# kocurvik/mdrp

Measured on AMD Instinct MI355X. Metric: image-pairs/sec (2000 corrs, 10k RANSAC iters), higher is better.
Workload: dtype f64

## Files before the change

### include/mdrp.h

```cpp
#ifndef MDRP_H
#define MDRP_H
#include <stddef.h>
#include <stdint.h>

#ifdef __cplusplus
extern "C" {
#endif

enum { MDRP_CALIB = 0, MDRP_SHARED_FOCAL = 1, MDRP_VARYING_FOCAL = 2,
       MDRP_RELPOSE_5PT = 3, MDRP_FUNDAMENTAL_7PT = 5,
       MDRP_SHARED_6PT = 4 };

enum {
    MDRP_OK = 0,
    MDRP_ERR_INVALID = 1,
    MDRP_ERR_HIP = 2,
    MDRP_ERR_NO_DEVICE = 3,
    MDRP_ERR_UNSUPPORTED = 4
};

enum {
    MDRP_MEM_HOST = 0,
    MDRP_MEM_DEVICE = 1
};

typedef struct {
    double q[4];
    double t[3];
    double scale, shift1, shift2;
    double f1, f2;
} mdrp_model;

typedef struct {
    uint64_t max_iterations;
    uint64_t min_iterations;
    double dyn_num_trials_mult;
    double success_prob;
    double max_reproj_error;
    double max_epipolar_error;
    uint64_t seed;
    int32_t monodepth_estimate_shift;
    float monodepth_weight_sampson;
    int32_t score_initial_model;
    int32_t progressive_sampling;
    uint64_t max_prosac_iterations;
    int32_t real_focal_check;
    int32_t reserved_;
} mdrp_ransac_opt;

typedef struct {
    uint64_t max_iterations;
    int32_t loss_type;
    double loss_scale;
    double gradient_tol;
    double step_tol;
    double initial_lambda;
    double min_lambda;
    double max_lambda;
} mdrp_bundle_opt;

typedef struct {
    int32_t model_id;
    int32_t pad_;
    double params[4];
} mdrp_camera;

typedef struct {
    mdrp_model model;
    uint64_t refinements, iterations, num_inliers;
    double inlier_ratio, model_score;
} mdrp_result;

typedef struct mdrp_handle mdrp_handle;

int mdrp_create_(int device, void *stream, mdrp_handle **out, int abi_version, int ransac_opt_bytes);
int mdrp_create_on_stream_(int device, void *stream, mdrp_handle **out, int abi_version, int ransac_opt_bytes);
#define mdrp_create(device, stream, out) mdrp_create_((device), (stream), (out), MDRP_ABI_VERSION, (int)sizeof(mdrp_ransac_opt))
#define mdrp_create_on_stream(device, stream, out) mdrp_create_on_stream_((device), (stream), (out), MDRP_ABI_VERSION, (int)sizeof(mdrp_ransac_opt))
void mdrp_destroy(mdrp_handle *h);
const char *mdrp_last_error(void);
const char *mdrp_version(void);
#define MDRP_ABI_VERSION 0x00000005
int mdrp_abi_version(void);
int mdrp_hip_build_version(void);
int mdrp_synchronize(mdrp_handle *h);

int mdrp_estimate_batch(mdrp_handle *h, int kind, int mem_space, const double *x1, const double *x2, const double *d1,
                        const double *d2, int batch, int n_max, const int32_t *n_per_pair, const mdrp_camera *cam1,
                        const mdrp_camera *cam2, const mdrp_ransac_opt *ropt, const mdrp_bundle_opt *bopt,
                        mdrp_result *out, uint8_t *inlier_mask);

int mdrp_estimate_batch_async(mdrp_handle *h, int kind, const double *x1_dev, const double *x2_dev, const double *d1_dev,
                              const double *d2_dev, int batch, int n_max, const int32_t *n_per_pair_host,
                              const mdrp_camera *cam1_host, const mdrp_camera *cam2_host, const mdrp_ransac_opt *ropt,
                              const mdrp_bundle_opt *bopt, uint8_t *inlier_mask_dev);
int mdrp_fetch_results(mdrp_handle *h, mdrp_result *out_host, int batch);
int mdrp_copy_results_device(mdrp_handle *h, void *dst_dev, int batch);

int mdrp_solver_batch(mdrp_handle *h, int solver, const double *x1h, const double *x2h, const double *d1,
                      const double *d2, int count, mdrp_model *out, int32_t *n_out);

int mdrp_classic_solver_batch(mdrp_handle *h, int kind, const double *x1h, const double *x2h, int count, mdrp_model *out,
                              int32_t *n_out);

int mdrp_score_models(mdrp_handle *h, int kind, int mem_space, const mdrp_model *models, int num_models,
                      const double *x1, const double *x2, int n, double sq_threshold, double *scores, int32_t *counts);

int mdrp_count_candidates(mdrp_handle *h, int kind, const mdrp_model *models, int num_models, const double *x1,
                          const double *x2, int n, double sq_threshold, int32_t *candidates);

int mdrp_bound_models(mdrp_handle *h, int kind, const mdrp_model *models, int num_models, const double *x1, const double *x2,
                      int n, double sq_threshold, double *score_lb, int32_t *count_ub);

int mdrp_refine_models(mdrp_handle *h, int kind, mdrp_model *models, int count, const double *x1, const double *x2,
                       const double *d1, const double *d2, int n, double scale_reproj, double weight_sampson,
                       const mdrp_bundle_opt *opt, int estimate_shift, double *final_cost );

int mdrp_last_sweep_stats(mdrp_handle *h, double *sweep_ms, int64_t *launches, int64_t *evaluations);

typedef struct {
    double count_ms;
    int64_t count_launches;
    double sweep_ms;
    int64_t sweep_launches;
    int64_t evals_algorithmic;
    int64_t evals_mfma;
    int64_t evals_fp64;
    int64_t evals_bound;
    double lo_ms;
    int64_t lo_launches;
    double final_ms;
    int64_t final_launches;
    double bound_ms;
    int64_t bound_launches;
    double solve_ms;
    int64_t solve_launches;
    int64_t lm_cost_evals;
    int64_t lm_accum_evals;
    int64_t final_cost_evals;
    int64_t final_accum_evals;
    int64_t fuse_gate_timeouts;
    int64_t fuse_wait_timeouts;
    int64_t first_chunk;
} mdrp_stats;
int mdrp_last_stats_sized(mdrp_handle *h, mdrp_stats *out, size_t out_size);
int mdrp_last_stats(mdrp_handle *h, mdrp_stats *out);

#ifdef __cplusplus
}
#endif
#endif
```

### mdrp_amd/_capi.py

```python
import ctypes as C
import os
import threading

import numpy as np

_HERE = os.path.dirname(os.path.abspath(__file__))
LIB_PATH = os.environ.get("MDRP_LIB") or os.path.join(_HERE, "libmdrp_hip.so")

CALIB, SHARED_FOCAL, VARYING_FOCAL = 0, 1, 2
RELPOSE_5PT, SHARED_6PT, FUNDAMENTAL_7PT = 3, 4, 5
MEM_HOST, MEM_DEVICE = 0, 1
SOLVER_P3P, SOLVER_SHIFT, SOLVER_SHARED, SOLVER_VARYING = 0, 1, 2, 3

EXPORTS = (
    "mdrp_create_", "mdrp_create_on_stream_", "mdrp_destroy", "mdrp_last_error", "mdrp_version", "mdrp_abi_version", "mdrp_hip_build_version", "mdrp_synchronize", "mdrp_estimate_batch",
    "mdrp_estimate_batch_async", "mdrp_fetch_results", "mdrp_copy_results_device", "mdrp_solver_batch", "mdrp_score_models", "mdrp_count_candidates", "mdrp_bound_models", "mdrp_refine_models",
    "mdrp_last_sweep_stats", "mdrp_last_stats", "mdrp_last_stats_sized", "mdrp_classic_solver_batch",
)


class Model(C.Structure):
    _fields_ = [("q", C.c_double * 4), ("t", C.c_double * 3), ("scale", C.c_double), ("shift1", C.c_double),
                ("shift2", C.c_double), ("f1", C.c_double), ("f2", C.c_double)]


class RansacOpt(C.Structure):
    _fields_ = [("max_iterations", C.c_uint64), ("min_iterations", C.c_uint64), ("dyn_num_trials_mult", C.c_double),
                ("success_prob", C.c_double), ("max_reproj_error", C.c_double), ("max_epipolar_error", C.c_double),
                ("seed", C.c_uint64), ("monodepth_estimate_shift", C.c_int32), ("monodepth_weight_sampson", C.c_float),
                ("score_initial_model", C.c_int32), ("progressive_sampling", C.c_int32), ("max_prosac_iterations", C.c_uint64),
                ("real_focal_check", C.c_int32), ("reserved_", C.c_int32)]


class BundleOpt(C.Structure):
    _fields_ = [("max_iterations", C.c_uint64), ("loss_type", C.c_int32), ("loss_scale", C.c_double),
                ("gradient_tol", C.c_double), ("step_tol", C.c_double), ("initial_lambda", C.c_double),
                ("min_lambda", C.c_double), ("max_lambda", C.c_double)]


class Camera(C.Structure):
    _fields_ = [("model_id", C.c_int32), ("pad_", C.c_int32), ("params", C.c_double * 4)]


class Stats(C.Structure):
    _fields_ = [("count_ms", C.c_double), ("count_launches", C.c_int64), ("sweep_ms", C.c_double), ("sweep_launches", C.c_int64),
                ("evals_algorithmic", C.c_int64), ("evals_mfma", C.c_int64), ("evals_fp64", C.c_int64), ("evals_bound", C.c_int64),
                ("lo_ms", C.c_double), ("lo_launches", C.c_int64), ("final_ms", C.c_double), ("final_launches", C.c_int64),
                ("bound_ms", C.c_double), ("bound_launches", C.c_int64), ("solve_ms", C.c_double), ("solve_launches", C.c_int64),
                ("lm_cost_evals", C.c_int64), ("lm_accum_evals", C.c_int64), ("final_cost_evals", C.c_int64), ("final_accum_evals", C.c_int64),
                ("fuse_gate_timeouts", C.c_int64), ("fuse_wait_timeouts", C.c_int64),
                ("first_chunk", C.c_int64)]


class Result(C.Structure):
    _fields_ = [("model", Model), ("refinements", C.c_uint64), ("iterations", C.c_uint64), ("num_inliers", C.c_uint64),
                ("inlier_ratio", C.c_double), ("model_score", C.c_double)]


MODEL_DTYPE = np.dtype([("q", "f8", 4), ("t", "f8", 3), ("scale", "f8"), ("shift1", "f8"), ("shift2", "f8"), ("f1", "f8"), ("f2", "f8")])
RESULT_DTYPE = np.dtype([("model", MODEL_DTYPE), ("refinements", "u8"), ("iterations", "u8"), ("num_inliers", "u8"),
                         ("inlier_ratio", "f8"), ("model_score", "f8")])
CAMERA_DTYPE = np.dtype([("model_id", "i4"), ("pad_", "i4"), ("params", "f8", 4)])
assert MODEL_DTYPE.itemsize == C.sizeof(Model) and RESULT_DTYPE.itemsize == C.sizeof(Result) and CAMERA_DTYPE.itemsize == C.sizeof(Camera)

_lib = None
_lib_lock = threading.Lock()


class MdrpError(RuntimeError):
    pass


def load_library():
    global _lib
    with _lib_lock:
        if _lib is not None:
            return _lib
        if not os.path.exists(LIB_PATH):
            raise MdrpError(f"{LIB_PATH} is not built (run __graft_entry__.build()); mdrp_amd has no CPU fallback")
        _ensure_hip_runtime()
        lib = C.CDLL(LIB_PATH)
        _check_hip_runtime_version(lib)
        vp, dp, ip = C.c_void_p, C.c_void_p, C.c_void_p
        lib.mdrp_last_error.restype = C.c_char_p
        lib.mdrp_version.restype = C.c_char_p
        abi = getattr(lib, "mdrp_abi_version", None)
        if abi is None or getattr(lib, "mdrp_create_", None) is None:
            raise MdrpError(f"{LIB_PATH} predates ABI {ABI_VERSION:#x} (no mdrp_abi_version / mdrp_create_): rebuild (mdrp_amd/build.py)")
        abi.restype = C.c_int
        if abi() != ABI_VERSION:
            raise MdrpError(f"{LIB_PATH} speaks ABI {abi():#x}, this binding {ABI_VERSION:#x}: rebuild (mdrp_amd/build.py)")
        lib.mdrp_create_.argtypes = [C.c_int, vp, C.POINTER(vp), C.c_int, C.c_int]
        lib.mdrp_create_on_stream_.argtypes = [C.c_int, vp, C.POINTER(vp), C.c_int, C.c_int]
        lib.mdrp_destroy.argtypes = [vp]
        lib.mdrp_destroy.restype = None
        lib.mdrp_synchronize.argtypes = [vp]
        lib.mdrp_estimate_batch.argtypes = [vp, C.c_int, C.c_int, dp, dp, dp, dp, C.c_int, C.c_int, ip, vp, vp,
                                            C.POINTER(RansacOpt), C.POINTER(BundleOpt), vp, vp]
        lib.mdrp_estimate_batch_async.argtypes = [vp, C.c_int, dp, dp, dp, dp, C.c_int, C.c_int, ip, vp, vp,
                                                  C.POINTER(RansacOpt), C.POINTER(BundleOpt), vp]
        lib.mdrp_fetch_results.argtypes = [vp, vp, C.c_int]
        lib.mdrp_copy_results_device.argtypes = [vp, vp, C.c_int]
        lib.mdrp_solver_batch.argtypes = [vp, C.c_int, dp, dp, dp, dp, C.c_int, vp, vp]
        lib.mdrp_score_models.argtypes = [vp, C.c_int, C.c_int, vp, C.c_int, dp, dp, C.c_int, C.c_double, vp, vp]
        lib.mdrp_count_candidates.argtypes = [vp, C.c_int, vp, C.c_int, dp, dp, C.c_int, C.c_double, vp]
        lib.mdrp_bound_models.argtypes = [vp, C.c_int, vp, C.c_int, dp, dp, C.c_int, C.c_double, vp, vp]
        lib.mdrp_refine_models.argtypes = [vp, C.c_int, vp, C.c_int, dp, dp, dp, dp, C.c_int, C.c_double, C.c_double,
                                           C.POINTER(BundleOpt), C.c_int, vp]
        lib.mdrp_last_sweep_stats.argtypes = [vp, C.POINTER(C.c_double), C.POINTER(C.c_int64), C.POINTER(C.c_int64)]
        lib.mdrp_last_stats.argtypes = [vp, C.POINTER(Stats)]
        lib.mdrp_last_stats_sized.argtypes = [vp, C.POINTER(Stats), C.c_size_t]
        lib.mdrp_classic_solver_batch.argtypes = [vp, C.c_int, dp, dp, C.c_int, vp, vp]
        _lib = lib
        return lib


ABI_VERSION = 0x00000005
ERR_UNSUPPORTED = 4


def _check(lib, rc):
    if rc == ERR_UNSUPPORTED:
        raise NotImplementedError(f"mdrp: {lib.mdrp_last_error().decode(errors='replace')} (DESIGN.md 9)")
    if rc != 0:
        raise MdrpError(f"mdrp error {rc}: {lib.mdrp_last_error().decode(errors='replace')}")


def _ptr(a):
    return None if a is None else C.c_void_p(a.ctypes.data)


def ransac_opt_from_dict(d=None):
    d = d or {}
    return RansacOpt(int(d.get("max_iterations", 100000)), int(d.get("min_iterations", 1000)),
                     float(d.get("dyn_num_trials_mult", 3.0)), float(d.get("success_prob", 0.9999)),
                     float(d.get("max_reproj_error", 12.0)), float(d.get("max_epipolar_error", 1.0)),
                     int(d.get("seed", 0)), int(bool(d.get("monodepth_estimate_shift", False))),
                     float(d.get("monodepth_weight_sampson", 1.0)), int(bool(d.get("score_initial_model", False))),
                     int(bool(d.get("progressive_sampling", False))), int(d.get("max_prosac_iterations", 100000)),
                     int(bool(d.get("real_focal_check", False))), 0)


LOSS_TYPES = {"TRIVIAL": 0, "TRUNCATED": 1, "HUBER": 2, "CAUCHY": 3, "TRUNCATED_CAUCHY": 4, "TRUNCATED_LE_ZACH": 5}


def bundle_opt_from_dict(d=None):
    d = d or {}
    lt = d.get("loss_type", "CAUCHY")
    if isinstance(lt, str):
        if lt.upper() not in LOSS_TYPES:
            raise ValueError(f"unknown loss_type {lt!r}")
        lt = LOSS_TYPES[lt.upper()]
    return BundleOpt(int(d.get("max_iterations", 100)), int(lt), float(d.get("loss_scale", 1.0)),
                     float(d.get("gradient_tol", 1e-10)), float(d.get("step_tol", 1e-8)), float(d.get("initial_lambda", 1e-3)),
                     float(d.get("min_lambda", 1e-10)), float(d.get("max_lambda", 1e10)))


def library_version():
    return load_library().mdrp_version().decode()


def library_source_hash():
    v = library_version()
    return v.split("MDRP_SRC_HASH=", 1)[1][:16] if "MDRP_SRC_HASH=" in v else None


_hip_runtime = None
hip_versions = None


def _check_hip_runtime_version(lib):
    import warnings
    try:
        lib.mdrp_hip_build_version.restype = C.c_int
        built = int(lib.mdrp_hip_build_version())
        v = C.c_int(0)
        rt = _hip_runtime.hipRuntimeGetVersion
        rt.argtypes = [C.POINTER(C.c_int)]
        if rt(C.byref(v)) != 0:
            return
    except (AttributeError, OSError):
        return
    have = int(v.value)
    if have // 10_000_000 != built // 10_000_000:
        raise MdrpError(f"libmdrp_hip.so was built against HIP {built // 10_000_000}.{built // 100_000 % 100} but the process's HIP runtime "
                        f"({getattr(_hip_runtime, '_name', '?')}) is {have // 10_000_000}.{have // 100_000 % 100}: set MDRP_HIP_RUNTIME to a "
                        "matching libamdhip64.so or rebuild (mdrp_amd/build.py)")
    global hip_versions
    hip_versions = {"built": built, "runtime": have}
    if have // 100_000 != built // 100_000 and os.environ.get("MDRP_DEBUG"):
        warnings.warn(f"mdrp: HIP runtime {have // 10_000_000}.{have // 100_000 % 100} in this process, library built against "
                      f"{built // 10_000_000}.{built // 100_000 % 100} (same major: continuing)", RuntimeWarning, stacklevel=3)


def _ensure_hip_runtime():
    global _hip_runtime
    if _hip_runtime is not None:
        return _hip_runtime
    import sys
    cands = []
    if os.environ.get("MDRP_HIP_RUNTIME"):
        cands.append(os.environ["MDRP_HIP_RUNTIME"])
    try:
        torch = sys.modules.get("torch")
        if torch is not None:
            tdir = os.path.dirname(torch.__file__)
        else:
            import importlib.util
            spec = importlib.util.find_spec("torch")
            tdir = list(spec.submodule_search_locations)[0] if spec is not None and spec.submodule_search_locations else None
        if tdir and os.path.exists(os.path.join(tdir, "lib", "libamdhip64.so")):
            cands.append(os.path.join(tdir, "lib", "libamdhip64.so"))
    except Exception:
        pass
    import glob
    rocm = os.environ.get("ROCM_PATH", "/opt/rocm")
    def _soname_version(path):
        tail = os.path.basename(path).split(".so.", 1)[-1]
        return tuple(int(x) for x in tail.split(".") if x.isdigit())
    cands += sorted(glob.glob(os.path.join(rocm, "lib", "libamdhip64.so.*")), key=_soname_version, reverse=True) + ["libamdhip64.so", os.path.join(rocm, "lib", "libamdhip64.so")]
    errs = []
    for c in cands:
        try:
            _hip_runtime = C.CDLL(c, mode=C.RTLD_GLOBAL)
            return _hip_runtime
        except OSError as e:
            errs.append(f"{c}: {e}")
    raise MdrpError("no HIP runtime (libamdhip64) could be loaded: " + "; ".join(errs))


class Handle:

    def __init__(self, device=0, stream=None):
        self._lib = load_library()
        h = C.c_void_p()
        if stream is None:
            _check(self._lib, self._lib.mdrp_create_(int(device), None, C.byref(h), ABI_VERSION, C.sizeof(RansacOpt)))
        else:
            _check(self._lib, self._lib.mdrp_create_on_stream_(int(device), C.c_void_p(int(stream)) if stream else None, C.byref(h), ABI_VERSION, C.sizeof(RansacOpt)))
        self._h = h
        self.device = int(device)
        self.stream = stream

    def close(self):
        if getattr(self, "_h", None):
            self._lib.mdrp_destroy(self._h)
            self._h = None

    def __del__(self):
        try:
            self.close()
        except Exception:
            pass

    def synchronize(self):
        _check(self._lib, self._lib.mdrp_synchronize(self._h))

    def estimate_batch(self, kind, x1, x2, d1, d2, ropt, bopt, n_per_pair=None, cam1=None, cam2=None, want_mask=True):
        x1 = np.ascontiguousarray(x1, dtype=np.float64)
        x2 = np.ascontiguousarray(x2, dtype=np.float64)
        if x1.ndim != 3 or x1.shape[2] != 2 or x2.shape != x1.shape:
            raise ValueError("expected x1,x2 (B,N,2)")
        if kind >= RELPOSE_5PT:
            d1 = d2 = None
        else:
            d1 = np.ascontiguousarray(d1, dtype=np.float64)
            d2 = np.ascontiguousarray(d2, dtype=np.float64)
            if d1.shape != x1.shape[:2] or d2.shape != d1.shape:
                raise ValueError("expected d1,d2 (B,N)")
        B, N = x1.shape[:2]
        npp = None if n_per_pair is None else np.ascontiguousarray(n_per_pair, dtype=np.int32)
        out = np.zeros(B, dtype=RESULT_DTYPE)
        mask = np.zeros((B, N), dtype=np.uint8) if want_mask else None
        c1 = None if cam1 is None else np.ascontiguousarray(cam1, dtype=CAMERA_DTYPE)
        c2 = None if cam2 is None else np.ascontiguousarray(cam2, dtype=CAMERA_DTYPE)
        _check(self._lib, self._lib.mdrp_estimate_batch(self._h, kind, MEM_HOST, _ptr(x1), _ptr(x2), _ptr(d1), _ptr(d2), B, N,
                                                        _ptr(npp), _ptr(c1), _ptr(c2), C.byref(ropt), C.byref(bopt),
                                                        _ptr(out), _ptr(mask)))
        return out, mask

    def estimate_batch_device(self, kind, x1_ptr, x2_ptr, d1_ptr, d2_ptr, batch, n_max, ropt, bopt, n_per_pair=None,
                              cam1=None, cam2=None, mask_ptr=None):
        npp = None if n_per_pair is None else np.ascontiguousarray(n_per_pair, dtype=np.int32)
        c1 = None if cam1 is None else np.ascontiguousarray(cam1, dtype=CAMERA_DTYPE)
        c2 = None if cam2 is None else np.ascontiguousarray(cam2, dtype=CAMERA_DTYPE)
        _check(self._lib, self._lib.mdrp_estimate_batch_async(self._h, kind, C.c_void_p(x1_ptr), C.c_void_p(x2_ptr),
                                                              C.c_void_p(d1_ptr) if d1_ptr else None, C.c_void_p(d2_ptr) if d2_ptr else None, int(batch), int(n_max),
                                                              _ptr(npp), _ptr(c1), _ptr(c2), C.byref(ropt), C.byref(bopt),
                                                              C.c_void_p(mask_ptr) if mask_ptr else None))

    def fetch_results(self, batch):
        out = np.zeros(batch, dtype=RESULT_DTYPE)
        _check(self._lib, self._lib.mdrp_fetch_results(self._h, _ptr(out), int(batch)))
        return out

    def copy_results_device(self, dst_ptr, batch):
        _check(self._lib, self._lib.mdrp_copy_results_device(self._h, C.c_void_p(dst_ptr), int(batch)))

    def last_sweep_stats(self):
        ms, launches, evals = C.c_double(0), C.c_int64(0), C.c_int64(0)
        _check(self._lib, self._lib.mdrp_last_sweep_stats(self._h, C.byref(ms), C.byref(launches), C.byref(evals)))
        return ms.value, launches.value, evals.value

    def last_stats(self):
        st = Stats()
        _check(self._lib, self._lib.mdrp_last_stats_sized(self._h, C.byref(st), C.sizeof(Stats)))
        d = {k: getattr(st, k) for k, _ in Stats._fields_}
        d["fuse_timeouts"] = d["fuse_gate_timeouts"] + d["fuse_wait_timeouts"]
        return d

    def solver_batch(self, solver, x1h, x2h, d1, d2):
        x1h = np.ascontiguousarray(x1h, dtype=np.float64).reshape(-1, 3, 3)
        x2h = np.ascontiguousarray(x2h, dtype=np.float64).reshape(-1, 3, 3)
        d1 = np.ascontiguousarray(d1, dtype=np.float64).reshape(-1, 3)
        d2 = np.ascontiguousarray(d2, dtype=np.float64).reshape(-1, 3)
        count = len(d1)
        out = np.zeros((count, 4), dtype=MODEL_DTYPE)
        n_out = np.zeros(count, dtype=np.int32)
        _check(self._lib, self._lib.mdrp_solver_batch(self._h, int(solver), _ptr(x1h), _ptr(x2h), _ptr(d1), _ptr(d2), count,
                                                      _ptr(out), _ptr(n_out)))
        return out, n_out

    def classic_solver_batch(self, kind, x1h, x2h):
        K, M = {RELPOSE_5PT: (5, 10), SHARED_6PT: (6, 15), FUNDAMENTAL_7PT: (7, 3)}[kind]
        x1h = np.ascontiguousarray(x1h, dtype=np.float64).reshape(-1, K, 3)
        x2h = np.ascontiguousarray(x2h, dtype=np.float64).reshape(-1, K, 3)
        count = len(x1h)
        out = np.zeros((count, M), dtype=MODEL_DTYPE)
        n_out = np.zeros(count, dtype=np.int32)
        _check(self._lib, self._lib.mdrp_classic_solver_batch(self._h, int(kind), _ptr(x1h), _ptr(x2h), count, _ptr(out), _ptr(n_out)))
        return out, n_out

    def score_models(self, kind, models, x1, x2, sq_threshold):
        models = np.ascontiguousarray(models, dtype=MODEL_DTYPE).reshape(-1)
        x1 = np.ascontiguousarray(x1, dtype=np.float64)
        x2 = np.ascontiguousarray(x2, dtype=np.float64)
        scores = np.zeros(len(models))
        counts = np.zeros(len(models), dtype=np.int32)
        _check(self._lib, self._lib.mdrp_score_models(self._h, int(kind), MEM_HOST, _ptr(models), len(models), _ptr(x1), _ptr(x2),
                                                      len(x1), float(sq_threshold), _ptr(scores), _ptr(counts)))
        return scores, counts

    def count_candidates(self, kind, models, x1, x2, sq_threshold):
        models = np.ascontiguousarray(models, dtype=MODEL_DTYPE).reshape(-1)
        x1 = np.ascontiguousarray(x1, dtype=np.float64)
        x2 = np.ascontiguousarray(x2, dtype=np.float64)
        cand = np.zeros(len(models), dtype=np.int32)
        _check(self._lib, self._lib.mdrp_count_candidates(self._h, int(kind), _ptr(models), len(models), _ptr(x1), _ptr(x2), len(x1),
                                                          float(sq_threshold), _ptr(cand)))
        return cand

    def bound_models(self, kind, models, x1, x2, sq_threshold):
        models = np.ascontiguousarray(models, dtype=MODEL_DTYPE).reshape(-1)
        x1 = np.ascontiguousarray(x1, dtype=np.float64)
        x2 = np.ascontiguousarray(x2, dtype=np.float64)
        lb = np.zeros(len(models))
        ub = np.zeros(len(models), dtype=np.int32)
        _check(self._lib, self._lib.mdrp_bound_models(self._h, int(kind), _ptr(models), len(models), _ptr(x1), _ptr(x2), len(x1),
                                                      float(sq_threshold), _ptr(lb), _ptr(ub)))
        return lb, ub

    def score_models_device(self, kind, models_ptr, num_models, x1_ptr, x2_ptr, n, sq_threshold, scores_ptr, counts_ptr):
        _check(self._lib, self._lib.mdrp_score_models(self._h, int(kind), MEM_DEVICE, C.c_void_p(models_ptr), int(num_models),
                                                      C.c_void_p(x1_ptr), C.c_void_p(x2_ptr), int(n), float(sq_threshold),
                                                      C.c_void_p(scores_ptr), C.c_void_p(counts_ptr)))

    def refine_models(self, kind, models, x1, x2, d1, d2, scale_reproj, weight_sampson, bopt, estimate_shift=False):
        models = np.ascontiguousarray(models, dtype=MODEL_DTYPE).reshape(-1).copy()
        x1 = np.ascontiguousarray(x1, dtype=np.float64)
        x2 = np.ascontiguousarray(x2, dtype=np.float64)
        d1 = None if d1 is None else np.ascontiguousarray(d1, dtype=np.float64)
        d2 = None if d2 is None else np.ascontiguousarray(d2, dtype=np.float64)
        cost = np.zeros(len(models))
        _check(self._lib, self._lib.mdrp_refine_models(self._h, int(kind), _ptr(models), len(models), _ptr(x1), _ptr(x2), _ptr(d1),
                                                       _ptr(d2), len(x1), float(scale_reproj), float(weight_sampson), C.byref(bopt),
                                                       int(bool(estimate_shift)), _ptr(cost)))
        return models, cost


_default_tls = threading.local()


def default_handle(device=0):
    handles = getattr(_default_tls, "handles", None)
    if handles is None:
        handles = _default_tls.handles = {}
    h = handles.get(device)
    if h is None:
        h = handles[device] = Handle(device)
    return h


def fundamental_to_model(F):
    m = np.zeros((), dtype=MODEL_DTYPE)
    flat = np.asarray(F, dtype=np.float64).reshape(9)
    m["q"] = flat[:4]; m["t"] = flat[4:7]; m["scale"] = flat[7]; m["shift1"] = flat[8]
    m["f1"] = m["f2"] = 1.0
    return m


def model_to_fundamental(m):
    return np.r_[m["q"], m["t"], m["scale"], m["shift1"]].reshape(3, 3).copy()


def model_to_array(m):
    return np.concatenate([m["q"], m["t"], [m["scale"], m["shift1"], m["shift2"], m["f1"], m["f2"]]]).astype(np.float64)


def array_to_models(a):
    a = np.asarray(a, dtype=np.float64).reshape(-1, 12)
    out = np.zeros(len(a), dtype=MODEL_DTYPE)
    out["q"] = a[:, :4]; out["t"] = a[:, 4:7]; out["scale"] = a[:, 7]; out["shift1"] = a[:, 8]; out["shift2"] = a[:, 9]
    out["f1"] = a[:, 10]; out["f2"] = a[:, 11]
    return out
```

### mdrp_amd/csrc/mdrp_capi.hip

```cpp
#include "../../include/mdrp.h"
#include "mdrp_kernels.h"
#include "mdrp_classic.h"
#ifdef MDRP_SPLIT_TU
#define MDRP_INST extern
#include "mdrp_instances.h"
namespace mdrp {
MDRP_INSTANCES_FINAL_64
MDRP_INSTANCES_FINAL_256
MDRP_INSTANCES_CLASSIC
}
#endif

#include <algorithm>
#include <cmath>
#include <cstdio>
#include <cstdlib>
#include <cstddef>
#include <cstring>
#include <functional>
#include <map>
#include <memory>
#include <mutex>
#include <string>
#include <vector>

using namespace mdrp;

static_assert(sizeof(mdrp_model) == sizeof(Model), "model layout");
static_assert(sizeof(mdrp_camera) == sizeof(CamDev), "camera layout");
static_assert(sizeof(mdrp_result) == sizeof(ResultDev), "result layout");

namespace {

thread_local std::string g_err;

#define HIPCHK(expr)                                                                                       \
    do {                                                                                                   \
        hipError_t e_ = (expr);                                                                            \
        if (e_ != hipSuccess) {                                                                            \
            char buf_[512];                                                                                \
            snprintf(buf_, sizeof buf_, "%s failed: %s (%s:%d)", #expr, hipGetErrorString(e_), __FILE__, __LINE__); \
            g_err = buf_;                                                                                  \
            return MDRP_ERR_HIP;                                                                           \
        }                                                                                                  \
    } while (0)

struct DevBuf {
    void *p = nullptr;
    size_t cap = 0;
    DevBuf() = default;
    DevBuf(const DevBuf &) = delete;
    DevBuf &operator=(const DevBuf &) = delete;
    ~DevBuf() { release(); }
    int ensure(size_t bytes) {
        if (bytes <= cap) return MDRP_OK;
        if (p) { (void)hipFree(p); p = nullptr; cap = 0; }
        size_t want = bytes + bytes / 8 + 256;
        hipError_t e = hipMalloc(&p, want);
        if (e != hipSuccess) { g_err = std::string("hipMalloc failed: ") + hipGetErrorString(e); p = nullptr; return MDRP_ERR_HIP; }
        cap = want;
        return MDRP_OK;
    }
    void release() { if (p) (void)hipFree(p); p = nullptr; cap = 0; }
    template <typename T> T *as() const { return reinterpret_cast<T *>(p); }
};

template <typename T, auto Destroy> struct Owned {
    T v = nullptr;
    Owned() = default;
    Owned(Owned &&o) noexcept : v(o.v) { o.v = nullptr; }
    Owned(const Owned &) = delete;
    Owned &operator=(const Owned &) = delete;
    ~Owned() { reset(); }
    void reset() { if (v) (void)Destroy(v); v = nullptr; }
    operator T() const { return v; }
    T operator->() const { return v; }
};
using Stream = Owned<hipStream_t, hipStreamDestroy>;
using Event = Owned<hipEvent_t, hipEventDestroy>;
template <typename T> using Pinned = Owned<T *, hipHostFree>;

struct Progress {
    int32_t n_active, pad_;
    unsigned long long max_needed;
    unsigned long long evals;
    unsigned long long evals_mfma;
    unsigned long long evals_sweep;
    unsigned long long evals_bound;
    int32_t wish_sum, wish_pairs;
};
struct Counters {
    int32_t unused_[2];
    Progress progress;
    int32_t lo_head[16];
    int32_t xcd_head[8 * LO_XCD_STRIDE];
};
static_assert(offsetof(Counters, progress) == 2 * sizeof(int32_t) && offsetof(Counters, lo_head) == 16 * sizeof(int32_t) &&
              offsetof(Counters, xcd_head) == 32 * sizeof(int32_t) && sizeof(Counters) == 640, "counter block layout");
static_assert(offsetof(Progress, evals_mfma) == offsetof(Progress, evals) + sizeof(unsigned long long), "k_count adds to stats[0] and stats[1]");
static_assert(offsetof(Progress, wish_pairs) == offsetof(Progress, wish_sum) + sizeof(int32_t), "RunParams::inl_stat is [2]");
constexpr size_t LM_STATS_BYTES = 6 * sizeof(unsigned long long);

struct DeviceGuard {
    int prev = -1;
    bool ok = true;
    explicit DeviceGuard(int device) {
        if (hipGetDevice(&prev) != hipSuccess) prev = -1;
        if (prev != device) ok = hipSetDevice(device) == hipSuccess;
    }
    ~DeviceGuard() {
        int cur = -1;
        if (prev >= 0 && hipGetDevice(&cur) == hipSuccess && cur != prev) (void)hipSetDevice(prev);
    }
};

}

struct mdrp_handle {
    std::mutex mu;
    int device = 0;
    hipStream_t stream = nullptr;
    Stream own_stream;
    Stream aux_stream;
    Stream aux_stream2;
    Stream copy_stream;
    Event ev_copied, ev_prepped, ev_solved6;
    DevBuf fuse;
    static constexpr int NC_MAX = 8;
    Event ev_lo, ev_tables, ev_sampled[2], ev_solved[NC_MAX], ev_scanned[NC_MAX];
    int num_cu = 256;
    DevBuf pts, dep, st;
    DevBuf params;
    Pinned<unsigned char> params_host;
    size_t params_host_cap = 0;
    DevBuf models, slot_score, slot_inl, triggers, work_pair, counters, results, mask, plan;
    DevBuf samples[2], tags[2], model_count[2];
    DevBuf tags_sorted[2];
    DevBuf tags_v, surv_count;
    DevBuf cand_stat;
    DevBuf und_count;
    DevBuf rfrag;
    DevBuf cplan;
    DevBuf surv2_count;
    DevBuf lo_mask;
    DevBuf red5;
    DevBuf lm_stats;
    Pinned<unsigned long long> lm_stats_host;
    int64_t fuse_gate_timeouts = 0, fuse_wait_timeouts = 0;
    int64_t first_chunk = 0;
    double seen_wish[3] = {-1.0, -1.0, -1.0};
    Pinned<int32_t> wish_host; Event ev_wish;
    int wish_kind = -1;
    bool fuse_disabled = false;
    int fuse_retry_in = 0;
    int fuse_backoff = 64;
    DevBuf in_x1, in_x2, in_d1, in_d2;
    DevBuf unit_a, unit_b, unit_c, unit_d, unit_e, unit_f;
    Pinned<Progress> progress_host;
    std::vector<std::pair<Event, Event>> ev_pool;
    std::vector<int> ev_what;
    size_t ev_used = 0;
    double sweep_ms = 0.0, count_ms = 0.0;
    double kind_ms[6] = {0, 0, 0, 0, 0, 0};
    int64_t kind_launches[6] = {0, 0, 0, 0, 0, 0};
    int64_t lm_cost_evals = 0, lm_accum_evals = 0, fin_cost_evals = 0, fin_accum_evals = 0;
    int64_t count_launches = 0;
    int64_t sweep_launches = 0, sweep_evals = 0, mfma_evals = 0, fp64_evals = 0, bound_evals = 0;
    int last_batch = 0;
};

namespace {

#define MDRP_LM_DISPATCH_T(KERNEL, T, kind, shift, grid, smem, stream, ...)                                          \
    do {                                                                                                             \
        if ((kind) == 0 && (shift)) hipLaunchKernelGGL((KERNEL<0, true, T>), grid, dim3(T), smem, stream, __VA_ARGS__);  \
        else if ((kind) == 0) hipLaunchKernelGGL((KERNEL<0, false, T>), grid, dim3(T), smem, stream, __VA_ARGS__);       \
        else if ((kind) == 1) hipLaunchKernelGGL((KERNEL<1, false, T>), grid, dim3(T), smem, stream, __VA_ARGS__);       \
        else hipLaunchKernelGGL((KERNEL<2, false, T>), grid, dim3(T), smem, stream, __VA_ARGS__);                        \
    } while (0)
#define MDRP_LM_DISPATCH(KERNEL, threads, kind, shift, grid, smem, stream, ...)                                      \
    do {                                                                                                             \
        if ((threads) == 64) MDRP_LM_DISPATCH_T(KERNEL, 64, kind, shift, grid, smem, stream, __VA_ARGS__);           \
        else MDRP_LM_DISPATCH_T(KERNEL, 256, kind, shift, grid, smem, stream, __VA_ARGS__);                          \
    } while (0)

#define MDRP_FINAL_DISPATCH_L(T, FL, kind, shift, grid, smem, stream, ...)                                                  \
    do {                                                                                                                   \
        if ((kind) == 0 && (shift)) hipLaunchKernelGGL((k_final<0, true, T, FL>), grid, dim3(T), smem, stream, __VA_ARGS__);  \
        else if ((kind) == 0) hipLaunchKernelGGL((k_final<0, false, T, FL>), grid, dim3(T), smem, stream, __VA_ARGS__);       \
        else if ((kind) == 1) hipLaunchKernelGGL((k_final<1, false, T, FL>), grid, dim3(T), smem, stream, __VA_ARGS__);       \
        else hipLaunchKernelGGL((k_final<2, false, T, FL>), grid, dim3(T), smem, stream, __VA_ARGS__);                        \
    } while (0)
#define MDRP_FINAL_DISPATCH_T(T, floss, kind, shift, grid, smem, stream, ...)                                               \
    do {                                                                                                                   \
        switch (floss) {                                                                                                   \
        case 1: MDRP_FINAL_DISPATCH_L(T, 1, kind, shift, grid, smem, stream, __VA_ARGS__); break;                          \
        case 2: MDRP_FINAL_DISPATCH_L(T, 2, kind, shift, grid, smem, stream, __VA_ARGS__); break;                          \
        case 3: MDRP_FINAL_DISPATCH_L(T, 3, kind, shift, grid, smem, stream, __VA_ARGS__); break;                          \
        case 4: MDRP_FINAL_DISPATCH_L(T, 4, kind, shift, grid, smem, stream, __VA_ARGS__); break;                          \
        case 5: MDRP_FINAL_DISPATCH_L(T, 5, kind, shift, grid, smem, stream, __VA_ARGS__); break;                          \
        default: MDRP_FINAL_DISPATCH_L(T, 0, kind, shift, grid, smem, stream, __VA_ARGS__); break;  \
        }                                                                                                                  \
    } while (0)
#define MDRP_FINAL_DISPATCH(threads, floss, kind, shift, grid, smem, stream, ...)                                           \
    do {                                                                                                                   \
        if ((threads) == 64) MDRP_FINAL_DISPATCH_T(64, floss, kind, shift, grid, smem, stream, __VA_ARGS__);               \
        else MDRP_FINAL_DISPATCH_T(256, floss, kind, shift, grid, smem, stream, __VA_ARGS__);                              \
    } while (0)

#define MDRP_SWEEP_DISPATCH(KERNEL, kind, grid, block, smem, stream, ...)                                                       \
    do {                                                                                                                        \
        if ((kind) == MDRP_CALIB || (kind) == MDRP_RELPOSE_5PT) hipLaunchKernelGGL((KERNEL<true, false>), grid, block, smem, stream, __VA_ARGS__); \
        else if ((kind) == MDRP_FUNDAMENTAL_7PT) hipLaunchKernelGGL((KERNEL<false, true>), grid, block, smem, stream, __VA_ARGS__); \
        else hipLaunchKernelGGL((KERNEL<false, false>), grid, block, smem, stream, __VA_ARGS__);                                 \
    } while (0)
#define MDRP_CLASSIC_LM_DISPATCH(KERNEL, threads, kind, grid, smem, stream, ...)                                                 \
    do {                                                                                                                        \
        if ((kind) == MDRP_RELPOSE_5PT && (threads) == 64) hipLaunchKernelGGL((KERNEL<CLASSIC_RELPOSE, 64>), grid, dim3(64), smem, stream, __VA_ARGS__); \
        else if ((kind) == MDRP_RELPOSE_5PT) hipLaunchKernelGGL((KERNEL<CLASSIC_RELPOSE, 256>), grid, dim3(256), smem, stream, __VA_ARGS__); \
        else if ((kind) == MDRP_SHARED_6PT && (threads) == 64) hipLaunchKernelGGL((KERNEL<CLASSIC_SHARED, 64>), grid, dim3(64), smem, stream, __VA_ARGS__); \
        else if ((kind) == MDRP_SHARED_6PT) hipLaunchKernelGGL((KERNEL<CLASSIC_SHARED, 256>), grid, dim3(256), smem, stream, __VA_ARGS__); \
        else if ((threads) == 64) hipLaunchKernelGGL((KERNEL<CLASSIC_FUND, 64>), grid, dim3(64), smem, stream, __VA_ARGS__);      \
        else hipLaunchKernelGGL((KERNEL<CLASSIC_FUND, 256>), grid, dim3(256), smem, stream, __VA_ARGS__);                        \
    } while (0)

int env_int(const char *name, int dflt) {
    const char *v = getenv(name);
    return v ? atoi(v) : dflt;
}

int lm_list_stride(int n_max) { return n_max <= LM_LIST_MAX_N ? ((n_max + 63) / 64) * 64 : 0; }
size_t lm_list_bytes(int n_max) { return (size_t)2 * lm_list_stride(n_max) * sizeof(uint16_t); }
int lm_mask_index_on(int n_max) { return lm_list_stride(n_max) > 0 && (size_t)3 * lm_list_stride(n_max) * sizeof(uint16_t) <= 32768 ? 1 : 0; }
size_t lm_final_list_bytes(int n_max) { return (size_t)(2 + lm_mask_index_on(n_max)) * lm_list_stride(n_max) * sizeof(uint16_t); }

int get_events(mdrp_handle *h, hipEvent_t *a, hipEvent_t *b, int what = 0) {
    if (h->ev_used == h->ev_pool.size()) {
        Event x, y;
        HIPCHK(hipEventCreate(&x.v));
        HIPCHK(hipEventCreate(&y.v));
        h->ev_pool.emplace_back(std::move(x), std::move(y));
        h->ev_what.push_back(0);
    }
    h->ev_what[h->ev_used] = what;
    *a = h->ev_pool[h->ev_used].first;
    *b = h->ev_pool[h->ev_used].second;
    h->ev_used++;
    return MDRP_OK;
}

int solver_for(int kind, int est_shift) {
    if (kind == MDRP_CALIB) return est_shift ? SOLVER_SHIFT : SOLVER_P3P;
    return kind == MDRP_SHARED_FOCAL ? SOLVER_SHARED : SOLVER_VARYING;
}

int model_slots(int kind) { return kind == MDRP_RELPOSE_5PT ? 12 : (kind == MDRP_SHARED_6PT ? 16 : 4); }
int sample_size(int kind) { return kind == MDRP_RELPOSE_5PT ? 5 : (kind == MDRP_SHARED_6PT ? 6 : (kind == MDRP_FUNDAMENTAL_7PT ? 7 : 3)); }

bool env_chunks(std::vector<uint64_t> &lead) {
    lead.clear();
    const char *e = getenv("MDRP_CHUNKS");
    if (!e) return false;
    const std::string spec = e;
    size_t pos = 0;
    while (pos < spec.size() && (int)lead.size() < mdrp_handle::NC_MAX - 1) {
        const size_t q = spec.find(',', pos);
        const long v = atol(spec.substr(pos, q == std::string::npos ? std::string::npos : q - pos).c_str());
        if (v > 0) lead.push_back((uint64_t)v);
        if (q == std::string::npos) break;
        pos = q + 1;
    }
    return true;
}

struct PassScratch {
    std::vector<std::pair<DevBuf *, size_t>> bufs;
    size_t fuse;
    size_t params, off_cam1, off_cam2, off_tn, off_tof, off_nper;
    size_t red5_blocks, red5_first_blocks;
    size_t total() const {
        size_t t = fuse;
        for (const auto &b : bufs) t += b.second;
        return t;
    }
};

PassScratch pass_scratch(mdrp_handle *h, int kind, int batch, int n_max, int n_tables, int chunk_cap, const std::vector<uint64_t> &lead) {
    const size_t b = (size_t)batch, n = (size_t)n_max, t = (size_t)n_tables, slots = b * chunk_cap * model_slots(kind);
    PassScratch z;
    z.fuse = 64 + 3 * sizeof(int32_t) * b;
    z.off_cam1 = sizeof(uint64_t) * t; z.off_cam2 = z.off_cam1 + sizeof(CamDev) * b; z.off_tn = z.off_cam2 + sizeof(CamDev) * b;
    z.off_tof = z.off_tn + sizeof(int32_t) * t; z.off_nper = z.off_tof + sizeof(int32_t) * b; z.params = z.off_nper + sizeof(int32_t) * b;
    z.red5_blocks = ((size_t)chunk_cap + 63) / 64;
    z.red5_first_blocks = (std::min<uint64_t>(lead.empty() ? 0 : lead[0], (uint64_t)chunk_cap / 2) + 63) / 64;
    const size_t samples = sizeof(uint32_t) * sample_size(kind) * t * chunk_cap, tags = sizeof(uint32_t) * slots, pair2 = sizeof(int32_t) * 2 * b;
    z.bufs = {
        {&h->pts, sizeof(double) * PT_STRIDE * b * n}, {&h->dep, kind >= MDRP_RELPOSE_5PT ? 0 : sizeof(double) * 2 * b * n}, {&h->st, sizeof(PairState) * b},
        {&h->samples[0], samples}, {&h->params, z.params},
        {&h->models, sizeof(Model) * slots}, {&h->slot_score, sizeof(double) * slots}, {&h->slot_inl, sizeof(int32_t) * slots},
        {&h->tags[0], tags}, {&h->model_count[0], pair2}, {&h->model_count[1], pair2}, {&h->tags[1], tags}, {&h->tags_sorted[0], tags},
        {&h->tags_sorted[1], tags}, {&h->samples[1], samples}, {&h->tags_v, tags},
        {&h->surv_count, sizeof(int32_t) * b}, {&h->cand_stat, sizeof(unsigned long long) * 2 * b}, {&h->und_count, pair2},
        {&h->cplan, sizeof(int32_t) * (b + 1)}, {&h->surv2_count, sizeof(int32_t) * b},
        {&h->rfrag, std::max<size_t>(1024, b * ((n + 15) / 16) * 1024)},
        {&h->triggers, sizeof(Trigger) * b * chunk_cap},
        {&h->work_pair, sizeof(int32_t) * (3 * b + 2)},
        {&h->counters, sizeof(Counters)},
        {&h->plan, sizeof(int32_t) * (2 * b + 2 + 4 + 16)},
        {&h->lo_mask, (kind == MDRP_RELPOSE_5PT || kind == MDRP_SHARED_6PT) ? (size_t)h->num_cu * 8 * std::max<size_t>(n, 1) : 0},
        {&h->red5, kind == MDRP_RELPOSE_5PT ? sizeof(double) * b * (z.red5_blocks + z.red5_first_blocks) * RED5_STRIDE * 64 : 0}};
    return z;
}

struct HostSrc { const double *x1, *x2, *d1, *d2; };
constexpr int HOST_SLICE_PAIRS = 256;

int run_pass(mdrp_handle *h, int kind, const double *x1, const double *x2, const double *d1, const double *d2, int batch,
             int n_max, const int32_t *n_host, const mdrp_camera *cam1, const mdrp_camera *cam2, const mdrp_ransac_opt *ro,
             const mdrp_bundle_opt *bo, int chunk_cap, uint8_t *mask_dev, ResultDev *results_dev, const HostSrc *host, int batch_call) {
    hipStream_t s = h->stream;
    const int est_shift = (kind == MDRP_CALIB && ro->monodepth_estimate_shift) ? 1 : 0;
    const bool classic = kind >= MDRP_RELPOSE_5PT;
    const int mps = model_slots(kind), ssz = sample_size(kind);

    std::vector<int32_t> table_of(batch), tab_n;
    {
        std::map<int32_t, int32_t> ids;
        for (int i = 0; i < batch; ++i) {
            auto it = ids.find(n_host[i]);
            if (it == ids.end()) { it = ids.emplace(n_host[i], (int32_t)tab_n.size()).first; tab_n.push_back(n_host[i]); }
            table_of[i] = it->second;
        }
    }
    const int n_tables = (int)tab_n.size();
    std::vector<uint64_t> tab_state(n_tables, ro->seed);

    const uint64_t certain = ro->max_iterations == 0 ? 1 : std::min<uint64_t>(ro->max_iterations, ro->min_iterations + 1);
    std::vector<uint64_t> lead;
    const bool chunks_set = env_chunks(lead);
    if (h->wish_kind >= 0 && hipEventQuery(h->ev_wish) == hipSuccess) {
        if (h->wish_host[1] > 0) h->seen_wish[h->wish_kind] = (double)h->wish_host[0] / (double)h->wish_host[1];
        h->wish_kind = -1;
    }
    if (!chunks_set) {
        if (kind == MDRP_FUNDAMENTAL_7PT) lead = {128, 1024};
        else if (kind == MDRP_SHARED_6PT) lead = {128};
        else if (kind == MDRP_RELPOSE_5PT) lead = {std::min<uint64_t>(512, std::max<uint64_t>(128, certain / 16 / 64 * 64))};
        else {
            lead = {std::min<uint64_t>(256, std::max<uint64_t>(128, certain / 16 / 64 * 64))};
            if (h->seen_wish[kind] >= 0.0 && certain >= 8192)
                lead[0] = (uint64_t)std::min(1024.0, std::max(128.0, std::ceil(h->seen_wish[kind] / 64.0) * 64.0));
        }
    }

    const PassScratch sz = pass_scratch(h, kind, batch, n_max, n_tables, chunk_cap, lead);
    int rc;
    for (const auto &b : sz.bufs) {
        if ((rc = b.first->ensure(b.second))) return rc;
        if (b.first == &h->params && h->params_host_cap < sz.params) {
            h->params_host.reset(); h->params_host_cap = 0;
            HIPCHK(hipHostMalloc((void **)&h->params_host.v, sz.params + sz.params / 2, hipHostMallocDefault));
            h->params_host_cap = sz.params + sz.params / 2;
        }
    }
    unsigned char *pd = h->params.as<unsigned char>();
    uint64_t *d_table_state = reinterpret_cast<uint64_t *>(pd);
    CamDev *d_cams1 = reinterpret_cast<CamDev *>(pd + sz.off_cam1), *d_cams2 = reinterpret_cast<CamDev *>(pd + sz.off_cam2);
    int32_t *d_table_n = reinterpret_cast<int32_t *>(pd + sz.off_tn), *d_table_of = reinterpret_cast<int32_t *>(pd + sz.off_tof),
            *d_nper = reinterpret_cast<int32_t *>(pd + sz.off_nper);
    Counters *cnt = h->counters.as<Counters>();
    const size_t groups_max = ((size_t)n_max + 15) / 16;
    const int trig_cap = chunk_cap;

    {
        unsigned char *ph = h->params_host;
        std::memcpy(ph, tab_state.data(), sizeof(uint64_t) * n_tables);
        const bool cams = kind == MDRP_CALIB || kind == MDRP_RELPOSE_5PT || kind == MDRP_SHARED_6PT;
        if (cams) { std::memcpy(ph + sz.off_cam1, cam1, sizeof(CamDev) * batch); std::memcpy(ph + sz.off_cam2, cam2 ? cam2 : cam1, sizeof(CamDev) * batch); }
        else std::memset(ph + sz.off_cam1, 0, 2 * sizeof(CamDev) * (size_t)batch);
        std::memcpy(ph + sz.off_tn, tab_n.data(), sizeof(int32_t) * n_tables);
        std::memcpy(ph + sz.off_tof, table_of.data(), sizeof(int32_t) * batch);
        std::memcpy(ph + sz.off_nper, n_host, sizeof(int32_t) * batch);
        HIPCHK(hipMemcpyAsync(pd, ph, sz.params, hipMemcpyHostToDevice, s));
    }
    HIPCHK(hipEventRecord(h->ev_tables, s));

    RunParams rp;
    std::memset(&rp, 0, sizeof rp);
    rp.kind = kind; rp.solver = solver_for(kind, est_shift); rp.est_shift = est_shift;
    rp.score_initial = ro->score_initial_model ? 1 : 0;
    rp.batch = batch; rp.n_max = n_max;
    rp.max_iterations = ro->max_iterations; rp.min_iterations = ro->min_iterations;
    rp.dyn_mult = ro->dyn_num_trials_mult; rp.log_prob_missing = std::log(1.0 - ro->success_prob);
    rp.weight_sampson = ro->monodepth_weight_sampson > 0.0f ? (double)ro->monodepth_weight_sampson : 0.0;
    rp.final_max_it = (int)std::min<uint64_t>(bo->max_iterations, 1u << 30); rp.final_loss = bo->loss_type;
    rp.grad_tol = bo->gradient_tol; rp.step_tol = bo->step_tol; rp.lambda0 = bo->initial_lambda;
    rp.lambda_min = bo->min_lambda; rp.lambda_max = bo->max_lambda;
    rp.chunk_len = chunk_cap; rp.chunk_off = 0; rp.slot_stride = chunk_cap * mps; rp.super_len = chunk_cap; rp.chunk_start = 0;
    rp.mps = mps; rp.sample_sz = ssz;

    auto launch_prep = [&](int p0, int pc, hipStream_t ps_) {
        const size_t o2 = (size_t)2 * p0 * n_max, o1 = (size_t)p0 * n_max;
        double *pts_p = h->pts.as<double>() + o1 * PT_STRIDE;
        uint4 *rfrag_p = h->rfrag.as<uint4>() + (size_t)p0 * groups_max * 64;
        if (classic)
            hipLaunchKernelGGL(kc_prep, dim3(pc), dim3(256), 0, ps_, rp, x1 + o2, x2 + o2, d_nper + p0, d_table_of + p0, d_cams1 + p0, d_cams2 + p0,
                               ro->max_epipolar_error, bo->loss_scale, pts_p, h->st.as<PairState>() + p0, rfrag_p);
        else
            hipLaunchKernelGGL(k_prep, dim3(pc), dim3(256), 0, ps_, rp, x1 + o2, x2 + o2, d1 + o1, d2 + o1, d_nper + p0, d_table_of + p0, d_cams1 + p0, d_cams2 + p0,
                               ro->max_epipolar_error, ro->max_reproj_error, bo->loss_scale, pts_p, h->dep.as<double>() + 2 * o1, h->st.as<PairState>() + p0, rfrag_p);
    };
    if (!host) {
        launch_prep(0, batch, s);
        HIPCHK(hipGetLastError());
    }
    rp.inl_stat = classic ? nullptr : &cnt->progress.wish_sum;

    const bool lo_overlap = env_int("MDRP_LO_OVERLAP", 1) != 0;
    const bool use_bound = env_int("MDRP_BOUND", 1) != 0;
    const bool score_split = env_int("MDRP_SCORE_SPLIT", 1) != 0;
    const int lo_threads = env_int("MDRP_LO_THREADS", (batch_call >= 128 && n_max < 4096) ? 64 : 256);
    const int final_threads = env_int("MDRP_FINAL_THREADS", batch_call >= 4096 ? 64 : 256);
    const int mask_index = lm_mask_index_on(n_max);
    const int clm_list_stride = lm_list_stride(n_max);
    const size_t clm_list_bytes = (size_t)2 * clm_list_stride * sizeof(uint16_t);
    const bool fuse_env = env_int("MDRP_FUSE_TAIL", ((kind == MDRP_CALIB && est_shift) || h->fuse_disabled) ? 0 : 1) != 0;
    bool final_done = false;
    auto launch_final = [&](const int32_t *ready, int32_t *fin_done, unsigned long long ticks, unsigned long long *timeouts) {
        if (classic)
            MDRP_CLASSIC_LM_DISPATCH(kc_final, final_threads, kind, dim3(batch), clm_list_bytes, s, rp, h->st.as<PairState>(), h->pts.as<double>(), mask_dev, results_dev,
                                     ready, fin_done, ticks, timeouts, clm_list_stride);
        else
            MDRP_FINAL_DISPATCH(final_threads, rp.final_loss, kind, est_shift, dim3(batch), (mask_index ? lm_final_list_bytes(n_max) : lm_list_bytes(n_max)), s, rp,
                                h->st.as<PairState>(), h->pts.as<double>(), h->dep.as<double>(), mask_dev, results_dev, lm_list_stride(n_max), mask_index,
                                h->lm_stats.as<unsigned long long>() + 2, ready, fin_done, ticks, timeouts);
    };
    const size_t tile_bytes = SCORE_TILE_BYTES;

    uint64_t it0 = 0;
    uint64_t max_needed = 0;
    while (true) {
        uint64_t lens[mdrp_handle::NC_MAX] = {0};
        int n_chunks = 1;
        if (it0 < certain) {
            const uint64_t span = std::min<uint64_t>(certain - it0, (uint64_t)chunk_cap);
            uint64_t used = 0;
            n_chunks = 0;
            if (it0 == 0)
                for (uint64_t l : lead) {
                    if (used + 2 * l > span) break;
                    lens[n_chunks++] = l; used += l;
                }
            lens[n_chunks++] = span - used;
        } else {
            lens[0] = std::min<uint64_t>(std::min<uint64_t>(std::max<uint64_t>(max_needed, 256), ro->max_iterations - it0), (uint64_t)chunk_cap);
        }
        uint64_t super_len = 0;
        for (int c = 0; c < n_chunks; ++c) super_len += lens[c];
        if (it0 == 0) h->first_chunk = (int64_t)lens[0];
        rp.chunk_start = it0; rp.super_len = (int)super_len;
        HIPCHK(hipMemsetAsync(h->counters.p, 0, sizeof(Counters), s));
        if (it0 == 0) HIPCHK(hipMemsetAsync(h->cand_stat.p, 0, sizeof(unsigned long long) * 2 * batch, s));
        const bool piped = n_chunks > 1 && lo_overlap;
        const bool fuse_tail = fuse_env && piped && it0 + super_len >= ro->max_iterations;
        int32_t *fz_ctl = nullptr, *fz_done = nullptr, *fz_fin = nullptr, *fz_ready = nullptr;
        if (fuse_tail) {
            if ((rc = h->fuse.ensure(sz.fuse))) return rc;
            fz_ctl = h->fuse.as<int32_t>(); fz_done = fz_ctl + 16; fz_fin = fz_done + batch; fz_ready = fz_fin + batch;
        }
        hipStream_t aux = piped ? h->aux_stream : s, aux2 = piped ? h->aux_stream2 : s;
        int offs[mdrp_handle::NC_MAX] = {0};
        for (int c = 1; c < n_chunks; ++c) offs[c] = offs[c - 1] + (int)lens[c - 1];
        const int samp_threads = env_int("MDRP_SAMPLE_THREADS", ssz == 3 ? SAMP_THREADS : (ssz == 5 ? 512 : 256));
        auto launch_samples = [&](hipStream_t st_, int len_, uint32_t *smp_) {
            if (ssz == 6) hipLaunchKernelGGL(kc_samples<6>, dim3(n_tables), dim3(samp_threads), 0, st_, n_tables, d_table_n, d_table_state, len_, smp_);
            else if (ssz == 5) hipLaunchKernelGGL(kc_samples<5>, dim3(n_tables), dim3(samp_threads), 0, st_, n_tables, d_table_n, d_table_state, len_, smp_);
            else if (ssz == 7) hipLaunchKernelGGL(kc_samples<7>, dim3(n_tables), dim3(samp_threads), 0, st_, n_tables, d_table_n, d_table_state, len_, smp_);
            else hipLaunchKernelGGL(k_samples, dim3(n_tables), dim3(samp_threads), 0, st_, n_tables, d_table_n, d_table_state, len_, smp_);
        };
        bool presampled[2] = {false, false};
        if (piped && it0 == 0) {
            HIPCHK(hipStreamWaitEvent(aux2, h->ev_tables, 0));
            for (int c = 0; c < 2 && c < n_chunks; ++c) {
                launch_samples(aux2, (int)lens[c], h->samples[c & 1].as<uint32_t>());
                HIPCHK(hipEventRecord(h->ev_sampled[c], aux2));
                presampled[c] = true;
            }
        }
        auto issue_solve = [&](int c, hipStream_t st_, int p0, int pc) -> int {
            RunParams r = rp;
            r.chunk_len = (int)lens[c]; r.chunk_off = offs[c]; r.batch = pc;
            const size_t so = (size_t)p0 * rp.slot_stride;
            uint32_t *tg = h->tags[c & 1].as<uint32_t>() + so;
            uint32_t *smp = h->samples[c & 1].as<uint32_t>();
            int32_t *mc = h->model_count[c & 1].as<int32_t>() + 2 * (size_t)p0;
            HIPCHK(hipMemsetAsync(mc, 0, sizeof(int32_t) * 2 * pc, st_));
            if (c < 2 && presampled[c]) HIPCHK(hipStreamWaitEvent(st_, h->ev_sampled[c], 0));
            else launch_samples(st_, r.chunk_len, smp);
            hipEvent_t v0, v1;
            int rc_;
            if ((rc_ = get_events(h, &v0, &v1, 5))) return rc_;
            HIPCHK(hipEventRecord(v0, st_));
            struct Stop { hipEvent_t e; hipStream_t s; ~Stop() { (void)hipEventRecord(e, s); } } stop_{v1, st_};
            PairState *st_p = h->st.as<PairState>() + p0;
            double *pts_p = h->pts.as<double>() + (size_t)p0 * n_max * PT_STRIDE;
            Model *models_p = h->models.as<Model>() + so;
            int32_t *inl_p = h->slot_inl.as<int32_t>() + so;
            if (classic) {
                const dim3 sgrid((r.chunk_len + 63) / 64, pc);
                if (kind == MDRP_SHARED_6PT)
                    hipLaunchKernelGGL(kc_solve<CLASSIC_SHARED>, sgrid, dim3(64), 0, st_, r, st_p, smp, pts_p, models_p, inl_p, tg, mc);
                else if (kind == MDRP_RELPOSE_5PT) {
                    const bool first_region = c == 0 && n_chunks > 1;
                    if (first_region && (size_t)sgrid.x > sz.red5_first_blocks) { g_err = "5-point first chunk longer than its Reduce5 region"; return MDRP_ERR_INVALID; }
                    double *red5 = h->red5.as<double>() + ((first_region ? (size_t)batch * sz.red5_blocks : 0) + (size_t)p0 * sgrid.x) * RED5_STRIDE * 64;
                    hipLaunchKernelGGL(kc_solve5_null, sgrid, dim3(64), SOLVE5N_LDS_BYTES, st_, r, st_p, smp, pts_p, red5);
                    hipLaunchKernelGGL(kc_solve5_reduce, sgrid, dim3(64), SOLVE5_LDS_BYTES, st_, r, st_p, red5);
                    hipLaunchKernelGGL(kc_solve5_roots, sgrid, dim3(64), SOLVE5B_LDS_BYTES, st_, r, st_p, smp, pts_p, red5, models_p, inl_p, tg, mc);
                }
                else
                    hipLaunchKernelGGL(kc_solve<CLASSIC_FUND>, sgrid, dim3(64), SOLVE7_LDS_BYTES, st_, r, st_p, smp, pts_p, models_p, inl_p, tg, mc);
                return MDRP_OK;
            }
            double *dep_p = h->dep.as<double>() + (size_t)p0 * n_max * 2;
#define MDRP_SOLVE_LAUNCH(S)                                                                                                   \
    hipLaunchKernelGGL(k_solve<S>, dim3((r.chunk_len + solve_threads(S) - 1) / solve_threads(S), pc), dim3(solve_threads(S)), 0, st_, r, st_p, smp, pts_p, dep_p, models_p, inl_p, tg, mc, 0, r.chunk_len)
            switch (r.solver) {
            case SOLVER_P3P: MDRP_SOLVE_LAUNCH(SOLVER_P3P); break;
            case SOLVER_SHIFT: MDRP_SOLVE_LAUNCH(SOLVER_SHIFT); break;
            case SOLVER_SHARED: MDRP_SOLVE_LAUNCH(SOLVER_SHARED); break;
            default: MDRP_SOLVE_LAUNCH(SOLVER_VARYING); break;
            }
#undef MDRP_SOLVE_LAUNCH
            return MDRP_OK;
        };
        auto sweep_chunk = [&](int c, int p0, int pc) -> int {
            RunParams r = rp;
            r.chunk_len = (int)lens[c]; r.chunk_off = offs[c]; r.batch = pc;
            const int len = r.chunk_len;
            const bool odd = c & 1;
            const size_t so = (size_t)p0 * rp.slot_stride;
            PairState *st_p = h->st.as<PairState>() + p0;
            const double *pts_p = h->pts.as<double>() + (size_t)p0 * n_max * PT_STRIDE;
            const Model *models_p = h->models.as<Model>() + so;
            uint32_t *tags_sc = h->tags_sorted[odd].as<uint32_t>() + so;
            int32_t *mcount_c = h->model_count[odd].as<int32_t>() + 2 * (size_t)p0;
            uint32_t *tags_c = h->tags[odd].as<uint32_t>() + so;
            uint32_t *tags_v = h->tags_v.as<uint32_t>() + so;
            int32_t *surv1 = h->surv_count.as<int32_t>() + p0, *surv2 = h->surv2_count.as<int32_t>() + p0;
            hipEvent_t e0, e1;
            int rc_;
            if ((rc_ = get_events(h, &e0, &e1, 0))) return rc_;
            unsigned long long *cstats = &cnt->progress.evals;
            {
                hipEvent_t c0, c1;
                if ((rc_ = get_events(h, &c0, &c1, 1))) return rc_;
                const bool two_phase = !(it0 == 0 && c == 0);
                unsigned long long *cand_stat = h->cand_stat.as<unsigned long long>() + 2 * (size_t)p0;
                uint32_t *tags_u = tags_sc;
                int32_t *und_part = reinterpret_cast<int32_t *>(h->tags_sorted[!odd].as<uint32_t>() + so), *und_cnt = h->und_count.as<int32_t>() + 2 * (size_t)p0;
                const uint4 *rfrag_p = h->rfrag.as<uint4>() + (size_t)p0 * groups_max * 64;
                hipLaunchKernelGGL(k_count_plan, dim3(1), dim3(PLAN_THREADS), 0, s, pc, st_p, mcount_c, 2, CNT_WG_MODELS, h->cplan.as<int32_t>(),
                                   surv1, (const int32_t *)nullptr, two_phase ? und_cnt : (int32_t *)nullptr);
                const dim3 cgrid((unsigned)pc * (unsigned)((len * mps + CNT_WG_MODELS - 1) / CNT_WG_MODELS));
                HIPCHK(hipEventRecord(c0, s));
                MDRP_SWEEP_DISPATCH(k_count, kind, cgrid, dim3(CNT_THREADS), 0, s, r, st_p, rfrag_p, models_p,
                                    tags_c, mcount_c, h->cplan.as<int32_t>(), tags_v, surv1, cstats, (int32_t *)nullptr, (const int32_t *)nullptr,
                                    1, tags_u, und_part, und_cnt, (const int32_t *)nullptr, cand_stat);
                if (two_phase) {
                    hipLaunchKernelGGL(k_count_plan, dim3(1), dim3(PLAN_THREADS), 0, s, pc, st_p, und_cnt, 2, CNT_WG_MODELS, h->cplan.as<int32_t>(),
                                       (int32_t *)nullptr, (const int32_t *)nullptr, (int32_t *)nullptr);
                    MDRP_SWEEP_DISPATCH(k_count, kind, cgrid, dim3(CNT_THREADS), 0, s, r, st_p, rfrag_p, models_p,
                                        tags_u, und_cnt, h->cplan.as<int32_t>(), tags_v, surv1, cstats, (int32_t *)nullptr, (const int32_t *)nullptr,
                                        2, (uint32_t *)nullptr, (int32_t *)nullptr, (int32_t *)nullptr, und_part, cand_stat);
                    h->count_launches++;
                }
                HIPCHK(hipEventRecord(c1, s));
                h->count_launches++;
            }
            const uint32_t *surv_tags = tags_v;
            const int32_t *surv_cnt = surv1;
            if (use_bound && batch_call > 16 && !(it0 == 0 && c == 0)) {
                hipLaunchKernelGGL(k_count_plan, dim3(1), dim3(PLAN_THREADS), 0, s, pc, st_p, surv1, 1, BND_THREADS, h->cplan.as<int32_t>(), surv2, (const int32_t *)nullptr);
                const dim3 bgrid((unsigned)pc * (unsigned)((len * mps + BND_THREADS - 1) / BND_THREADS));
                unsigned long long *bstats = &cnt->progress.evals_bound;
                hipEvent_t b0, b1;
                if ((rc_ = get_events(h, &b0, &b1, 4))) return rc_;
                HIPCHK(hipEventRecord(b0, s));
                MDRP_SWEEP_DISPATCH(k_bound, kind, bgrid, dim3(BND_THREADS), 0, s, r, st_p, pts_p, models_p, tags_v, surv1, h->cplan.as<int32_t>(), tags_c, surv2, bstats);
                HIPCHK(hipEventRecord(b1, s));
                surv_tags = tags_c; surv_cnt = surv2;
            }
            int32_t *plan = h->plan.as<int32_t>(), *totals = plan + 2 * (size_t)batch + 2;
            if (batch_call <= SCORE_WAVE_MAX_PAIRS) {
                hipLaunchKernelGGL(k_count_plan, dim3(1), dim3(PLAN_THREADS), 0, s, pc, st_p, surv_cnt, 1, SCW_THREADS / 64, plan, (int32_t *)nullptr, (const int32_t *)nullptr, (int32_t *)nullptr);
                hipLaunchKernelGGL(k_sort_tags, dim3(pc), dim3(256), 0, s, r, st_p, mcount_c, surv_cnt, surv_tags, tags_sc);
                HIPCHK(hipEventRecord(e0, s));
                const long long ub = (long long)pc * ((len * mps + SCW_THREADS / 64 - 1) / (SCW_THREADS / 64));
                const dim3 grid((unsigned)std::min<long long>(ub, (long long)h->num_cu * 32));
                MDRP_SWEEP_DISPATCH(k_score_w, kind, grid, dim3(SCW_THREADS), 0, s, r, st_p, pts_p, models_p, tags_sc, mcount_c,
                                    h->slot_score.as<double>() + so, h->slot_inl.as<int32_t>() + so, plan);
            } else if (score_split && !(it0 == 0 && c == 0)) {
                hipLaunchKernelGGL(k_sort_tags, dim3(pc), dim3(256), 0, s, r, st_p, mcount_c, surv_cnt, surv_tags, tags_sc);
                hipLaunchKernelGGL(k_plan, dim3(1), dim3(PLAN_THREADS), 0, s, pc, mcount_c, plan, totals, SPLIT_HYP);
                HIPCHK(hipEventRecord(e0, s));
                const long long ub = (long long)pc * ((len * mps + SPLIT_HYP - 1) / SPLIT_HYP + 1);
                const dim3 grid((unsigned)std::min<long long>(ub, (long long)h->num_cu * 32));
                MDRP_SWEEP_DISPATCH(k_score_split, kind, grid, dim3(SPLIT_THREADS), 0, s, r, st_p, pts_p, models_p, tags_sc, mcount_c,
                                    h->slot_score.as<double>() + so, h->slot_inl.as<int32_t>() + so, plan, totals);
            } else {
                hipLaunchKernelGGL(k_sort_tags, dim3(pc), dim3(256), 0, s, r, st_p, mcount_c, surv_cnt, surv_tags, tags_sc);
                hipLaunchKernelGGL(k_plan, dim3(1), dim3(PLAN_THREADS), 0, s, pc, mcount_c, plan, totals, SCORE_THREADS);
                HIPCHK(hipEventRecord(e0, s));
                const dim3 grid((unsigned)pc * (unsigned)((len * mps + SCORE_THREADS - 1) / SCORE_THREADS));
                MDRP_SWEEP_DISPATCH(k_score, kind, grid, dim3(SCORE_THREADS), tile_bytes, s, r, st_p, pts_p, models_p, tags_sc, mcount_c,
                                    h->slot_score.as<double>() + so, h->slot_inl.as<int32_t>() + so, plan, totals);
            }
            HIPCHK(hipEventRecord(e1, s));
            h->sweep_launches++;
            Trigger *trig_p = h->triggers.as<Trigger>() + (size_t)p0 * trig_cap;
            unsigned long long *scan_stats = &cnt->progress.evals_sweep;
#define MDRP_SCAN(M, I) hipLaunchKernelGGL((k_scan<M, I>), dim3(pc), dim3(64), 0, s, r, st_p, h->slot_score.as<double>() + so, h->slot_inl.as<int32_t>() + so, trig_p, trig_cap, mcount_c, scan_stats)
            if (mps == 16) MDRP_SCAN(16, 1);
            else if (mps == 12) MDRP_SCAN(12, 1);
            else if (len >= 1024) MDRP_SCAN(4, 4);
            else MDRP_SCAN(4, 1);
#undef MDRP_SCAN
            return MDRP_OK;
        };
        bool solved1 = false;
        int swept0 = 0;
        if (host && it0 == 0) {
            const bool sliced = piped && n_chunks >= 2 && batch >= 2 * HOST_SLICE_PAIRS;
            const int sl = sliced ? HOST_SLICE_PAIRS : batch;
            for (int p0 = 0; p0 < batch; p0 += sl) {
                const int pc = std::min(sl, batch - p0);
                const size_t o2 = (size_t)2 * p0 * n_max, o1 = (size_t)p0 * n_max, n2 = sizeof(double) * 2 * (size_t)pc * n_max, n1 = sizeof(double) * (size_t)pc * n_max;
                hipStream_t cs = sliced ? h->copy_stream : s;
                HIPCHK(hipMemcpyAsync(const_cast<double *>(x1) + o2, host->x1 + o2, n2, hipMemcpyHostToDevice, cs));
                HIPCHK(hipMemcpyAsync(const_cast<double *>(x2) + o2, host->x2 + o2, n2, hipMemcpyHostToDevice, cs));
                if (host->d1 && host->d2) {
                    HIPCHK(hipMemcpyAsync(const_cast<double *>(d1) + o1, host->d1 + o1, n1, hipMemcpyHostToDevice, cs));
                    HIPCHK(hipMemcpyAsync(const_cast<double *>(d2) + o1, host->d2 + o1, n1, hipMemcpyHostToDevice, cs));
                }
                if (!sliced) { launch_prep(p0, pc, s); break; }
                HIPCHK(hipEventRecord(h->ev_copied, cs)); HIPCHK(hipStreamWaitEvent(aux, h->ev_copied, 0));
                if (p0 == 0) HIPCHK(hipStreamWaitEvent(aux, h->ev_tables, 0));
                launch_prep(p0, pc, aux);
                HIPCHK(hipEventRecord(h->ev_prepped, aux));
                if ((rc = issue_solve(1, aux, p0, pc))) return rc;
                const bool last = p0 + sl >= batch, last_but_one = !last && p0 + 2 * sl >= batch;
                if (last_but_one || last) HIPCHK(hipStreamWaitEvent(s, h->ev_prepped, 0));
                auto solve_first = [&](int q0, int qc) -> int {
                    if (kind != MDRP_SHARED_6PT) return issue_solve(0, s, q0, qc);
                    int rc_ = issue_solve(0, aux, q0, qc);
                    if (rc_) return rc_;
                    HIPCHK(hipEventRecord(h->ev_solved6, aux));
                    HIPCHK(hipStreamWaitEvent(s, h->ev_solved6, 0));
                    return MDRP_OK;
                };
                if (last_but_one) { swept0 = p0 + pc; if ((rc = solve_first(0, swept0)) || (rc = sweep_chunk(0, 0, swept0))) return rc; }
                if (last) { if ((rc = solve_first(swept0, batch - swept0)) || (rc = sweep_chunk(0, swept0, batch - swept0))) return rc; swept0 = batch; }
            }
            if (sliced) { HIPCHK(hipEventRecord(h->ev_solved[1], aux)); solved1 = true; }
        }
        if (swept0 < batch && (rc = issue_solve(0, s, 0, batch))) return rc;
        if (piped) HIPCHK(hipEventRecord(h->ev_solved[0], s));
        for (int c = 0; c < n_chunks; ++c) {
            rp.chunk_len = (int)lens[c]; rp.chunk_off = offs[c];
            if (c == 0 && swept0 >= batch) {
                if (piped) HIPCHK(hipEventRecord(h->ev_scanned[0], s));
                continue;
            }
            if (piped && c + 1 < n_chunks && !(c == 0 && solved1)) {
                HIPCHK(hipStreamWaitEvent(aux, c == 0 ? h->ev_solved[0] : h->ev_scanned[c - 1], 0));
                if ((rc = issue_solve(c + 1, aux, 0, batch))) return rc;
                HIPCHK(hipEventRecord(h->ev_solved[c + 1], aux));
            }
            if (piped && c > 0) HIPCHK(hipStreamWaitEvent(s, h->ev_solved[c], 0));
            if (!piped && c > 0 && (rc = issue_solve(c, s, 0, batch))) return rc;
            if ((rc = sweep_chunk(c, 0, batch))) return rc;
            if (c + 1 < n_chunks) {
                if (piped) HIPCHK(hipEventRecord(h->ev_scanned[c], s));
                continue;
            }
            int32_t *lo_plan = h->work_pair.as<int32_t>();
            hipLaunchKernelGGL(k_lo_plan, dim3(1), dim3(PLAN_THREADS), 0, s, batch, h->st.as<PairState>(), (const int32_t *)nullptr, lo_plan);
            if (fuse_tail) {
                HIPCHK(hipMemsetAsync(fz_ctl, 0, 64 + 2 * sizeof(int32_t) * (size_t)batch, s));
                HIPCHK(hipMemsetAsync(fz_ready, 0xFF, sizeof(int32_t) * (size_t)batch, s));
            }
            if (piped) { HIPCHK(hipEventRecord(h->ev_scanned[c], s)); HIPCHK(hipStreamWaitEvent(aux2, h->ev_scanned[c], 0)); }
            const int lo_blocks = h->num_cu * (lo_threads == 64 ? 8 : 2);
            const FuseTail fz = fuse_tail ? FuseTail{fz_done, fz_ready, fz_ctl, h->st.as<PairState>()} : FuseTail{nullptr, nullptr, nullptr, nullptr};
            unsigned long long *lm_stats = h->lm_stats.as<unsigned long long>();
            int32_t *xheads = cnt->xcd_head;
            hipEvent_t l0, l1;
            if ((rc = get_events(h, &l0, &l1, 2))) return rc;
            HIPCHK(hipEventRecord(l0, aux2));
            if (classic)
                MDRP_CLASSIC_LM_DISPATCH(kc_lo, lo_threads, kind, dim3(lo_blocks), clm_list_bytes, aux2, rp, h->st.as<PairState>(), h->pts.as<double>(),
                                         h->models.as<Model>(), h->triggers.as<Trigger>(), trig_cap, lo_plan, cnt->lo_head, xheads,
                                         h->lo_mask.as<uint8_t>(), clm_list_stride, fz);
            else
                MDRP_LM_DISPATCH(k_lo, lo_threads, kind, est_shift, dim3(lo_blocks), lm_list_bytes(n_max), aux2, rp,
                                 h->st.as<PairState>(), h->pts.as<double>(), h->dep.as<double>(), h->models.as<Model>(), h->triggers.as<Trigger>(),
                                 trig_cap, lo_plan, cnt->lo_head, xheads, lm_list_stride(n_max), lm_stats, fz);
            HIPCHK(hipEventRecord(l1, aux2));
        }
        if (fuse_tail) {
            const int32_t *plan_l = h->work_pair.as<int32_t>();
            const int lo_blocks_l = h->num_cu * (lo_threads == 64 ? 8 : 2);
            const long long n_scale = std::max(1, (n_max + 1999) / 2000);
            const unsigned long long gate_ticks = 100ull * (unsigned long long)env_int("MDRP_FUSE_GATE_US", (int)std::min<long long>((50000 + 40ll * batch) * n_scale, 200000));
            const unsigned long long wait_ticks = 100ull * (unsigned long long)env_int("MDRP_FUSE_WAIT_US", (int)std::min<long long>((20000 + 4ll * batch) * n_scale, 100000));
            hipLaunchKernelGGL(k_gate, dim3(1), dim3(1), 0, s, (const int32_t *)cnt->lo_head, plan_l + 3 * (size_t)batch + 1,
                               (const int32_t *)fz_ctl, lo_blocks_l, gate_ticks, h->lm_stats.as<unsigned long long>() + 4);
            hipEvent_t g0, g1;
            if ((rc = get_events(h, &g0, &g1, 3))) return rc;
            HIPCHK(hipEventRecord(g0, s));
            launch_final(fz_ready, fz_fin, wait_ticks, h->lm_stats.as<unsigned long long>() + 5);
            HIPCHK(hipEventRecord(g1, s));
            final_done = true;
        }
        if (piped) { HIPCHK(hipEventRecord(h->ev_lo, aux2)); HIPCHK(hipStreamWaitEvent(s, h->ev_lo, 0)); }
        if (fuse_tail)
            launch_final(nullptr, fz_fin, 0, nullptr);
        if (!fuse_tail)
            hipLaunchKernelGGL(k_walk, dim3((batch + 63) / 64), dim3(64), 0, s, rp, h->st.as<PairState>(), h->models.as<Model>(),
                               h->triggers.as<Trigger>(), trig_cap, &cnt->progress.n_active, &cnt->progress.max_needed,
                               (const int32_t *)nullptr, 0, 0, 0);
        HIPCHK(hipGetLastError());
        HIPCHK(hipMemcpyAsync(h->progress_host, &cnt->progress, sizeof(Progress), hipMemcpyDeviceToHost, s));
        HIPCHK(hipStreamSynchronize(s));
        h->sweep_evals += (int64_t)h->progress_host->evals;
        h->mfma_evals += (int64_t)h->progress_host->evals_mfma;
        h->fp64_evals += (int64_t)h->progress_host->evals_sweep;
        h->bound_evals += (int64_t)h->progress_host->evals_bound;
        if (final_done && h->progress_host->wish_pairs > 0)
            h->seen_wish[kind] = (double)h->progress_host->wish_sum / (double)h->progress_host->wish_pairs;
        if (getenv("MDRP_DEBUG"))
            fprintf(stderr, "[mdrp] super-chunk start %llu len %llu (%d chunks): evals %llu (mfma %llu, fp32 bound %llu, fp64 sweep %llu = %.2f %%) active %d max_needed %llu\n",
                    (unsigned long long)it0, (unsigned long long)super_len, n_chunks, h->progress_host->evals, h->progress_host->evals_mfma,
                    h->progress_host->evals_bound, h->progress_host->evals_sweep, 100.0 * (double)h->progress_host->evals_sweep / (double)std::max<unsigned long long>(1, h->progress_host->evals),
                    h->progress_host->n_active, h->progress_host->max_needed);
        it0 += super_len;
        if (h->progress_host->n_active == 0 || it0 >= ro->max_iterations) break;
        max_needed = h->progress_host->max_needed;
    }

    if (final_done) return MDRP_OK;
    hipEvent_t f0, f1;
    if ((rc = get_events(h, &f0, &f1, 3))) return rc;
    HIPCHK(hipEventRecord(f0, s));
    launch_final(nullptr, nullptr, 0, nullptr);
    HIPCHK(hipEventRecord(f1, s));
    if (rp.inl_stat && h->wish_kind < 0) {
        HIPCHK(hipMemcpyAsync(h->wish_host, rp.inl_stat, 2 * sizeof(int32_t), hipMemcpyDeviceToHost, s));
        HIPCHK(hipEventRecord(h->ev_wish, s));
        h->wish_kind = kind;
    }
    HIPCHK(hipGetLastError());
// ... 249 lines not shown
        if ((rc = h->in_x1.ensure(sizeof(double) * 2 * np + 16)) || (rc = h->in_x2.ensure(sizeof(double) * 2 * np + 16)) ||
            (rc = h->in_d1.ensure(sizeof(double) * np + 16)) || (rc = h->in_d2.ensure(sizeof(double) * np + 16)))
            return rc;
        hsrc = HostSrc{x1, x2, (d1 && d2) ? d1 : nullptr, (d1 && d2) ? d2 : nullptr};
        if (d1 && d2) { d1 = h->in_d1.as<double>(); d2 = h->in_d2.as<double>(); }
        x1 = h->in_x1.as<double>(); x2 = h->in_x2.as<double>();
        use_host = true;
        mask_dev = nullptr;
    }
    rc = estimate_device(h, kind, x1, x2, d1, d2, batch, n_max, n_per_pair, cam1, cam2, ropt, bopt, mask_dev, use_host ? &hsrc : nullptr);
    if (rc) return rc;
    if (mem_space == MDRP_MEM_HOST && inlier_mask && np > 0)
        HIPCHK(hipMemcpyAsync(inlier_mask, h->mask.p, np, hipMemcpyDeviceToHost, h->stream));
    return fetch_results_locked(h, out, batch);
}

int mdrp_last_sweep_stats(mdrp_handle *h, double *sweep_ms, int64_t *launches, int64_t *evaluations) {
    if (!h) return MDRP_ERR_INVALID;
    std::lock_guard<std::mutex> lock_(h->mu);
    if (sweep_ms) *sweep_ms = h->sweep_ms;
    if (launches) *launches = h->sweep_launches;
    if (evaluations) *evaluations = h->sweep_evals;
    return MDRP_OK;
}

int mdrp_last_stats_sized(mdrp_handle *h, mdrp_stats *out, size_t out_size) {
    if (!h || !out || out_size < sizeof(double)) return MDRP_ERR_INVALID;
    std::lock_guard<std::mutex> lock_(h->mu);
    mdrp_stats full, *caller = out;
    out = &full;
    out->count_ms = h->count_ms; out->count_launches = h->count_launches;
    out->sweep_ms = h->sweep_ms; out->sweep_launches = h->sweep_launches;
    out->evals_algorithmic = h->sweep_evals; out->evals_mfma = h->mfma_evals; out->evals_fp64 = h->fp64_evals; out->evals_bound = h->bound_evals;
    out->lo_ms = h->kind_ms[2]; out->lo_launches = h->kind_launches[2]; out->final_ms = h->kind_ms[3]; out->final_launches = h->kind_launches[3];
    out->bound_ms = h->kind_ms[4]; out->bound_launches = h->kind_launches[4]; out->solve_ms = h->kind_ms[5]; out->solve_launches = h->kind_launches[5];
    out->lm_cost_evals = h->lm_cost_evals; out->lm_accum_evals = h->lm_accum_evals;
    out->final_cost_evals = h->fin_cost_evals; out->final_accum_evals = h->fin_accum_evals;
    out->fuse_gate_timeouts = h->fuse_gate_timeouts; out->fuse_wait_timeouts = h->fuse_wait_timeouts;
    out->first_chunk = h->first_chunk;
    std::memcpy(caller, &full, std::min(out_size, sizeof full));
    return MDRP_OK;
}

int mdrp_last_stats(mdrp_handle *h, mdrp_stats *out) { return mdrp_last_stats_sized(h, out, offsetof(mdrp_stats, fuse_gate_timeouts)); }

int mdrp_solver_batch(mdrp_handle *h, int solver, const double *x1h, const double *x2h, const double *d1, const double *d2,
                      int count, mdrp_model *out, int32_t *n_out) {
    if (!h || count < 0 || solver < 0 || solver > 3 || !out || !n_out) { g_err = "invalid argument"; return MDRP_ERR_INVALID; }
    if (count == 0) return MDRP_OK;
    MDRP_ENTER(h);
    int rc;
    if ((rc = h->unit_a.ensure(sizeof(double) * 9 * count)) || (rc = h->unit_b.ensure(sizeof(double) * 9 * count)) ||
        (rc = h->unit_c.ensure(sizeof(double) * 3 * count)) || (rc = h->unit_d.ensure(sizeof(double) * 3 * count)) ||
        (rc = h->unit_e.ensure(sizeof(Model) * 4 * count)) || (rc = h->unit_f.ensure(sizeof(int32_t) * count)))
        return rc;
    hipStream_t s = h->stream;
    HIPCHK(hipMemcpyAsync(h->unit_a.p, x1h, sizeof(double) * 9 * count, hipMemcpyHostToDevice, s));
    HIPCHK(hipMemcpyAsync(h->unit_b.p, x2h, sizeof(double) * 9 * count, hipMemcpyHostToDevice, s));
    HIPCHK(hipMemcpyAsync(h->unit_c.p, d1, sizeof(double) * 3 * count, hipMemcpyHostToDevice, s));
    HIPCHK(hipMemcpyAsync(h->unit_d.p, d2, sizeof(double) * 3 * count, hipMemcpyHostToDevice, s));
    HIPCHK(hipMemsetAsync(h->unit_e.p, 0, sizeof(Model) * 4 * count, s));
    hipLaunchKernelGGL(k_solver_unit, dim3((count + 63) / 64), dim3(64), 0, s, solver, count, h->unit_a.as<double>(),
                       h->unit_b.as<double>(), h->unit_c.as<double>(), h->unit_d.as<double>(), h->unit_e.as<Model>(), h->unit_f.as<int32_t>());
    HIPCHK(hipGetLastError());
    HIPCHK(hipMemcpyAsync(out, h->unit_e.p, sizeof(Model) * 4 * count, hipMemcpyDeviceToHost, s));
    HIPCHK(hipMemcpyAsync(n_out, h->unit_f.p, sizeof(int32_t) * count, hipMemcpyDeviceToHost, s));
    HIPCHK(hipStreamSynchronize(s));
    return MDRP_OK;
}

int mdrp_classic_solver_batch(mdrp_handle *h, int kind, const double *x1h, const double *x2h, int count, mdrp_model *out, int32_t *n_out) {
    if (!h || count < 0 || kind < MDRP_RELPOSE_5PT || kind > MDRP_FUNDAMENTAL_7PT || !out || !n_out) { g_err = "invalid argument"; return MDRP_ERR_INVALID; }
    if (count == 0) return MDRP_OK;
    MDRP_ENTER(h);
    const int K = kind == MDRP_RELPOSE_5PT ? 5 : (kind == MDRP_SHARED_6PT ? 6 : 7), M = kind == MDRP_RELPOSE_5PT ? MAX_MODELS_5PT : (kind == MDRP_SHARED_6PT ? MAX_MODELS_6PT : 3);
    int rc;
    if ((rc = h->unit_a.ensure(sizeof(double) * 3 * K * count)) || (rc = h->unit_b.ensure(sizeof(double) * 3 * K * count)) ||
        (rc = h->unit_e.ensure(sizeof(Model) * M * count)) || (rc = h->unit_f.ensure(sizeof(int32_t) * count)))
        return rc;
    hipStream_t s = h->stream;
    HIPCHK(hipMemcpyAsync(h->unit_a.p, x1h, sizeof(double) * 3 * K * count, hipMemcpyHostToDevice, s));
    HIPCHK(hipMemcpyAsync(h->unit_b.p, x2h, sizeof(double) * 3 * K * count, hipMemcpyHostToDevice, s));
    HIPCHK(hipMemsetAsync(h->unit_e.p, 0, sizeof(Model) * M * count, s));
    if (kind == MDRP_SHARED_6PT)
        hipLaunchKernelGGL(kc_solver_unit<CLASSIC_SHARED>, dim3((count + 63) / 64), dim3(64), 0, s, count, h->unit_a.as<double>(),
                           h->unit_b.as<double>(), h->unit_e.as<Model>(), h->unit_f.as<int32_t>());
    else if (kind == MDRP_RELPOSE_5PT)
        hipLaunchKernelGGL(kc_solver_unit<CLASSIC_RELPOSE>, dim3((count + 63) / 64), dim3(64), SOLVE5_LDS_BYTES, s, count, h->unit_a.as<double>(),
                           h->unit_b.as<double>(), h->unit_e.as<Model>(), h->unit_f.as<int32_t>());
    else
        hipLaunchKernelGGL(kc_solver_unit<CLASSIC_FUND>, dim3((count + 63) / 64), dim3(64), SOLVE7_LDS_BYTES, s, count, h->unit_a.as<double>(),
                           h->unit_b.as<double>(), h->unit_e.as<Model>(), h->unit_f.as<int32_t>());
    HIPCHK(hipGetLastError());
    HIPCHK(hipMemcpyAsync(out, h->unit_e.p, sizeof(Model) * M * count, hipMemcpyDeviceToHost, s));
    HIPCHK(hipMemcpyAsync(n_out, h->unit_f.p, sizeof(int32_t) * count, hipMemcpyDeviceToHost, s));
    HIPCHK(hipStreamSynchronize(s));
    return MDRP_OK;
}

int mdrp_score_models(mdrp_handle *h, int kind, int mem_space, const mdrp_model *models, int num_models, const double *x1,
                      const double *x2, int n, double sq_threshold, double *scores, int32_t *counts) {
    if (!h || num_models < 0 || n < 0 || kind < 0 || kind > 5 || !scores || !counts) { g_err = "invalid argument"; return MDRP_ERR_INVALID; }
    if (num_models == 0) return MDRP_OK;
    MDRP_ENTER(h);
    hipStream_t s = h->stream;
    const int chunk = (num_models + 3) / 4;
    const size_t slots = (size_t)chunk * 4;
    int rc;
    if ((rc = h->pts.ensure(sizeof(double) * PT_STRIDE * std::max(n, 1))) || (rc = h->st.ensure(sizeof(PairState))) ||
        (rc = h->models.ensure(sizeof(Model) * slots)) || (rc = h->slot_score.ensure(sizeof(double) * slots)) ||
        (rc = h->slot_inl.ensure(sizeof(int32_t) * slots)) || (rc = h->tags[0].ensure(sizeof(uint32_t) * slots)) ||
        (rc = h->model_count[0].ensure(2 * sizeof(int32_t))))
        return rc;
    const double *x1d = x1, *x2d = x2;
    const Model *md = reinterpret_cast<const Model *>(models);
    if (mem_space == MDRP_MEM_HOST) {
        if ((rc = h->in_x1.ensure(sizeof(double) * 2 * std::max(n, 1))) || (rc = h->in_x2.ensure(sizeof(double) * 2 * std::max(n, 1)))) return rc;
        HIPCHK(hipMemcpyAsync(h->in_x1.p, x1, sizeof(double) * 2 * n, hipMemcpyHostToDevice, s));
        HIPCHK(hipMemcpyAsync(h->in_x2.p, x2, sizeof(double) * 2 * n, hipMemcpyHostToDevice, s));
        HIPCHK(hipMemcpyAsync(h->models.p, models, sizeof(Model) * num_models, hipMemcpyHostToDevice, s));
        x1d = h->in_x1.as<double>(); x2d = h->in_x2.as<double>();
        md = h->models.as<Model>();
    } else {
        HIPCHK(hipMemcpyAsync(h->models.p, models, sizeof(Model) * num_models, hipMemcpyDeviceToDevice, s));
        md = h->models.as<Model>();
    }
    if ((rc = upload_iota(s, h->tags[0].p, num_models))) return rc;
    const int32_t counts2[2] = {num_models, 0};
    HIPCHK(hipMemcpyAsync(h->model_count[0].p, counts2, 2 * sizeof(int32_t), hipMemcpyHostToDevice, s));
    if ((rc = stage_unit_pair(h, x1d, x2d, n, sq_threshold))) return rc;
    RunParams rp;
    std::memset(&rp, 0, sizeof rp);
    rp.kind = kind; rp.batch = 1; rp.n_max = std::max(n, 1); rp.chunk_len = chunk; rp.chunk_off = 0; rp.slot_stride = chunk * 4; rp.super_len = chunk;
    rp.mps = 4; rp.sample_sz = 3;
    const size_t tile_bytes = SCORE_TILE_BYTES;
    if ((rc = h->plan.ensure(sizeof(int32_t) * 8))) return rc;
    int32_t *plan = h->plan.as<int32_t>(), *totals = plan + 4;
    hipLaunchKernelGGL(k_plan, dim3(1), dim3(PLAN_THREADS), 0, s, 1, h->model_count[0].as<int32_t>(), plan, totals, SCORE_THREADS);
    const dim3 grid((unsigned)std::min(h->num_cu * 4, (num_models + SCORE_THREADS - 1) / SCORE_THREADS));
    h->ev_used = 0; h->sweep_launches = 1; h->sweep_evals = (int64_t)num_models * n;
    hipEvent_t e0, e1;
    if ((rc = get_events(h, &e0, &e1))) return rc;
    HIPCHK(hipEventRecord(e0, s));
    MDRP_SWEEP_DISPATCH(k_score, kind, grid, dim3(SCORE_THREADS), tile_bytes, s, rp, h->st.as<PairState>(), h->pts.as<double>(), md,
                        h->tags[0].as<uint32_t>(), h->model_count[0].as<int32_t>(), h->slot_score.as<double>(), h->slot_inl.as<int32_t>(), plan, totals);
    HIPCHK(hipEventRecord(e1, s));
    HIPCHK(hipGetLastError());
    const hipMemcpyKind back = mem_space == MDRP_MEM_HOST ? hipMemcpyDeviceToHost : hipMemcpyDeviceToDevice;
    HIPCHK(hipMemcpyAsync(scores, h->slot_score.p, sizeof(double) * num_models, back, s));
    HIPCHK(hipMemcpyAsync(counts, h->slot_inl.p, sizeof(int32_t) * num_models, back, s));
    return finish_timing(h);
}

int mdrp_count_candidates(mdrp_handle *h, int kind, const mdrp_model *models, int num_models, const double *x1, const double *x2,
                          int n, double sq_threshold, int32_t *candidates) {
    if (!h || num_models < 0 || n < 0 || kind < 0 || kind > 5 || !candidates || !models) { g_err = "invalid argument"; return MDRP_ERR_INVALID; }
    if (num_models == 0) return MDRP_OK;
    MDRP_ENTER(h);
    hipStream_t s = h->stream;
    const int nn = std::max(n, 1);
    const size_t slots = (size_t)num_models;
    int rc;
    if ((rc = h->pts.ensure(sizeof(double) * PT_STRIDE * nn)) || (rc = h->st.ensure(sizeof(PairState))) ||
        (rc = h->models.ensure(sizeof(Model) * slots)) || (rc = h->slot_inl.ensure(sizeof(int32_t) * slots)) ||
        (rc = h->tags[0].ensure(sizeof(uint32_t) * slots)) || (rc = h->tags_v.ensure(sizeof(uint32_t) * slots)) ||
        (rc = h->model_count[0].ensure(2 * sizeof(int32_t))) || (rc = h->surv_count.ensure(sizeof(int32_t))) ||
        (rc = h->cplan.ensure(2 * sizeof(int32_t))) || (rc = h->rfrag.ensure((size_t)((nn + 15) / 16) * 1024)) ||
        (rc = h->unit_f.ensure(sizeof(int32_t) * slots)) || (rc = h->in_x1.ensure(sizeof(double) * 2 * nn)) ||
        (rc = h->in_x2.ensure(sizeof(double) * 2 * nn)))
        return rc;
    HIPCHK(hipMemcpyAsync(h->in_x1.p, x1, sizeof(double) * 2 * n, hipMemcpyHostToDevice, s));
    HIPCHK(hipMemcpyAsync(h->in_x2.p, x2, sizeof(double) * 2 * n, hipMemcpyHostToDevice, s));
    HIPCHK(hipMemcpyAsync(h->models.p, models, sizeof(Model) * num_models, hipMemcpyHostToDevice, s));
    if ((rc = upload_iota(s, h->tags[0].p, num_models))) return rc;
    const int32_t counts2[2] = {num_models, 0};
    HIPCHK(hipMemcpyAsync(h->model_count[0].p, counts2, 2 * sizeof(int32_t), hipMemcpyHostToDevice, s));
    HIPCHK(hipMemsetAsync(h->surv_count.p, 0, sizeof(int32_t), s));
    if ((rc = stage_unit_pair(h, h->in_x1.as<double>(), h->in_x2.as<double>(), n, sq_threshold))) return rc;
    hipLaunchKernelGGL(k_frag_unit, dim3((n + 16 + 255) / 256), dim3(256), 0, s, n, h->pts.as<double>(), h->rfrag.as<uint4>());
    RunParams rp;
    std::memset(&rp, 0, sizeof rp);
    rp.kind = kind; rp.batch = 1; rp.n_max = nn; rp.slot_stride = num_models; rp.mps = 4; rp.sample_sz = 3;
    hipLaunchKernelGGL(k_count_plan, dim3(1), dim3(PLAN_THREADS), 0, s, 1, h->st.as<PairState>(), h->model_count[0].as<int32_t>(), 2, CNT_WG_MODELS, h->cplan.as<int32_t>(),
                       (int32_t *)nullptr);
    const dim3 grid((unsigned)((num_models + CNT_WG_MODELS - 1) / CNT_WG_MODELS));
    MDRP_SWEEP_DISPATCH(k_count, kind, grid, dim3(CNT_THREADS), 0, s, rp, h->st.as<PairState>(), h->rfrag.as<uint4>(), h->models.as<Model>(),
                        h->tags[0].as<uint32_t>(), h->model_count[0].as<int32_t>(), h->cplan.as<int32_t>(),
                        h->tags_v.as<uint32_t>(), h->surv_count.as<int32_t>(), (unsigned long long *)nullptr, h->unit_f.as<int32_t>());
    HIPCHK(hipGetLastError());
    HIPCHK(hipMemcpyAsync(candidates, h->unit_f.p, sizeof(int32_t) * num_models, hipMemcpyDeviceToHost, s));
    HIPCHK(hipStreamSynchronize(s));
    return MDRP_OK;
}

int mdrp_bound_models(mdrp_handle *h, int kind, const mdrp_model *models, int num_models, const double *x1, const double *x2,
                      int n, double sq_threshold, double *score_lb, int32_t *count_ub) {
    if (!h || num_models < 0 || n < 0 || kind < 0 || kind > 5 || !score_lb || !count_ub || !models) { g_err = "invalid argument"; return MDRP_ERR_INVALID; }
    if (num_models == 0) return MDRP_OK;
    MDRP_ENTER(h);
    hipStream_t s = h->stream;
    const int nn = std::max(n, 1);
    const size_t slots = (size_t)num_models;
    int rc;
    if ((rc = h->pts.ensure(sizeof(double) * PT_STRIDE * nn)) || (rc = h->st.ensure(sizeof(PairState))) ||
        (rc = h->models.ensure(sizeof(Model) * slots)) || (rc = h->slot_inl.ensure(sizeof(int32_t) * slots)) ||
        (rc = h->tags[0].ensure(sizeof(uint32_t) * slots)) || (rc = h->tags_v.ensure(sizeof(uint32_t) * slots)) ||
        (rc = h->surv_count.ensure(sizeof(int32_t))) || (rc = h->surv2_count.ensure(sizeof(int32_t))) ||
        (rc = h->cplan.ensure(2 * sizeof(int32_t))) || (rc = h->unit_a.ensure(sizeof(double) * slots)) ||
        (rc = h->unit_f.ensure(sizeof(int32_t) * slots)) || (rc = h->in_x1.ensure(sizeof(double) * 2 * nn)) ||
        (rc = h->in_x2.ensure(sizeof(double) * 2 * nn)))
        return rc;
    HIPCHK(hipMemcpyAsync(h->in_x1.p, x1, sizeof(double) * 2 * n, hipMemcpyHostToDevice, s));
    HIPCHK(hipMemcpyAsync(h->in_x2.p, x2, sizeof(double) * 2 * n, hipMemcpyHostToDevice, s));
    HIPCHK(hipMemcpyAsync(h->models.p, models, sizeof(Model) * num_models, hipMemcpyHostToDevice, s));
    if ((rc = upload_iota(s, h->tags_v.p, num_models))) return rc;
    HIPCHK(hipMemcpyAsync(h->surv_count.p, &num_models, sizeof(int32_t), hipMemcpyHostToDevice, s));
    HIPCHK(hipMemsetAsync(h->unit_a.p, 0, sizeof(double) * slots, s));
    HIPCHK(hipMemsetAsync(h->unit_f.p, 0, sizeof(int32_t) * slots, s));
    if ((rc = stage_unit_pair(h, h->in_x1.as<double>(), h->in_x2.as<double>(), n, sq_threshold))) return rc;
    RunParams rp;
    std::memset(&rp, 0, sizeof rp);
    rp.kind = kind; rp.batch = 1; rp.n_max = nn; rp.slot_stride = num_models; rp.mps = 4; rp.sample_sz = 3;
    hipLaunchKernelGGL(k_count_plan, dim3(1), dim3(PLAN_THREADS), 0, s, 1, h->st.as<PairState>(), h->surv_count.as<int32_t>(), 1, BND_THREADS,
                       h->cplan.as<int32_t>(), h->surv2_count.as<int32_t>());
    const dim3 grid((unsigned)((num_models + BND_THREADS - 1) / BND_THREADS));
    MDRP_SWEEP_DISPATCH(k_bound, kind, grid, dim3(BND_THREADS), 0, s, rp, h->st.as<PairState>(), h->pts.as<double>(), h->models.as<Model>(),
                        h->tags_v.as<uint32_t>(), h->surv_count.as<int32_t>(), h->cplan.as<int32_t>(),
                        h->tags[0].as<uint32_t>(), h->surv2_count.as<int32_t>(), (unsigned long long *)nullptr, h->unit_a.as<double>(), h->unit_f.as<int32_t>());
    HIPCHK(hipGetLastError());
    HIPCHK(hipMemcpyAsync(score_lb, h->unit_a.p, sizeof(double) * num_models, hipMemcpyDeviceToHost, s));
    HIPCHK(hipMemcpyAsync(count_ub, h->unit_f.p, sizeof(int32_t) * num_models, hipMemcpyDeviceToHost, s));
    HIPCHK(hipStreamSynchronize(s));
    return MDRP_OK;
}

int mdrp_refine_models(mdrp_handle *h, int kind, mdrp_model *models, int count, const double *x1, const double *x2,
                       const double *d1, const double *d2, int n, double scale_reproj, double weight_sampson,
                       const mdrp_bundle_opt *opt, int estimate_shift, double *final_cost) {
    if (!h || count < 0 || n < 0 || kind < 0 || kind > 5 || !opt || !models) { g_err = "invalid argument"; return MDRP_ERR_INVALID; }
    if (count == 0) return MDRP_OK;
    MDRP_ENTER(h);
    hipStream_t s = h->stream;
    int rc;
    const int nn = std::max(n, 1);
    if (kind >= MDRP_RELPOSE_5PT) {
        if ((rc = h->pts.ensure(sizeof(double) * PT_STRIDE * nn)) || (rc = h->in_x1.ensure(sizeof(double) * 2 * nn)) ||
            (rc = h->in_x2.ensure(sizeof(double) * 2 * nn)) || (rc = h->unit_e.ensure(sizeof(Model) * count)) ||
            (rc = h->unit_a.ensure(sizeof(double) * count)))
            return rc;
        HIPCHK(hipMemcpyAsync(h->in_x1.p, x1, sizeof(double) * 2 * n, hipMemcpyHostToDevice, s));
        HIPCHK(hipMemcpyAsync(h->in_x2.p, x2, sizeof(double) * 2 * n, hipMemcpyHostToDevice, s));
        HIPCHK(hipMemcpyAsync(h->unit_e.p, models, sizeof(Model) * count, hipMemcpyHostToDevice, s));
        hipLaunchKernelGGL(k_pack_unit, dim3((n + 255) / 256 + 1), dim3(256), 0, s, n, h->in_x1.as<double>(), h->in_x2.as<double>(),
                           (const double *)nullptr, (const double *)nullptr, h->pts.as<double>(), (double *)nullptr);
        MDRP_CLASSIC_LM_DISPATCH(kc_refine_unit, (count >= 2048 ? 64 : 256), kind, dim3(count), 0, s, count, h->unit_e.as<Model>(),
                                 h->pts.as<double>(), n, lm_opt(opt), h->unit_a.as<double>());
        HIPCHK(hipGetLastError());
        HIPCHK(hipMemcpyAsync(models, h->unit_e.p, sizeof(Model) * count, hipMemcpyDeviceToHost, s));
        if (final_cost) HIPCHK(hipMemcpyAsync(final_cost, h->unit_a.p, sizeof(double) * count, hipMemcpyDeviceToHost, s));
        HIPCHK(hipStreamSynchronize(s));
        return MDRP_OK;
    }
    if ((rc = h->pts.ensure(sizeof(double) * PT_STRIDE * nn)) || (rc = h->dep.ensure(sizeof(double) * 2 * nn)) ||
        (rc = h->in_x1.ensure(sizeof(double) * 2 * nn)) || (rc = h->in_x2.ensure(sizeof(double) * 2 * nn)) ||
        (rc = h->in_d1.ensure(sizeof(double) * nn)) || (rc = h->in_d2.ensure(sizeof(double) * nn)) ||
        (rc = h->unit_e.ensure(sizeof(Model) * count)) || (rc = h->unit_a.ensure(sizeof(double) * count)))
        return rc;
    HIPCHK(hipMemcpyAsync(h->in_x1.p, x1, sizeof(double) * 2 * n, hipMemcpyHostToDevice, s));
    HIPCHK(hipMemcpyAsync(h->in_x2.p, x2, sizeof(double) * 2 * n, hipMemcpyHostToDevice, s));
    HIPCHK(hipMemcpyAsync(h->in_d1.p, d1, sizeof(double) * n, hipMemcpyHostToDevice, s));
    HIPCHK(hipMemcpyAsync(h->in_d2.p, d2, sizeof(double) * n, hipMemcpyHostToDevice, s));
    HIPCHK(hipMemcpyAsync(h->unit_e.p, models, sizeof(Model) * count, hipMemcpyHostToDevice, s));
    hipLaunchKernelGGL(k_pack_unit, dim3((n + 255) / 256 + 1), dim3(256), 0, s, n, h->in_x1.as<double>(), h->in_x2.as<double>(),
                       h->in_d1.as<double>(), h->in_d2.as<double>(), h->pts.as<double>(), h->dep.as<double>());
    MDRP_LM_DISPATCH(k_refine_unit, (count >= 2048 ? 64 : 256), kind, (kind == MDRP_CALIB && estimate_shift), dim3(count), lm_list_bytes(n), s,
                     count, h->unit_e.as<Model>(), h->pts.as<double>(), h->dep.as<double>(), n, scale_reproj, weight_sampson, lm_opt(opt),
                     h->unit_a.as<double>(), lm_list_stride(n));
    HIPCHK(hipGetLastError());
    HIPCHK(hipMemcpyAsync(models, h->unit_e.p, sizeof(Model) * count, hipMemcpyDeviceToHost, s));
    if (final_cost) HIPCHK(hipMemcpyAsync(final_cost, h->unit_a.p, sizeof(double) * count, hipMemcpyDeviceToHost, s));
    HIPCHK(hipStreamSynchronize(s));
    return MDRP_OK;
}

}
```

### mdrp_amd/csrc/mdrp_kernels.h

```cpp
#pragma once
#include <hip/hip_runtime.h>
#include <float.h>
#include "mdrp_logtab.h"
#include "mdrp_math.h"

#ifdef MDRP_SECONDARY_TU
#define MDRP_GLOBAL static __global__
#else
#define MDRP_GLOBAL __global__
#endif

namespace mdrp {

constexpr int PT_STRIDE = 6;
#define MDRP_TILE_PTS 512
#define MDRP_SCORE_MINWAVES 4
constexpr int TILE_PTS = MDRP_TILE_PTS;
constexpr size_t SCORE_TILE_BYTES = (size_t)TILE_PTS * (PT_STRIDE * sizeof(double) + 4 * sizeof(float));
#define MDRP_P1F_UNROLL 8
#define MDRP_P1_UNROLL 4
constexpr int PRUNE_EVERY = 4;
#define MDRP_DENSE_KEY 40
#define MDRP_SOLVE_MINWAVES 2
#define MDRP_SCORE_THREADS 256
// ... 548 lines not shown
    const double C = fma(c, e0, fma(d, e1, e2));
    return C * C < thr_hi * dmax;
}

template <bool POSE, bool BOUND>
__device__ __forceinline__ void score_tile(const double *__restrict__ recs, int npts, const double E[9], const Model *__restrict__ mp,
                                           double thr, double thr_dmax, double &score, int &cnt, Prune &pr) {
    const double thr_hi = thr * (1.0 + 1e-12);
    for (int p0 = 0; p0 < npts; p0 += 32) {
        const int g = min(32, npts - p0);
        const double *base = recs + (size_t)p0 * PT_STRIDE;
        uint32_t mask = 0;
        if (g == 32) {
#pragma unroll 1
            for (int j0 = 0; j0 < 32; j0 += MDRP_P1_UNROLL) {
#pragma unroll
                for (int jj = 0; jj < MDRP_P1_UNROLL; ++jj) {
                    const int j = j0 + jj;
                    const double2 *P = reinterpret_cast<const double2 *>(base + j * PT_STRIDE);
                    const double2 p01 = P[0], p23 = P[1];
                    if (BOUND) {
                        mask |= sampson_maybe(E, p01.x, p01.y, p23.x, p23.y, thr_hi, thr_dmax) ? (1u << j) : 0u;
                    } else {
                        const SampsonTerms s = sampson_terms(E, p01.x, p01.y, p23.x, p23.y);
                        mask |= (s.C2 < thr_hi * s.den) ? (1u << j) : 0u;
                    }
                }
            }
        } else {
            for (int j = 0; j < g; ++j) {
                const double2 *P = reinterpret_cast<const double2 *>(base + j * PT_STRIDE);
                const double2 p01 = P[0], p23 = P[1];
                if (BOUND) {
                    mask |= sampson_maybe(E, p01.x, p01.y, p23.x, p23.y, thr_hi, thr_dmax) ? (1u << j) : 0u;
                } else {
                    const SampsonTerms s = sampson_terms(E, p01.x, p01.y, p23.x, p23.y);
                    mask |= (s.C2 < thr_hi * s.den) ? (1u << j) : 0u;
                }
            }
        }
        if (pr.dead) mask = 0;
        if (mask) {
            double R[9], t[3];
            if (POSE) {
                double q[4];
                q[0] = mp->q[0]; q[1] = mp->q[1]; q[2] = mp->q[2]; q[3] = mp->q[3];
                t[0] = mp->t[0]; t[1] = mp->t[1]; t[2] = mp->t[2];
                quat_to_R(q, R);
            }
            while (mask) {
                const int j = __ffs(mask) - 1;
                mask &= mask - 1;
                score_point<POSE>(base + j * PT_STRIDE, E, R, t, thr, score, cnt);
            }
        }
        pr.processed += g;
        if (pr.rec_score < DBL_MAX && ((p0 >> 5) & (PRUNE_EVERY - 1)) == PRUNE_EVERY - 1) {
            pr.dead = pr.dead || (((long long)cnt + (long long)(pr.n - pr.processed) <= pr.rec_cnt) &&
                                  (score + thr * (double)(pr.processed - cnt) >= pr.rec_score));
            if (__all(pr.dead)) { pr.wave_dead = true; return; }
        }
    }
}

typedef float f32x2 __attribute__((ext_vector_type(2)));
template <bool POSE>
__device__ __forceinline__ void score_tile_f32(const double *__restrict__ recs, const float4 *__restrict__ recs32, int npts,
                                               const double E[9], const float Ef[9], float tb, const Model *__restrict__ mp,
                                               double thr, double &score, int &cnt, Prune &pr) {
    constexpr int WIN = 64;
    static_assert(TILE_PTS % WIN == 0, "window must divide the tile");
    f32x2 Ev[9];
#pragma unroll
    for (int i = 0; i < 9; ++i) Ev[i] = (f32x2)(Ef[i]);
    for (int p0 = 0; p0 < npts; p0 += WIN) {
        const int g = min(WIN, npts - p0);
        const double *base = recs + (size_t)p0 * PT_STRIDE;
        uint32_t half[2] = {0, 0};
#pragma unroll
        for (int h = 0; h < 2; ++h) {
            const int q0 = 32 * h;
            if (q0 < g) {
                const float4 *b32 = recs32 + p0 + q0;
                uint32_t mask = 0;
#pragma unroll 1
                for (int j0 = 0; j0 < 32; j0 += MDRP_P1F_UNROLL) {
#pragma unroll
                    for (int jj = 0; jj < MDRP_P1F_UNROLL; jj += 2) {
                        const int j = j0 + jj;
                        const float4 ab = b32[j], cd = b32[j + 1];
                        const f32x2 a = {ab.x, ab.y}, b = {ab.z, ab.w}, c = {cd.x, cd.y}, d = {cd.z, cd.w};
                        const f32x2 e0 = __builtin_elementwise_fma(Ev[0], a, __builtin_elementwise_fma(Ev[1], b, Ev[2]));
                        const f32x2 e1 = __builtin_elementwise_fma(Ev[3], a, __builtin_elementwise_fma(Ev[4], b, Ev[5]));
                        const f32x2 e2 = __builtin_elementwise_fma(Ev[6], a, __builtin_elementwise_fma(Ev[7], b, Ev[8]));
                        const f32x2 C = __builtin_elementwise_fma(c, e0, __builtin_elementwise_fma(d, e1, e2));
                        const float cx = C.x, cy = C.y;
                        unsigned long long kx, ky, co;
                        asm("v_cmp_ngt_f32_e64 %0, |%1|, %2" : "=s"(kx) : "v"(cx), "v"(tb));
                        asm("v_cmp_ngt_f32_e64 %0, |%1|, %2" : "=s"(ky) : "v"(cy), "v"(tb));
                        asm("v_addc_co_u32_e64 %0, %1, %0, %0, %2" : "+v"(mask), "=s"(co) : "s"(kx));
                        asm("v_addc_co_u32_e64 %0, %1, %0, %0, %2" : "+v"(mask), "=s"(co) : "s"(ky));
                    }
                }
                mask = __brev(mask);
                const int valid = g - q0;
                if (valid < 32) mask &= (1u << valid) - 1u;
                half[h] = mask;
            }
        }
        uint64_t m = (uint64_t)half[0] | ((uint64_t)half[1] << 32);
        if (pr.dead) m = 0;
        if (m) {
            double R[9], t[3];
            if (POSE) {
                double q[4];
                q[0] = mp->q[0]; q[1] = mp->q[1]; q[2] = mp->q[2]; q[3] = mp->q[3];
                t[0] = mp->t[0]; t[1] = mp->t[1]; t[2] = mp->t[2];
                quat_to_R(q, R);
            }
            while (m) {
                const int j = __ffsll((unsigned long long)m) - 1;
                m &= m - 1;
                score_point<POSE>(base + j * PT_STRIDE, E, R, t, thr, score, cnt);
            }
        }
        pr.processed += g;
        if (pr.rec_score < DBL_MAX) {
            pr.dead = pr.dead || (((long long)cnt + (long long)(pr.n - pr.processed) <= pr.rec_cnt) &&
                                  (score + thr * (double)(pr.processed - cnt) >= pr.rec_score));
            if (__all(pr.dead)) { pr.wave_dead = true; return; }
        }
    }
}

__device__ __forceinline__ int plan_find(const int32_t *__restrict__ prefix, int batch, int w) {
    int lo = 0, hi = batch;
    while (hi - lo > 1) {
        const int mid = (lo + hi) >> 1;
        if (prefix[mid] <= w) lo = mid; else hi = mid;
    }
    return lo;
}

#define MDRP_CNT_TILES 8
constexpr int CNT_TILES = MDRP_CNT_TILES;
constexpr int CNT_ROUNDS = (16 * CNT_TILES) / 64;
static_assert(CNT_TILES == 4 || CNT_TILES == 8, "a wavefront owns 64 or 128 hypotheses");
constexpr int CNT_WAVE_MODELS = 16 * CNT_TILES;
constexpr int CNT_THREADS = 256;
constexpr int CNT_WG_MODELS = CNT_WAVE_MODELS * (CNT_THREADS / 64);
typedef __bf16 bf16x8_t __attribute__((ext_vector_type(8)));
typedef float f32x4_t __attribute__((ext_vector_type(4)));

constexpr int PLAN_THREADS = 1024;
__device__ __forceinline__ int plan_block_scan(int v, int &total, int *s_w) {
    const int lane = threadIdx.x & 63, wave = threadIdx.x >> 6;
    int inc = v;
#pragma unroll
    for (int o = 1; o < 64; o <<= 1) { const int u = __shfl_up(inc, o, 64); if (lane >= o) inc += u; }
    __syncthreads();
    if (lane == 63) s_w[wave] = inc;
    __syncthreads();
    if (wave == 0) {
        const int x = lane < PLAN_THREADS / 64 ? s_w[lane] : 0;
        int xi = x;
#pragma unroll
        for (int o = 1; o < PLAN_THREADS / 64; o <<= 1) { const int u = __shfl_up(xi, o, 64); if (lane >= o) xi += u; }
        if (lane < PLAN_THREADS / 64) s_w[lane] = xi - x;
        if (lane == PLAN_THREADS / 64 - 1) s_w[PLAN_THREADS / 64] = xi;
    }
    __syncthreads();
    total = s_w[PLAN_THREADS / 64];
    return inc - v + s_w[wave];
}
MDRP_GLOBAL __launch_bounds__(PLAN_THREADS) void k_count_plan(int batch, const PairState *__restrict__ st, const int32_t *__restrict__ counts, int stride,
                                                             int per_wg, int32_t *__restrict__ plan, int32_t *__restrict__ zero_a,
                                                             const int32_t *__restrict__ begin = nullptr, int32_t *__restrict__ zero_b2 = nullptr ) {
    __shared__ int s_w[PLAN_THREADS / 64 + 1];
    int run = 0;
    for (int p0 = 0; p0 < batch; p0 += PLAN_THREADS) {
        const int p = p0 + threadIdx.x;
        const int b = (p < batch && st[p].active) ? (counts[stride * p] - (begin ? begin[stride * p] : 0) + per_wg - 1) / per_wg : 0;
        int tot;
        const int ex = plan_block_scan(b, tot, s_w);
        if (p < batch) { plan[p] = run + ex; if (zero_a) zero_a[p] = 0; if (zero_b2) zero_b2[2 * p] = 0; }
        run += tot;
    }
    if (threadIdx.x == 0) plan[batch] = run;
}

__device__ __forceinline__ int count_split_tiles(const PairState &ps, int n_tiles, const unsigned long long *__restrict__ cand_stat, int pair) {
    if (!(ps.best_min_score < DBL_MAX) || n_tiles < 4 || !cand_stat) return n_tiles;
    const unsigned long long cs = cand_stat[2 * pair], es = cand_stat[2 * pair + 1];
    if (es == 0) return n_tiles;
    const double rec_score = ps.best_min_score * (1.0 + 1e-12);
    long long bar = (long long)floor((double)ps.n - rec_score / ps.sq_thr);
    if (bar > (long long)ps.best_min_cnt) bar = (long long)ps.best_min_cnt;
    if (bar <= 0) return n_tiles;
    const double g = fmin(0.5, 1.1 * (double)cs / (double)es + 0.005);
    const long long ra = (long long)((double)((long long)ps.n - bar) / (1.0 - g)) + 32;
    const int ta = (int)((ra + 255) >> 8);
    return ta + 2 > n_tiles ? n_tiles : ta;
}

template <bool POSE, bool RAWF = false>
__global__ __launch_bounds__(CNT_THREADS, 4) void k_count(RunParams rp, const PairState *__restrict__ st, const uint4 *__restrict__ rfrag,
                                                          const Model *__restrict__ models, const uint32_t *__restrict__ tags,
                                                          const int32_t *__restrict__ model_count, const int32_t *__restrict__ plan,
                                                          uint32_t *__restrict__ tags_surv,
                                                          int32_t *__restrict__ surv_count, unsigned long long *__restrict__ stats,
                                                          int32_t *__restrict__ cand_out ,
                                                          const int32_t *__restrict__ tag_begin = nullptr ,
                                                          int phase = 0, uint32_t *__restrict__ tags_und = nullptr, int32_t *__restrict__ und_part = nullptr,
                                                          int32_t *__restrict__ und_count = nullptr, const int32_t *__restrict__ part_in = nullptr,
                                                          unsigned long long *__restrict__ cand_stat = nullptr ) {
    constexpr int A_TILE_GROUPS = 16;
    __shared__ uint4 s_lds[2 * A_TILE_GROUPS * 64];
    uint4 (*s_frag)[CNT_WAVE_MODELS][4] = reinterpret_cast<uint4 (*)[CNT_WAVE_MODELS][4]>(s_lds);
    static_assert(sizeof(uint4) * (CNT_THREADS / 64) * CNT_WAVE_MODELS * 4 <= sizeof(uint4) * 2 * A_TILE_GROUPS * 64, "fragment staging fits the tile buffers");
    const int total = plan[rp.batch];
    const int w = blockIdx.x;
    if (w >= total) return;
    const int pair = plan_find(plan, rp.batch, w);
    const int blk = w - plan[pair];
    const PairState &ps = st[pair];
    const int tbeg = tag_begin ? tag_begin[2 * pair] : 0;
    const int n = ps.n, cnt = model_count[2 * pair] - tbeg;
    const int tid = threadIdx.x, lane = tid & 63, wave = tid >> 6;
    const int m0 = blk * CNT_WG_MODELS + wave * CNT_WAVE_MODELS;
    const size_t slot_base = (size_t)pair * rp.slot_stride;
    const uint32_t *tags_p = tags + slot_base + tbeg;
    const double thr = ps.sq_thr;
    uint32_t slot_r[CNT_ROUNDS] = {};
    int part_r[CNT_ROUNDS] = {};
    double mq[CNT_ROUNDS][4], mt[CNT_ROUNDS][3], mf[CNT_ROUNDS][2], ms[CNT_ROUNDS][2];
#pragma unroll
    for (int r = 0; r < CNT_ROUNDS; ++r) {
        const int i = m0 + 64 * r + lane;
        if (i < cnt) { slot_r[r] = tags_p[i] & 0xFFFFFFu; if (phase == 2) part_r[r] = part_in[slot_base + tbeg + i]; }
    }
#pragma unroll
    for (int r = 0; r < CNT_ROUNDS; ++r) {
        const Model *mp = models + slot_base + slot_r[r];
        const double2 *P = reinterpret_cast<const double2 *>(mp);
        const double2 q01 = P[0], q23 = P[1], t01 = P[2], t2s = P[3], f12 = P[5];
        mq[r][0] = q01.x; mq[r][1] = q01.y; mq[r][2] = q23.x; mq[r][3] = q23.y;
        mt[r][0] = t01.x; mt[r][1] = t01.y; mt[r][2] = t2s.x;
        mf[r][0] = f12.x; mf[r][1] = f12.y;
        ms[r][0] = t2s.y; ms[r][1] = RAWF ? P[4].x : 0.0;
    }
#pragma unroll
    for (int r = 0; r < CNT_ROUNDS; ++r) {
        const int i = m0 + 64 * r + lane;
        uint16_t eh[8], el[8], e8[3];
        float tb = 1.0f;
#pragma unroll
        for (int j = 0; j < 8; ++j) { eh[j] = 0; el[j] = 0; }
        e8[0] = e8[1] = e8[2] = 0;
        if (i < cnt) {
            double R[9], Em[9], E[9];
            if (RAWF) {
#pragma unroll
                for (int q = 0; q < 4; ++q) E[q] = mq[r][q];
                E[4] = mt[r][0]; E[5] = mt[r][1]; E[6] = mt[r][2]; E[7] = ms[r][0]; E[8] = ms[r][1];
            } else {
                quat_to_R(mq[r], R);
                essential_from_Rt(R, mt[r], Em);
                if (POSE) {
#pragma unroll
                    for (int q = 0; q < 9; ++q) E[q] = Em[q];
                } else fundamental_from_E(Em, mf[r][0], mf[r][1], E);
            }
            count_setup_scaled(E, ps.box, thr, eh, el, e8, tb);
        }
        uint4 *dst = s_frag[wave][64 * r + lane];
        dst[0] = pack_bf16x8(eh);
        dst[1] = pack_bf16x8(el);
        dst[2] = make_uint4((uint32_t)e8[0] | ((uint32_t)e8[1] << 16), (uint32_t)e8[2], 0u, 0u);
        dst[3] = make_uint4(__float_as_uint(tb), 0u, 0u, 0u);
    }
    __syncthreads();
    const bool idle = m0 >= cnt;
    const int col = lane & 15, ksl = lane >> 4;
    const int part = ksl < 2 ? 0 : ksl - 1;
    bf16x8_t bfrag[CNT_TILES];
    float tbv[CNT_TILES];
    float cand[CNT_TILES];
#pragma unroll
    for (int t = 0; t < CNT_TILES; ++t) {
        const uint4 *src = s_frag[wave][16 * t + col];
        bfrag[t] = __builtin_bit_cast(bf16x8_t, src[part]);
        const float tb2 = __uint_as_float(src[3].x);
        tbv[t] = tb2;
        cand[t] = 0.f;
    }
    __syncthreads();
    f32x4_t acc[CNT_TILES];
    auto mfma2 = [&](const uint4 &araw, int t0) {
        const bf16x8_t a = __builtin_bit_cast(bf16x8_t, araw);
        asm volatile("v_mfma_f32_16x16x32_bf16 %0, %2, %3, 0\n\t"
                     "v_mfma_f32_16x16x32_bf16 %1, %2, %4, 0"
                     : "=&v"(acc[t0]), "=&v"(acc[t0 + 1]) : "v"(a), "v"(bfrag[t0]), "v"(bfrag[t0 + 1]));
    };
    auto test2 = [&](int t0) {
        float d0, d1, d2, d3, d4, d5, d6, d7;
        asm volatile("v_fma_f32 %2, -%10, %10, %18 clamp\n\t"
                     "v_fma_f32 %3, -%11, %11, %18 clamp\n\t"
                     "v_fma_f32 %4, -%12, %12, %18 clamp\n\t"
                     "v_fma_f32 %5, -%13, %13, %18 clamp\n\t"
                     "v_fma_f32 %6, -%14, %14, %19 clamp\n\t"
                     "v_fma_f32 %7, -%15, %15, %19 clamp\n\t"
                     "v_fma_f32 %8, -%16, %16, %19 clamp\n\t"
                     "v_fma_f32 %9, -%17, %17, %19 clamp\n\t"
                     "v_add_f32 %2, %2, %3\n\t"
                     "v_add_f32 %4, %4, %5\n\t"
                     "v_add_f32 %6, %6, %7\n\t"
                     "v_add_f32 %8, %8, %9\n\t"
                     "v_add_f32 %0, %0, %2\n\t"
                     "v_add_f32 %1, %1, %6\n\t"
                     "v_add_f32 %0, %0, %4\n\t"
                     "v_add_f32 %1, %1, %8"
                     : "+v"(cand[t0]), "+v"(cand[t0 + 1]), "=&v"(d0), "=&v"(d1), "=&v"(d2), "=&v"(d3), "=&v"(d4), "=&v"(d5), "=&v"(d6), "=&v"(d7)
                     : "v"(acc[t0][0]), "v"(acc[t0][1]), "v"(acc[t0][2]), "v"(acc[t0][3]), "v"(acc[t0 + 1][0]), "v"(acc[t0 + 1][1]),
                       "v"(acc[t0 + 1][2]), "v"(acc[t0 + 1][3]), "v"(tbv[t0]), "v"(tbv[t0 + 1]));
    };
    const int G = (n + 15) >> 4;
    const uint4 *A = rfrag + (size_t)pair * ((rp.n_max + 15) >> 4) * 64;
    const int n_tiles = (G + A_TILE_GROUPS - 1) / A_TILE_GROUPS;
    const int t_split = phase == 0 ? n_tiles : count_split_tiles(ps, n_tiles, cand_stat, pair);
    const int t_lo = phase == 2 ? t_split : 0, t_hi = phase == 1 ? t_split : n_tiles;
    uint4 stage[4];
    auto fetch = [&](int tile) {
        const int g0 = tile * A_TILE_GROUPS;
#pragma unroll
        for (int k = 0; k < 4; ++k) {
            const int idx = k * CNT_THREADS + tid;
            stage[k] = (g0 + (idx >> 6)) < G ? A[(size_t)g0 * 64 + idx] : make_uint4(0u, 0u, 0u, 0u);
        }
    };
    auto commit = [&](int buf) {
#pragma unroll
        for (int k = 0; k < 4; ++k) s_lds[buf * A_TILE_GROUPS * 64 + k * CNT_THREADS + tid] = stage[k];
    };
    if (t_lo >= t_hi) return;
    fetch(t_lo);
    commit(t_lo & 1);
    __syncthreads();
    for (int tile = t_lo; tile < t_hi; ++tile) {
        const int buf = tile & 1;
        if (tile + 1 < t_hi) fetch(tile + 1);
        if (!idle) {
            const uint4 *T = s_lds + buf * A_TILE_GROUPS * 64 + lane;
            uint4 f0 = T[0], f1 = T[64];
#pragma unroll
            for (int t = 0; t < CNT_TILES; t += 2) mfma2(f0, t);
#pragma unroll
            for (int g = 0; g < A_TILE_GROUPS; g += 2) {
                f0 = T[(size_t)min(g + 2, A_TILE_GROUPS - 1) * 64];
#pragma unroll
                for (int t = 0; t < CNT_TILES; t += 2) { test2(t); mfma2(f1, t); }
                f1 = T[(size_t)min(g + 3, A_TILE_GROUPS - 1) * 64];
                if (g + 2 < A_TILE_GROUPS) {
#pragma unroll
                    for (int t = 0; t < CNT_TILES; t += 2) { test2(t); mfma2(f0, t); }
                } else {
#pragma unroll
                    for (int t = 0; t < CNT_TILES; t += 2) test2(t);
                }
            }
        }
        if (tile + 1 < t_hi) commit(buf ^ 1);
        __syncthreads();
    }
    if (idle) return;
    uint32_t *s_out = reinterpret_cast<uint32_t *>(&s_frag[wave][0][0]);
    const int swept = (t_hi - t_lo) * A_TILE_GROUPS * 16, real = min(max(n - t_lo * A_TILE_GROUPS * 16, 0), swept);
    const int pad = swept - real;
    const bool split_a = phase == 1 && t_hi < n_tiles;
    const int rest = split_a ? n - t_hi * A_TILE_GROUPS * 16 : 0;
#pragma unroll
    for (int t = 0; t < CNT_TILES; ++t) {
        float o = cand[t];
        o += __shfl_xor(o, 16, 64);
        o += __shfl_xor(o, 32, 64);
        if (ksl == 0) s_out[16 * t + col] = (uint32_t)((int)o - pad);
    }
    __builtin_amdgcn_fence(__ATOMIC_RELEASE, "wavefront");
    __builtin_amdgcn_wave_barrier();
    const long long rec_cnt = (long long)ps.best_min_cnt;
    const double rec_score = ps.best_min_score < DBL_MAX ? ps.best_min_score * (1.0 + 1e-12) : DBL_MAX;
#pragma unroll
    for (int r = 0; r < CNT_ROUNDS; ++r) {
        const int i = m0 + 64 * r + lane;
        const bool live = i < cnt;
        const int cnd_here = live ? (int)s_out[64 * r + lane] + part_r[r] : 0;
        const int cnd = cnd_here + rest;
        if (cand_stat && phase == 1 && !split_a && rec_cnt == 0 && !(ps.best_min_score < DBL_MAX)) {
            const int tot = wave_sum_i(cnd_here), lv = __popcll(__ballot(live));
            if (lane == 0 && lv) { atomicAdd(&cand_stat[2 * pair], (unsigned long long)tot); atomicAdd(&cand_stat[2 * pair + 1], (unsigned long long)lv * (unsigned long long)n); }
        }
        if (cand_out && live) cand_out[i] = cnd;
        const bool surv = live && ((long long)cnd > rec_cnt || thr * (double)(n - cnd) < rec_score);
        const unsigned long long ball = __ballot(surv);
        if (ball) {
            int base = 0;
            const int first = __ffsll((long long)ball) - 1;
            if (lane == first) base = atomicAdd(split_a ? &und_count[2 * pair] : &surv_count[pair], __popcll(ball));
            base = __shfl(base, first, 64);
            if (surv) {
                const size_t at = slot_base + base + __popcll(ball & ((1ull << lane) - 1ull));
                if (split_a) { tags_und[at] = slot_r[r]; und_part[at] = cnd_here; }
                else {
                    const uint32_t key = (uint32_t)min(PROBE_PTS, (int)(((long long)cnd * PROBE_PTS + n - 1) / n));
                    tags_surv[at] = slot_r[r] | (key << 24);
                }
            }
        }
    }
    if (stats && lane == 0 && wave == 0 && blk == 0) {
        if (phase != 2) atomicAdd(&stats[0], (unsigned long long)cnt * (unsigned long long)n);
        atomicAdd(&stats[1], (unsigned long long)(((cnt + 15) / 16) * 16) * (unsigned long long)swept);
    }
}

constexpr int BND_THREADS = 256;
#define MDRP_BND_TILE 256
constexpr int BND_TILE = MDRP_BND_TILE;

template <bool POSE, bool RAWF>
__device__ __forceinline__ void model_matrix(const Model &m, double E[9]) {
    if (RAWF) {
#pragma unroll
        for (int q = 0; q < 9; ++q) E[q] = reinterpret_cast<const double *>(&m)[q];
    } else {
        double R[9], Em[9];
        quat_to_R(m.q, R);
        essential_from_Rt(R, m.t, Em);
        if (POSE) {
#pragma unroll
            for (int q = 0; q < 9; ++q) E[q] = Em[q];
        } else fundamental_from_E(Em, m.f1, m.f2, E);
    }
}

template <bool POSE, bool RAWF = false>
__global__ __launch_bounds__(BND_THREADS, 4) void k_bound(RunParams rp, const PairState *__restrict__ st, const double *__restrict__ pts,
                                                          const Model *__restrict__ models, const uint32_t *__restrict__ tags_in,
                                                          const int32_t *__restrict__ cnt_in, const int32_t *__restrict__ plan,
                                                          uint32_t *__restrict__ tags_out,
                                                          int32_t *__restrict__ cnt_out, unsigned long long *__restrict__ stats,
                                                          double *__restrict__ dbg_lb = nullptr ,
                                                          int32_t *__restrict__ dbg_cnt_ub = nullptr) {
    __shared__ float4 s_rec[BND_TILE];
    struct Open { uint32_t tag; int32_t sane; float Ef[9], eC, eD, thr_dn, c0, c1; double lb; };
    __shared__ Open s_open[BND_THREADS];
    __shared__ int s_wave_open[BND_THREADS / 64];
    const int total = plan[rp.batch];
    const int w = blockIdx.x;
    if (w >= total) return;
    const int pair = plan_find(plan, rp.batch, w);
    const int blk = w - plan[pair];
    const PairState &ps = st[pair];
    const int n = ps.n, cnt = cnt_in[pair];
    const int tid = threadIdx.x, lane = tid & 63, wave = tid >> 6;
    const int i = blk * BND_THREADS + tid;
    bool open = i < cnt;
    const size_t slot_base = (size_t)pair * rp.slot_stride;
    const double thr = ps.sq_thr;
    uint32_t tag = 0;
    float Ef[9], eC = 0.f, eD = 1.f, thr_dn = 0.f;
    bool sane = false;
#pragma unroll
    for (int q = 0; q < 9; ++q) Ef[q] = 0.f;
    if (open) {
        tag = tags_in[slot_base + i];
        const Model m = models[slot_base + (tag & 0xFFFFFFu)];
        double E[9];
        model_matrix<POSE, RAWF>(m, E);
        sane = bound_setup32(E, ps.box, thr, Ef, eC, eD, thr_dn);
    }
    double total_lb = 0.0;
    f32x2 cnt2 = {0.f, 0.f};
    const float thr_cnt = (float)(thr * (1.0 + 1e-5)) * (1.0f + 1e-6f);
    const float BIG = 1.2089258e24f;
    const f32x2 nbig = {-BIG, -BIG}, kcnt = {thr_cnt * BIG, thr_cnt * BIG};
    const long long rec_cnt = (long long)ps.best_min_cnt;
    const double rec_score = ps.best_min_score < DBL_MAX ? ps.best_min_score * (1.0 + 1e-12) : DBL_MAX;
    float4 *s_pair = s_rec;
    const double *gp = pts + (size_t)pair * rp.n_max * PT_STRIDE;
    for (int t0 = 0; t0 < n; t0 += BND_TILE) {
        const int npts = min(BND_TILE, n - t0);
        __syncthreads();
        for (int j = tid; j < npts; j += BND_THREADS) {
            const double2 *src = reinterpret_cast<const double2 *>(gp + (size_t)(t0 + j) * PT_STRIDE);
            const double2 p0 = src[0], p1 = src[1];
            store_rec32(s_pair, j, p0.x, p0.y, p1.x, p1.y);
        }
        __syncthreads();
        if (__ballot(open)) {
            f32x2 Ev[9];
#pragma unroll
            for (int q = 0; q < 9; ++q) Ev[q] = (f32x2){Ef[q], Ef[q]};
            const f32x2 eDv = {eD, eD};
            const int npairs = npts >> 1;
            for (int j0 = 0; j0 < npairs; j0 += 32) {
                const int je = min(32, npairs - j0);
                f32x2 part = {0.f, 0.f};
#pragma unroll 2
                for (int j = 0; j < je; ++j) {
                    const float4 ab = s_pair[2 * (j0 + j)], cd = s_pair[2 * (j0 + j) + 1];
                    const f32x2 a = {ab.x, ab.y}, b = {ab.z, ab.w}, c = {cd.x, cd.y}, d = {cd.z, cd.w};
                    const f32x2 e0 = __builtin_elementwise_fma(Ev[0], a, __builtin_elementwise_fma(Ev[1], b, Ev[2]));
                    const f32x2 e1 = __builtin_elementwise_fma(Ev[3], a, __builtin_elementwise_fma(Ev[4], b, Ev[5]));
                    const f32x2 e2 = __builtin_elementwise_fma(Ev[6], a, __builtin_elementwise_fma(Ev[7], b, Ev[8]));
                    const f32x2 g0 = __builtin_elementwise_fma(Ev[0], c, __builtin_elementwise_fma(Ev[3], d, Ev[6]));
                    const f32x2 g1 = __builtin_elementwise_fma(Ev[1], c, __builtin_elementwise_fma(Ev[4], d, Ev[7]));
                    const f32x2 C = __builtin_elementwise_fma(c, e0, __builtin_elementwise_fma(d, e1, e2));
                    const f32x2 den = __builtin_elementwise_fma(e0, e0, __builtin_elementwise_fma(e1, e1, __builtin_elementwise_fma(g0, g0, __builtin_elementwise_fma(g1, g1, eDv))));
                    const f32x2 t = {fmaxf(fabsf(C.x) - eC, 0.0f), fmaxf(fabsf(C.y) - eC, 0.0f)};
                    const f32x2 rc = {__builtin_amdgcn_rcpf(den.x), __builtin_amdgcn_rcpf(den.y)};
                    const f32x2 q = (t * t) * rc;
                    const f32x2 term = {__builtin_fminf(q.x, thr_dn), __builtin_fminf(q.y, thr_dn)};
                    part += term;
                    f32x2 o;
                    asm("v_pk_fma_f32 %0, %1, %2, %3 clamp" : "=v"(o) : "v"(q), "v"(nbig), "v"(kcnt));
                    cnt2 += o;
                }
                total_lb += (double)part.x + (double)part.y;
            }
            if (npts & 1) {
                const float *fl = reinterpret_cast<const float *>(s_pair) + (npts >> 1) * 8;
                const float q = bound_r2_32(Ef, eC, eD, fl[0], fl[2], fl[4], fl[6]);
                total_lb += (double)__builtin_fminf(q, thr_dn);
                cnt2.x += (q < thr_cnt) ? 1.0f : 0.0f;
            }
        }
        const int seen = t0 + npts;
        if (open && sane) {
            const long long cnt_ub = (long long)(cnt2.x + cnt2.y) + 1 + (long long)(n - seen);
            if (cnt_ub <= rec_cnt && total_lb * (1.0 - BOUND_SLACK) >= rec_score) open = false;
        }
        if (seen >= n) break;
        const unsigned long long ob = __ballot(open);
        if (lane == 0) s_wave_open[wave] = __popcll(ob);
        __syncthreads();
        int tot = 0, before = 0, waves_used = 0;
#pragma unroll
        for (int v = 0; v < BND_THREADS / 64; ++v) { const int c = s_wave_open[v]; if (v < wave) before += c; tot += c; waves_used += c > 0; }
        if (tot == 0) break;
        if ((tot + 63) / 64 < waves_used) {
            if (open) {
                Open &o = s_open[before + __popcll(ob & ((1ull << lane) - 1ull))];
                o.tag = tag; o.sane = sane; o.eC = eC; o.eD = eD; o.thr_dn = thr_dn; o.c0 = cnt2.x; o.c1 = cnt2.y; o.lb = total_lb;
#pragma unroll
                for (int q = 0; q < 9; ++q) o.Ef[q] = Ef[q];
            }
            __syncthreads();
            open = tid < tot;
            if (open) {
                const Open &o = s_open[tid];
                tag = o.tag; sane = o.sane != 0; eC = o.eC; eD = o.eD; thr_dn = o.thr_dn; cnt2.x = o.c0; cnt2.y = o.c1; total_lb = o.lb;
#pragma unroll
                for (int q = 0; q < 9; ++q) Ef[q] = o.Ef[q];
            }
        }
    }
    const bool surv = open;
    if (dbg_lb && surv) {
        dbg_lb[tag & 0xFFFFFFu] = sane ? total_lb * (1.0 - BOUND_SLACK) : 0.0;
        dbg_cnt_ub[tag & 0xFFFFFFu] = sane ? (int32_t)min((long long)n, (long long)(cnt2.x + cnt2.y) + 1) : n;
    }
    const unsigned long long ball = __ballot(surv);
    if (ball) {
        int base = 0;
        const int first = __ffsll((long long)ball) - 1;
        if (lane == first) base = atomicAdd(&cnt_out[pair], __popcll(ball));
        base = __shfl(base, first, 64);
        if (surv) tags_out[slot_base + base + __popcll(ball & ((1ull << lane) - 1ull))] = tag;
    }
    if (stats && tid == 0 && blk == 0) atomicAdd(stats, (unsigned long long)cnt * (unsigned long long)n);
}

MDRP_GLOBAL __launch_bounds__(256) void k_sort_tags(RunParams rp, const PairState *__restrict__ st, int32_t *__restrict__ model_count,
                                                   const int32_t *__restrict__ surv_count,
                                                   const uint32_t *__restrict__ tags, uint32_t *__restrict__ tags_sorted) {
    const int pair = blockIdx.x, tid = threadIdx.x;
    const PairState &ps = st[pair];
    if (!ps.active) return;
    __shared__ int s_hist[PROBE_PTS + 1], s_pos[PROBE_PTS + 1];
    __shared__ int s_dense;
    if (tid <= PROBE_PTS) s_hist[tid] = 0;
    if (tid == 0) s_dense = 0;
    __syncthreads();
    const int cnt = surv_count[pair];
    const size_t slot_base = (size_t)pair * rp.slot_stride;
    const uint32_t *src = tags + slot_base;
    uint32_t *dst = tags_sorted + slot_base;
    const int dense_min = ps.n >= 8 ? MDRP_DENSE_KEY : PROBE_PTS + 1;
    for (int i = tid; i < cnt; i += 256) atomicAdd(&s_hist[min(src[i] >> 24, (uint32_t)PROBE_PTS)], 1);
    __syncthreads();
    if (tid < 64) {
        const int v = tid < dense_min ? s_hist[tid] : 0;
        int incl = v;
#pragma unroll
        for (int o = 1; o < 64; o <<= 1) {
            const int u = __shfl_up(incl, o, 64);
            if (tid >= o) incl += u;
        }
        s_pos[tid] = incl - v;
        if (tid == 63) s_pos[64] = incl;
    }
    __syncthreads();
    const int cap = rp.slot_stride;
    for (int i = tid; i < cnt; i += 256) {
        const uint32_t t = src[i];
        const int key = (int)min(t >> 24, (uint32_t)PROBE_PTS);
        if (key >= dense_min) dst[cap - 1 - atomicAdd(&s_dense, 1)] = t & 0xFFFFFFu;
        else dst[atomicAdd(&s_pos[key], 1)] = t & 0xFFFFFFu;
    }
    __syncthreads();
    if (tid == 0) { model_count[2 * pair] = cnt - s_dense; model_count[2 * pair + 1] = s_dense; }
}

MDRP_GLOBAL __launch_bounds__(PLAN_THREADS) void k_plan(int batch, const int32_t *__restrict__ model_count, int32_t *__restrict__ plan,
                                                       int32_t *__restrict__ totals , int per_wg) {
    __shared__ int s_w[PLAN_THREADS / 64 + 1];
    int run_d = 0, run_s = 0;
    int32_t *pd = plan, *psp = plan + batch + 1;
    for (int p0 = 0; p0 < batch; p0 += PLAN_THREADS) {
        const int p = p0 + threadIdx.x;
        int bd = 0, bs = 0;
        if (p < batch) {
            bs = (model_count[2 * p] + per_wg - 1) / per_wg;
            bd = (model_count[2 * p + 1] + per_wg - 1) / per_wg;
        }
        int tot_d, tot_s;
        const int ed = plan_block_scan(bd, tot_d, s_w), es = plan_block_scan(bs, tot_s, s_w);
        if (p < batch) { pd[p] = run_d + run_s + ed + es; psp[p] = bs; }
        run_d += tot_d;
        run_s += tot_s;
    }
    if (threadIdx.x == 0) { pd[batch] = run_d + run_s; psp[batch] = 0; totals[0] = run_d; totals[1] = run_d + run_s; totals[2] = 0; }
}

template <bool POSE, bool RAWF = false>
__global__ __launch_bounds__(SCORE_THREADS, MDRP_SCORE_MINWAVES) void k_score(RunParams rp, const PairState *__restrict__ st, const double *__restrict__ pts,
                                                         const Model *__restrict__ models, const uint32_t *__restrict__ tags,
                                                         const int32_t *__restrict__ model_count, double *__restrict__ slot_score,
                                                         int32_t *__restrict__ slot_inl, const int32_t *__restrict__ plan,
                                                         int32_t *__restrict__ totals) {
    extern __shared__ double tile[];
    float4 *tile32 = reinterpret_cast<float4 *>(tile + TILE_PTS * PT_STRIDE);
    const int total = totals[1];
    const int tid = threadIdx.x;
    for (int w = blockIdx.x; w < total; w += gridDim.x) {
    const int pair = plan_find(plan, rp.batch, w);
    const int blk_sparse = plan[rp.batch + 1 + pair];
    const int bi = w - plan[pair];
    const bool dense = bi >= blk_sparse;
    const int blk = dense ? bi - blk_sparse : bi;
    const int cnt_sparse = model_count[2 * pair], cnt_dense = model_count[2 * pair + 1];
    const PairState &ps = st[pair];
    const int n = ps.n;
    const double thr = ps.sq_thr;
    const size_t slot_base = (size_t)pair * rp.slot_stride;
    const int cap = rp.slot_stride;
    bool live;
    uint32_t slot = 0;
    {
        const int i = blk * SCORE_THREADS + tid;
        live = i < (dense ? cnt_dense : cnt_sparse);
        if (live) slot = tags[slot_base + (dense ? cap - 1 - i : i)];
    }
    double E[9], thr_dmax;
    float tb, Ef[9];
    const Model *mp = models + slot_base + slot;
#pragma unroll
    for (int i = 0; i < 9; ++i) E[i] = 0;
    if (live) {
        const Model m = *mp;
        double R[9], Em[9];
        if (RAWF) {
#pragma unroll
            for (int i = 0; i < 9; ++i) E[i] = reinterpret_cast<const double *>(&m)[i];
        } else {
            quat_to_R(m.q, R);
            essential_from_Rt(R, m.t, Em);
            if (POSE) {
#pragma unroll
                for (int i = 0; i < 9; ++i) E[i] = Em[i];
            } else {
                fundamental_from_E(Em, m.f1, m.f2, E);
            }
        }
    }
    bound_setup(E, ps, thr, Ef, tb, thr_dmax);
    double score = 0;
    int cnt = 0;
    Prune pr;
    pr.rec_cnt = (long long)ps.best_min_cnt;
    pr.rec_score = ps.best_min_score < DBL_MAX ? ps.best_min_score * (1.0 + 1e-12) : DBL_MAX;
    pr.n = n; pr.processed = 0; pr.dead = !live; pr.wave_dead = false;
    const double *gp = pts + (size_t)pair * rp.n_max * PT_STRIDE;
    for (int t0 = 0; t0 < n; t0 += TILE_PTS) {
        const int npts = min(TILE_PTS, n - t0);
        __syncthreads();
        {
            const double2 *src = reinterpret_cast<const double2 *>(gp + (size_t)t0 * PT_STRIDE);
            double2 *dst = reinterpret_cast<double2 *>(tile);
            for (int i = tid; i < npts; i += SCORE_THREADS) {
                const double2 p0 = src[3 * i], p1 = src[3 * i + 1], p2 = src[3 * i + 2];
                dst[3 * i] = p0; dst[3 * i + 1] = p1; dst[3 * i + 2] = p2;
                if (!dense) store_rec32(tile32, i, p0.x, p0.y, p1.x, p1.y);
            }
        }
        __syncthreads();
        if (!pr.wave_dead) {
            if (dense) score_tile_dense<POSE>(tile, npts, E, mp, thr, score, cnt, pr);
            else score_tile_f32<POSE>(tile, tile32, npts, E, Ef, tb, mp, thr, score, cnt, pr);
        }
    }
    if (live) {
        const bool pruned = pr.dead;
        slot_score[slot_base + slot] = pruned ? DBL_MAX : score + thr * (double)(n - cnt);
        slot_inl[slot_base + slot] = pruned ? -2 : cnt;
    }
    }
}

constexpr int SCORE_WAVE_MAX_PAIRS = 128;
constexpr int SCW_THREADS = 256;
template <bool POSE, bool RAWF = false>
__global__ __launch_bounds__(SCW_THREADS) void k_score_w(RunParams rp, const PairState *__restrict__ st, const double *__restrict__ pts,
                                                         const Model *__restrict__ models, const uint32_t *__restrict__ tags ,
                                                         const int32_t *__restrict__ model_count, double *__restrict__ slot_score,
                                                         int32_t *__restrict__ slot_inl, const int32_t *__restrict__ plan ) {
    __shared__ double s_r2[SCW_THREADS / 64][64];
    const int total = plan[rp.batch];
    const int lane = threadIdx.x & 63, wave = threadIdx.x >> 6;
    const unsigned long long lt = (1ull << lane) - 1ull;
    for (int w = blockIdx.x; w < total; w += gridDim.x) {
        const int pair = plan_find(plan, rp.batch, w);
        const int i = (w - plan[pair]) * (SCW_THREADS / 64) + wave;
        const int cnt_sparse = model_count[2 * pair], cnt_dense = model_count[2 * pair + 1];
        if (i >= cnt_sparse + cnt_dense) continue;
        const PairState &ps = st[pair];
        const int n = ps.n;
        const double thr = ps.sq_thr;
        const size_t slot_base = (size_t)pair * rp.slot_stride;
        const uint32_t slot = tags[slot_base + (i < cnt_sparse ? i : rp.slot_stride - 1 - (i - cnt_sparse))];
        const Model m = models[slot_base + slot];
        double E[9], R[9], t[3] = {m.t[0], m.t[1], m.t[2]};
#pragma unroll
        for (int q = 0; q < 9; ++q) R[q] = 0;
        if (RAWF) {
#pragma unroll
            for (int q = 0; q < 9; ++q) E[q] = reinterpret_cast<const double *>(&m)[q];
        } else {
            double Em[9];
            quat_to_R(m.q, R);
            essential_from_Rt(R, m.t, Em);
            if (POSE) {
#pragma unroll
                for (int q = 0; q < 9; ++q) E[q] = Em[q];
            } else fundamental_from_E(Em, m.f1, m.f2, E);
        }
        const long long rec_cnt = (long long)ps.best_min_cnt;
        const double rec_score = ps.best_min_score < DBL_MAX ? ps.best_min_score * (1.0 + 1e-12) : DBL_MAX;
        const double *gp = pts + (size_t)pair * rp.n_max * PT_STRIDE;
        double score = 0;
        int cnt = 0;
        bool pruned = false;
        for (int t0 = 0; t0 < n; t0 += 64) {
            const int r = t0 + lane;
            double s1 = 0;
            int c1 = 0;
            if (r < n) score_point<POSE>(gp + (size_t)r * PT_STRIDE, E, R, t, thr, s1, c1);
            const unsigned long long ball = __ballot(c1 != 0);
            if (ball) {
                if (c1) s_r2[wave][__popcll(ball & lt)] = s1;
                __builtin_amdgcn_fence(__ATOMIC_RELEASE, "wavefront");
                __builtin_amdgcn_wave_barrier();
                __builtin_amdgcn_fence(__ATOMIC_ACQUIRE, "wavefront");
                const int k = __popcll(ball);
                for (int j = 0; j < k; ++j) score += s_r2[wave][j];
                cnt += k;
                __builtin_amdgcn_wave_barrier();
            }
            const int processed = min(t0 + 64, n);
            if (rec_score < DBL_MAX && ((processed & 127) == 0 || processed == n) &&
                (long long)cnt + (long long)(n - processed) <= rec_cnt && score + thr * (double)(processed - cnt) >= rec_score) { pruned = true; break; }
        }
        if (lane == 0) {
            slot_score[slot_base + slot] = pruned ? DBL_MAX : score + thr * (double)(n - cnt);
            slot_inl[slot_base + slot] = pruned ? -2 : cnt;
        }
    }
}

constexpr int SPLIT_THREADS = 256;
constexpr int SPLIT_WAVES = SPLIT_THREADS / 64;
constexpr int SPLIT_HYP = 64;
constexpr int SPLIT_Q = 8;
constexpr int SPLIT_STEP = SPLIT_WAVES * SPLIT_Q;
static_assert(128 % SPLIT_STEP == 0, "the bail-out positions (every 128 records) must be step boundaries");
template <bool POSE, bool RAWF = false>
__global__ __launch_bounds__(SPLIT_THREADS, MDRP_SCORE_MINWAVES) void k_score_split(RunParams rp, const PairState *__restrict__ st, const double *__restrict__ pts,
                                                               const Model *__restrict__ models, const uint32_t *__restrict__ tags ,
                                                               const int32_t *__restrict__ model_count, double *__restrict__ slot_score,
                                                               int32_t *__restrict__ slot_inl, const int32_t *__restrict__ plan ,
                                                               const int32_t *__restrict__ totals) {
    __shared__ double s_rec[2][SPLIT_WAVES][SPLIT_Q * PT_STRIDE];
    __shared__ float4 s_rec32[2][SPLIT_WAVES][SPLIT_Q];
    __shared__ double s_r2[2][SPLIT_STEP][SPLIT_HYP];
    __shared__ int32_t s_cnt[2][SPLIT_WAVES][SPLIT_HYP];
    __shared__ unsigned long long s_dead[2];
    const int total = totals[1];
    const int lane = threadIdx.x & 63;
    const int wave = __builtin_amdgcn_readfirstlane(threadIdx.x >> 6);
    for (int w = blockIdx.x; w < total; w += gridDim.x) {
        const int pair = plan_find(plan, rp.batch, w);
        const int blk_sparse = plan[rp.batch + 1 + pair];
        const int bi = w - plan[pair];
        const bool dense = bi >= blk_sparse;
        const int blk = dense ? bi - blk_sparse : bi;
        const int cnt_sparse = model_count[2 * pair], cnt_dense = model_count[2 * pair + 1];
        const PairState &ps = st[pair];
        const int n = ps.n;
        const double thr = ps.sq_thr;
        const size_t slot_base = (size_t)pair * rp.slot_stride;
        const int i = blk * SPLIT_HYP + lane;
        const bool live = i < (dense ? cnt_dense : cnt_sparse);
        uint32_t slot = 0;
        if (live) slot = tags[slot_base + (dense ? rp.slot_stride - 1 - i : i)];
        double E[9], R[9], t[3] = {0, 0, 0};
#pragma unroll
        for (int q = 0; q < 9; ++q) { E[q] = 0; R[q] = 0; }
        if (live) {
            const Model m = models[slot_base + slot];
            if (RAWF) {
#pragma unroll
                for (int q = 0; q < 9; ++q) E[q] = reinterpret_cast<const double *>(&m)[q];
            } else {
                double Em[9];
                quat_to_R(m.q, R);
                essential_from_Rt(R, m.t, Em);
                t[0] = m.t[0]; t[1] = m.t[1]; t[2] = m.t[2];
                if (POSE) {
#pragma unroll
                    for (int q = 0; q < 9; ++q) E[q] = Em[q];
                } else fundamental_from_E(Em, m.f1, m.f2, E);
            }
        }
        double thr_dmax;
        float Ef[9], tb;
        bound_setup(E, ps, thr, Ef, tb, thr_dmax);
        const long long rec_cnt = (long long)ps.best_min_cnt;
        const double rec_score = ps.best_min_score < DBL_MAX ? ps.best_min_score * (1.0 + 1e-12) : DBL_MAX;
        const double *gp = pts + (size_t)pair * rp.n_max * PT_STRIDE;
        const int steps = (n + SPLIT_STEP - 1) / SPLIT_STEP;
        double2 nx = {0, 0};
        auto fetch = [&](int j) {
            const int r = j * SPLIT_STEP + wave * SPLIT_Q + lane / 3;
            if (lane < 3 * SPLIT_Q && r < n) nx = reinterpret_cast<const double2 *>(gp + (size_t)r * PT_STRIDE)[lane % 3];
        };
        auto stage = [&](int j) {
            const int k = lane / 3, part = lane % 3;
            if (lane < 3 * SPLIT_Q && j * SPLIT_STEP + wave * SPLIT_Q + k < n) {
                reinterpret_cast<double2 *>(s_rec[j & 1][wave])[lane] = nx;
                float *q = reinterpret_cast<float *>(s_rec32[j & 1][wave]) + (k >> 1) * 8 + (k & 1);
                if (part == 0) { q[0] = (float)nx.x; q[2] = (float)nx.y; }
                else if (part == 1) { q[4] = (float)nx.x; q[6] = (float)nx.y; }
            }
        };
        fetch(0);
        stage(0);
        __syncthreads();
        double score = 0;
        int cnt = 0;
        bool dead = !live;
        bool skip = !live;
        for (int j = 0; j <= steps; ++j) {
            if (j > 0) {
                const unsigned long long dm = s_dead[(j - 1) & 1];
                if (dm == ~0ull) break;
                skip = (dm >> lane) & 1;
            }
            if (wave == 0) {
                if (j > 0) {
                    const int b = (j - 1) & 1;
                    if (!dead) {
#pragma unroll 1
                        for (int q = 0; q < SPLIT_WAVES; ++q) {
#pragma unroll
                            for (int r = 0; r < SPLIT_Q; ++r) score += s_r2[b][q * SPLIT_Q + r][lane];
                            cnt += s_cnt[b][q][lane];
                        }
                    }
                    const int processed = min(j * SPLIT_STEP, n);
                    if (rec_score < DBL_MAX && ((processed & 127) == 0 || processed == n))
                        dead = dead || (((long long)cnt + (long long)(n - processed) <= rec_cnt) &&
                                        (score + thr * (double)(processed - cnt) >= rec_score));
                }
                if (j < steps) {
                    const unsigned long long dm = __ballot(dead);
                    if (lane == 0) s_dead[j & 1] = dm;
                }
                skip = dead;
            }
            if (j == steps) break;
            if (j + 1 < steps) fetch(j + 1);
            const int b = j & 1;
            const int valid = min(SPLIT_Q, n - (j * SPLIT_STEP + wave * SPLIT_Q));
            const double *rec = s_rec[b][wave];
            double *out = &s_r2[b][wave * SPLIT_Q][lane];
            int found = 0;
            if (dense) {
#pragma unroll 2
                for (int jj = 0; jj < SPLIT_Q; ++jj) {
                    double v = 0.0, r2;
                    if (jj < valid && !skip && record_inlier<POSE>(rec + jj * PT_STRIDE, E, R, t, thr, r2)) { v = r2; ++found; }
                    out[jj * SPLIT_HYP] = v;
                }
            } else {
#pragma unroll
                for (int jj = 0; jj < SPLIT_Q; ++jj) out[jj * SPLIT_HYP] = 0.0;
                const float4 *b32 = s_rec32[b][wave];
                f32x2 Ev[9];
#pragma unroll
                for (int q = 0; q < 9; ++q) Ev[q] = (f32x2)(Ef[q]);
                uint32_t mask = 0;
#pragma unroll
                for (int jj = 0; jj < SPLIT_Q; jj += 2) {
                    const float4 ab = b32[jj], cd = b32[jj + 1];
                    const f32x2 a = {ab.x, ab.y}, bb = {ab.z, ab.w}, c = {cd.x, cd.y}, d = {cd.z, cd.w};
                    const f32x2 e0 = __builtin_elementwise_fma(Ev[0], a, __builtin_elementwise_fma(Ev[1], bb, Ev[2]));
                    const f32x2 e1 = __builtin_elementwise_fma(Ev[3], a, __builtin_elementwise_fma(Ev[4], bb, Ev[5]));
                    const f32x2 e2 = __builtin_elementwise_fma(Ev[6], a, __builtin_elementwise_fma(Ev[7], bb, Ev[8]));
                    const f32x2 C = __builtin_elementwise_fma(c, e0, __builtin_elementwise_fma(d, e1, e2));
                    mask |= (!(fabsf(C.x) > tb) ? 1u : 0u) << jj;
                    mask |= (!(fabsf(C.y) > tb) ? 1u : 0u) << (jj + 1);
                }
                mask &= valid >= SPLIT_Q ? 0xFFu : (valid > 0 ? (1u << valid) - 1u : 0u);
                if (skip) mask = 0;
                while (mask) {
                    const int jj = __ffs(mask) - 1;
                    mask &= mask - 1;
                    double r2;
                    if (record_inlier<POSE>(rec + jj * PT_STRIDE, E, R, t, thr, r2)) { out[jj * SPLIT_HYP] = r2; ++found; }
                }
            }
            s_cnt[b][wave][lane] = found;
            if (j + 1 < steps) stage(j + 1);
            __syncthreads();
        }
        if (wave == 0 && live) {
            slot_score[slot_base + slot] = dead ? DBL_MAX : score + thr * (double)(n - cnt);
            slot_inl[slot_base + slot] = dead ? -2 : cnt;
        }
    }
}

template <int MPS = 4, int IPL = 1>
__global__ __launch_bounds__(64) void k_scan(RunParams rp, PairState *__restrict__ st, const double *__restrict__ slot_score,
                                             const int32_t *__restrict__ slot_inl, Trigger *__restrict__ triggers,
                                             int trig_cap, const int32_t *__restrict__ model_count,
                                             unsigned long long *__restrict__ evals) {
    const int pair = blockIdx.x, lane = threadIdx.x;
    PairState &ps = st[pair];
    if (!ps.active) { if (lane == 0) ps.n_triggers = 0; return; }
    if (lane == 0 && evals) atomicAdd(evals, (unsigned long long)(model_count[2 * pair] + model_count[2 * pair + 1]) * (unsigned long long)ps.n);
    long long run_cnt = (long long)ps.best_min_cnt;
    double run_score = ps.best_min_score;
    const double nan_score = (double)ps.n * ps.sq_thr;
    int ntrig = rp.chunk_off > 0 ? ps.n_triggers : 0;
    static_assert(MPS % 4 == 0, "slots of an iteration are read as 16-byte groups");
    constexpr int NG = MPS / 4;
    const size_t slot_base = (size_t)pair * rp.slot_stride + (size_t)rp.chunk_off * MPS;
    struct Slots { int4 c[IPL][NG]; double2 s01[IPL][NG], s23[IPL][NG]; };
    auto fetch = [&](int it0) {
        Slots r;
#pragma unroll
        for (int j = 0; j < IPL; ++j) {
            const int it = it0 + IPL * lane + j;
#pragma unroll
            for (int g = 0; g < NG; ++g) {
                if (it < rp.chunk_len) {
                    r.c[j][g] = *reinterpret_cast<const int4 *>(slot_inl + slot_base + (size_t)it * MPS + 4 * g);
                    const double2 *sp = reinterpret_cast<const double2 *>(slot_score + slot_base + (size_t)it * MPS + 4 * g);
                    r.s01[j][g] = sp[0]; r.s23[j][g] = sp[1];
                } else { r.c[j][g] = make_int4(-1, -1, -1, -1); r.s01[j][g] = r.s23[j][g] = make_double2(DBL_MAX, DBL_MAX); }
            }
        }
        return r;
    };
    Slots nxt = fetch(0);
    for (int it0 = 0; it0 < rp.chunk_len; it0 += 64 * IPL) {
        const Slots cur = nxt;
        if (it0 + 64 * IPL < rp.chunk_len) nxt = fetch(it0 + 64 * IPL);
        int c[IPL][MPS];
        double s[IPL][MPS];
        long long lc = -1;
        double ls = DBL_MAX;
#pragma unroll
        for (int j = 0; j < IPL; ++j) {
#pragma unroll
            for (int g = 0; g < NG; ++g) {
                c[j][4 * g] = cur.c[j][g].x; c[j][4 * g + 1] = cur.c[j][g].y; c[j][4 * g + 2] = cur.c[j][g].z; c[j][4 * g + 3] = cur.c[j][g].w;
                s[j][4 * g] = c[j][4 * g] >= 0 ? cur.s01[j][g].x : DBL_MAX; s[j][4 * g + 1] = c[j][4 * g + 1] >= 0 ? cur.s01[j][g].y : DBL_MAX;
                s[j][4 * g + 2] = c[j][4 * g + 2] >= 0 ? cur.s23[j][g].x : DBL_MAX; s[j][4 * g + 3] = c[j][4 * g + 3] >= 0 ? cur.s23[j][g].y : DBL_MAX;
            }
            if (c[j][0] == -3) { c[j][0] = 0; s[j][0] = nan_score; }
#pragma unroll
            for (int k = 0; k < MPS; ++k) if (c[j][k] >= 0) { lc = max(lc, (long long)c[j][k]); ls = fmin(ls, s[j][k]); }
        }
        if (__all(lc <= run_cnt && !(ls < run_score))) continue;
        long long pc = lc;
        double psn = ls;
#pragma unroll
        for (int o = 1; o < 64; o <<= 1) {
            const long long vc = __shfl_up(pc, o, 64);
            const double vs = __shfl_up(psn, o, 64);
            if (lane >= o) { pc = max(pc, vc); psn = fmin(psn, vs); }
        }
        const long long tot_c = __shfl(pc, 63, 64);
        const double tot_s = __shfl(psn, 63, 64);
        long long ec = __shfl_up(pc, 1, 64);
        double es = __shfl_up(psn, 1, 64);
        if (lane == 0) { ec = -1; es = DBL_MAX; }
        long long bc = max(run_cnt, ec);
        double bs = fmin(run_score, es);
        int k_ref[IPL], k_min[IPL], cnt_min[IPL], cnt_ref[IPL], mine = 0;
        double score_min[IPL];
#pragma unroll
        for (int j = 0; j < IPL; ++j) {
            k_ref[j] = -1; k_min[j] = -1; cnt_min[j] = 0; cnt_ref[j] = 0; score_min[j] = 0;
#pragma unroll
            for (int k = 0; k < MPS; ++k) {
                if (c[j][k] >= 0) {
                    const bool more = (long long)c[j][k] > bc, better = s[j][k] < bs;
                    if (more || better) {
                        if (more) bc = c[j][k];
                        if (better) { bs = s[j][k]; k_min[j] = k; score_min[j] = s[j][k]; cnt_min[j] = c[j][k]; }
                        k_ref[j] = k; cnt_ref[j] = c[j][k];
                    }
                }
            }
            mine += k_ref[j] >= 0;
        }
        int before = mine;
#pragma unroll
        for (int o = 1; o < 64; o <<= 1) { const int v = __shfl_up(before, o, 64); if (lane >= o) before += v; }
        const int step_total = __shfl(before, 63, 64);
        int pos = ntrig + before - mine;
#pragma unroll
// ... 809 lines not shown
```

Baseline: 130,100.

## Record per-segment non-candidate counts in count pass to tighten bound and score pruning

The candidate-counting kernel now snapshots per-hypothesis prefix counts at up to eight boundaries across the point set, using cross-lane permlane reductions into LDS, and stores how many remaining points are provably non-candidates. The bound and split-score kernels read this row and credit those points as guaranteed outliers. That tightens the inlier-count upper bound and the score lower bound, so hypotheses can be marked dead earlier and more scoring work is skipped. The cost is extra LDS, reductions and a 16-byte global write per model in the count kernel, plus an extra load in the consumers. Debug APIs for row inspection and an open-hypothesis histogram are also added.

```diff
diff --git a/include/mdrp.h b/include/mdrp.h
--- a/include/mdrp.h
+++ b/include/mdrp.h
@@ -109,6 +109,12 @@
 int mdrp_count_candidates(mdrp_handle *h, int kind, const mdrp_model *models, int num_models, const double *x1,
                           const double *x2, int n, double sq_threshold, int32_t *candidates);
 
+int mdrp_count_candidate_rows(mdrp_handle *h, int kind, const mdrp_model *models, int num_models, const double *x1,
+                              const double *x2, int n, double sq_threshold, int32_t *candidates, uint16_t *rows,
+                              int32_t *row_step);
+
+int mdrp_debug_bound_open(mdrp_handle *h, uint64_t *open_after_tile, int tiles);
+
 int mdrp_bound_models(mdrp_handle *h, int kind, const mdrp_model *models, int num_models, const double *x1, const double *x2,
                       int n, double sq_threshold, double *score_lb, int32_t *count_ub);
 
diff --git a/mdrp_amd/_capi.py b/mdrp_amd/_capi.py
--- a/mdrp_amd/_capi.py
+++ b/mdrp_amd/_capi.py
@@ -15,7 +15,7 @@
 EXPORTS = (
     "mdrp_create_", "mdrp_create_on_stream_", "mdrp_destroy", "mdrp_last_error", "mdrp_version", "mdrp_abi_version", "mdrp_hip_build_version", "mdrp_synchronize", "mdrp_estimate_batch",
     "mdrp_estimate_batch_async", "mdrp_fetch_results", "mdrp_copy_results_device", "mdrp_solver_batch", "mdrp_score_models", "mdrp_count_candidates", "mdrp_bound_models", "mdrp_refine_models",
-    "mdrp_last_sweep_stats", "mdrp_last_stats", "mdrp_last_stats_sized", "mdrp_classic_solver_batch",
+    "mdrp_last_sweep_stats", "mdrp_last_stats", "mdrp_last_stats_sized", "mdrp_classic_solver_batch", "mdrp_count_candidate_rows", "mdrp_debug_bound_open",
 )
 
 
@@ -105,6 +105,8 @@
         lib.mdrp_score_models.argtypes = [vp, C.c_int, C.c_int, vp, C.c_int, dp, dp, C.c_int, C.c_double, vp, vp]
         lib.mdrp_count_candidates.argtypes = [vp, C.c_int, vp, C.c_int, dp, dp, C.c_int, C.c_double, vp]
         lib.mdrp_bound_models.argtypes = [vp, C.c_int, vp, C.c_int, dp, dp, C.c_int, C.c_double, vp, vp]
+        lib.mdrp_count_candidate_rows.argtypes = [vp, C.c_int, vp, C.c_int, dp, dp, C.c_int, C.c_double, vp, vp, vp]
+        lib.mdrp_debug_bound_open.argtypes = [vp, vp, C.c_int]
         lib.mdrp_refine_models.argtypes = [vp, C.c_int, vp, C.c_int, dp, dp, dp, dp, C.c_int, C.c_double, C.c_double,
                                            C.POINTER(BundleOpt), C.c_int, vp]
         lib.mdrp_last_sweep_stats.argtypes = [vp, C.POINTER(C.c_double), C.POINTER(C.c_int64), C.POINTER(C.c_int64)]
@@ -350,6 +352,22 @@
                                                           float(sq_threshold), _ptr(cand)))
         return cand
 
+    def count_candidate_rows(self, kind, models, x1, x2, sq_threshold):
+        models = np.ascontiguousarray(models, dtype=MODEL_DTYPE).reshape(-1)
+        x1 = np.ascontiguousarray(x1, dtype=np.float64)
+        x2 = np.ascontiguousarray(x2, dtype=np.float64)
+        cand = np.zeros(len(models), dtype=np.int32)
+        rows = np.zeros((len(models), 8), dtype=np.uint16)
+        step = C.c_int32(0)
+        _check(self._lib, self._lib.mdrp_count_candidate_rows(self._h, int(kind), _ptr(models), len(models), _ptr(x1), _ptr(x2), len(x1),
+                                                              float(sq_threshold), _ptr(cand), _ptr(rows), C.addressof(step)))
+        return cand, rows, int(step.value)
+
+    def bound_open_counts(self, tiles=64):
+        out = np.zeros(int(tiles), dtype=np.uint64)
+        _check(self._lib, self._lib.mdrp_debug_bound_open(self._h, _ptr(out), int(tiles)))
+        return out
+
     def bound_models(self, kind, models, x1, x2, sq_threshold):
         models = np.ascontiguousarray(models, dtype=MODEL_DTYPE).reshape(-1)
         x1 = np.ascontiguousarray(x1, dtype=np.float64)
diff --git a/mdrp_amd/csrc/mdrp_capi.hip b/mdrp_amd/csrc/mdrp_capi.hip
--- a/mdrp_amd/csrc/mdrp_capi.hip
+++ b/mdrp_amd/csrc/mdrp_capi.hip
@@ -142,6 +142,8 @@
     DevBuf rfrag;
     DevBuf cplan;
     DevBuf surv2_count;
+    DevBuf cand_rows;
+    DevBuf bound_open;
     DevBuf lo_mask;
     DevBuf red5;
     DevBuf lm_stats;
@@ -301,7 +303,7 @@
         {&h->tags[0], tags}, {&h->model_count[0], pair2}, {&h->model_count[1], pair2}, {&h->tags[1], tags}, {&h->tags_sorted[0], tags},
         {&h->tags_sorted[1], tags}, {&h->samples[1], samples}, {&h->tags_v, tags},
         {&h->surv_count, sizeof(int32_t) * b}, {&h->cand_stat, sizeof(unsigned long long) * 2 * b}, {&h->und_count, pair2},
-        {&h->cplan, sizeof(int32_t) * (b + 1)}, {&h->surv2_count, sizeof(int32_t) * b},
+        {&h->cplan, sizeof(int32_t) * (b + 1)}, {&h->surv2_count, sizeof(int32_t) * b}, {&h->cand_rows, sizeof(uint4) * slots},
         {&h->rfrag, std::max<size_t>(1024, b * ((n + 15) / 16) * 1024)},
         {&h->triggers, sizeof(Trigger) * b * chunk_cap},
         {&h->work_pair, sizeof(int32_t) * (3 * b + 2)},
@@ -313,6 +315,7 @@
 }
 
 struct HostSrc { const double *x1, *x2, *d1, *d2; };
+constexpr int BOUND_HIST_TILES = 64;
 constexpr int HOST_SLICE_PAIRS = 256;
 
 int run_pass(mdrp_handle *h, int kind, const double *x1, const double *x2, const double *d1, const double *d2, int batch,
@@ -419,6 +422,13 @@
     const bool lo_overlap = env_int("MDRP_LO_OVERLAP", 1) != 0;
     const bool use_bound = env_int("MDRP_BOUND", 1) != 0;
     const bool score_split = env_int("MDRP_SCORE_SPLIT", 1) != 0;
+    const bool tile_bounds = env_int("MDRP_TILE_BOUNDS", 1) != 0 && batch_call > 16 && n_max <= ROW_N_MAX;
+    const int row_shift = cand_row_shift(n_max);
+    unsigned long long *bound_open = nullptr;
+    if (env_int("MDRP_BOUND_HIST", 0) != 0) {
+        if (!h->bound_open.p) { if ((rc = h->bound_open.ensure(sizeof(unsigned long long) * BOUND_HIST_TILES))) return rc; HIPCHK(hipMemsetAsync(h->bound_open.p, 0, sizeof(unsigned long long) * BOUND_HIST_TILES, s)); }
+        if ((n_max + BND_TILE - 1) / BND_TILE <= BOUND_HIST_TILES) bound_open = h->bound_open.as<unsigned long long>();
+    }
     const int lo_threads = env_int("MDRP_LO_THREADS", (batch_call >= 128 && n_max < 4096) ? 64 : 256);
     const int final_threads = env_int("MDRP_FINAL_THREADS", batch_call >= 4096 ? 64 : 256);
     const int mask_index = lm_mask_index_on(n_max);
@@ -551,6 +561,7 @@
             hipEvent_t e0, e1;
             int rc_;
             if ((rc_ = get_events(h, &e0, &e1, 0))) return rc_;
+            uint4 *rows_c = (tile_bounds && !(it0 == 0 && c == 0)) ? h->cand_rows.as<uint4>() + so : nullptr;
             unsigned long long *cstats = &cnt->progress.evals;
             {
                 hipEvent_t c0, c1;
@@ -566,13 +577,13 @@
                 HIPCHK(hipEventRecord(c0, s));
                 MDRP_SWEEP_DISPATCH(k_count, kind, cgrid, dim3(CNT_THREADS), 0, s, r, st_p, rfrag_p, models_p,
                                     tags_c, mcount_c, h->cplan.as<int32_t>(), tags_v, surv1, cstats, (int32_t *)nullptr, (const int32_t *)nullptr,
-                                    1, tags_u, und_part, und_cnt, (const int32_t *)nullptr, cand_stat);
+                                    1, tags_u, und_part, und_cnt, (const int32_t *)nullptr, cand_stat, rows_c, row_shift);
                 if (two_phase) {
                     hipLaunchKernelGGL(k_count_plan, dim3(1), dim3(PLAN_THREADS), 0, s, pc, st_p, und_cnt, 2, CNT_WG_MODELS, h->cplan.as<int32_t>(),
                                        (int32_t *)nullptr, (const int32_t *)nullptr, (int32_t *)nullptr);
                     MDRP_SWEEP_DISPATCH(k_count, kind, cgrid, dim3(CNT_THREADS), 0, s, r, st_p, rfrag_p, models_p,
                                         tags_u, und_cnt, h->cplan.as<int32_t>(), tags_v, surv1, cstats, (int32_t *)nullptr, (const int32_t *)nullptr,
-                                        2, (uint32_t *)nullptr, (int32_t *)nullptr, (int32_t *)nullptr, und_part, cand_stat);
+                                        2, (uint32_t *)nullptr, (int32_t *)nullptr, (int32_t *)nullptr, und_part, cand_stat, rows_c, row_shift);
                     h->count_launches++;
                 }
                 HIPCHK(hipEventRecord(c1, s));
@@ -587,7 +598,8 @@
                 hipEvent_t b0, b1;
                 if ((rc_ = get_events(h, &b0, &b1, 4))) return rc_;
                 HIPCHK(hipEventRecord(b0, s));
-                MDRP_SWEEP_DISPATCH(k_bound, kind, bgrid, dim3(BND_THREADS), 0, s, r, st_p, pts_p, models_p, tags_v, surv1, h->cplan.as<int32_t>(), tags_c, surv2, bstats);
+                MDRP_SWEEP_DISPATCH(k_bound, kind, bgrid, dim3(BND_THREADS), 0, s, r, st_p, pts_p, models_p, tags_v, surv1, h->cplan.as<int32_t>(), tags_c, surv2, bstats,
+                                    (double *)nullptr, (int32_t *)nullptr, rows_c, row_shift, bound_open);
                 HIPCHK(hipEventRecord(b1, s));
                 surv_tags = tags_c; surv_cnt = surv2;
             }
@@ -607,7 +619,8 @@
                 const long long ub = (long long)pc * ((len * mps + SPLIT_HYP - 1) / SPLIT_HYP + 1);
                 const dim3 grid((unsigned)std::min<long long>(ub, (long long)h->num_cu * 32));
                 MDRP_SWEEP_DISPATCH(k_score_split, kind, grid, dim3(SPLIT_THREADS), 0, s, r, st_p, pts_p, models_p, tags_sc, mcount_c,
-                                    h->slot_score.as<double>() + so, h->slot_inl.as<int32_t>() + so, plan, totals);
+                                    h->slot_score.as<double>() + so, h->slot_inl.as<int32_t>() + so, plan, totals,
+                                    rows_c, row_shift);
             } else {
                 hipLaunchKernelGGL(k_sort_tags, dim3(pc), dim3(256), 0, s, r, st_p, mcount_c, surv_cnt, surv_tags, tags_sc);
                 hipLaunchKernelGGL(k_plan, dim3(1), dim3(PLAN_THREADS), 0, s, pc, mcount_c, plan, totals, SCORE_THREADS);
@@ -1163,8 +1176,8 @@
     return finish_timing(h);
 }
 
-int mdrp_count_candidates(mdrp_handle *h, int kind, const mdrp_model *models, int num_models, const double *x1, const double *x2,
-                          int n, double sq_threshold, int32_t *candidates) {
+static int count_candidates_impl(mdrp_handle *h, int kind, const mdrp_model *models, int num_models, const double *x1, const double *x2,
+                                 int n, double sq_threshold, int32_t *candidates, uint16_t *rows_out, int32_t *row_step_out) {
     if (!h || num_models < 0 || n < 0 || kind < 0 || kind > 5 || !candidates || !models) { g_err = "invalid argument"; return MDRP_ERR_INVALID; }
     if (num_models == 0) return MDRP_OK;
     MDRP_ENTER(h);
@@ -1178,7 +1191,7 @@
         (rc = h->model_count[0].ensure(2 * sizeof(int32_t))) || (rc = h->surv_count.ensure(sizeof(int32_t))) ||
         (rc = h->cplan.ensure(2 * sizeof(int32_t))) || (rc = h->rfrag.ensure((size_t)((nn + 15) / 16) * 1024)) ||
         (rc = h->unit_f.ensure(sizeof(int32_t) * slots)) || (rc = h->in_x1.ensure(sizeof(double) * 2 * nn)) ||
-        (rc = h->in_x2.ensure(sizeof(double) * 2 * nn)))
+        (rc = h->in_x2.ensure(sizeof(double) * 2 * nn)) || (rows_out && (rc = h->cand_rows.ensure(sizeof(uint4) * slots))))
         return rc;
     HIPCHK(hipMemcpyAsync(h->in_x1.p, x1, sizeof(double) * 2 * n, hipMemcpyHostToDevice, s));
     HIPCHK(hipMemcpyAsync(h->in_x2.p, x2, sizeof(double) * 2 * n, hipMemcpyHostToDevice, s));
@@ -1195,12 +1208,41 @@
     hipLaunchKernelGGL(k_count_plan, dim3(1), dim3(PLAN_THREADS), 0, s, 1, h->st.as<PairState>(), h->model_count[0].as<int32_t>(), 2, CNT_WG_MODELS, h->cplan.as<int32_t>(),
                        (int32_t *)nullptr);
     const dim3 grid((unsigned)((num_models + CNT_WG_MODELS - 1) / CNT_WG_MODELS));
+    uint4 *rows = (rows_out && nn <= ROW_N_MAX) ? h->cand_rows.as<uint4>() : nullptr;
+    const int row_shift = cand_row_shift(nn);
+    if (rows_out) { HIPCHK(hipMemsetAsync(h->cand_rows.p, 0, sizeof(uint4) * slots, s)); *row_step_out = 1 << row_shift; }
     MDRP_SWEEP_DISPATCH(k_count, kind, grid, dim3(CNT_THREADS), 0, s, rp, h->st.as<PairState>(), h->rfrag.as<uint4>(), h->models.as<Model>(),
                         h->tags[0].as<uint32_t>(), h->model_count[0].as<int32_t>(), h->cplan.as<int32_t>(),
-                        h->tags_v.as<uint32_t>(), h->surv_count.as<int32_t>(), (unsigned long long *)nullptr, h->unit_f.as<int32_t>());
+                        h->tags_v.as<uint32_t>(), h->surv_count.as<int32_t>(), (unsigned long long *)nullptr, h->unit_f.as<int32_t>(),
+                        (const int32_t *)nullptr, 0, (uint32_t *)nullptr, (int32_t *)nullptr, (int32_t *)nullptr, (const int32_t *)nullptr, (unsigned long long *)nullptr,
+                        rows, row_shift);
     HIPCHK(hipGetLastError());
+    if (rows_out) HIPCHK(hipMemcpyAsync(rows_out, h->cand_rows.p, sizeof(uint4) * num_models, hipMemcpyDeviceToHost, s));
     HIPCHK(hipMemcpyAsync(candidates, h->unit_f.p, sizeof(int32_t) * num_models, hipMemcpyDeviceToHost, s));
     HIPCHK(hipStreamSynchronize(s));
+    return MDRP_OK;
+}
+
+int mdrp_count_candidates(mdrp_handle *h, int kind, const mdrp_model *models, int num_models, const double *x1, const double *x2,
+                          int n, double sq_threshold, int32_t *candidates) {
+    return count_candidates_impl(h, kind, models, num_models, x1, x2, n, sq_threshold, candidates, nullptr, nullptr);
+}
+
+int mdrp_count_candidate_rows(mdrp_handle *h, int kind, const mdrp_model *models, int num_models, const double *x1, const double *x2,
+                              int n, double sq_threshold, int32_t *candidates, uint16_t *rows, int32_t *row_step) {
+    if (!rows || !row_step) { g_err = "invalid argument"; return MDRP_ERR_INVALID; }
+    return count_candidates_impl(h, kind, models, num_models, x1, x2, n, sq_threshold, candidates, rows, row_step);
+}
+
+int mdrp_debug_bound_open(mdrp_handle *h, uint64_t *open_after_tile, int tiles) {
+    if (!h || !open_after_tile || tiles < 0) { g_err = "invalid argument"; return MDRP_ERR_INVALID; }
+    MDRP_ENTER(h);
+    const int m = std::min(tiles, BOUND_HIST_TILES);
+    std::memset(open_after_tile, 0, sizeof(uint64_t) * tiles);
+    if (!h->bound_open.p || m == 0) return MDRP_OK;
+    HIPCHK(hipStreamSynchronize(h->stream));
+    HIPCHK(hipMemcpy(open_after_tile, h->bound_open.p, sizeof(uint64_t) * m, hipMemcpyDeviceToHost));
+    HIPCHK(hipMemset(h->bound_open.p, 0, sizeof(unsigned long long) * BOUND_HIST_TILES));
     return MDRP_OK;
 }
 
diff --git a/mdrp_amd/csrc/mdrp_kernels.h b/mdrp_amd/csrc/mdrp_kernels.h
--- a/mdrp_amd/csrc/mdrp_kernels.h
+++ b/mdrp_amd/csrc/mdrp_kernels.h
@@ -724,6 +724,23 @@
 typedef __bf16 bf16x8_t __attribute__((ext_vector_type(8)));
 typedef float f32x4_t __attribute__((ext_vector_type(4)));
 
+constexpr int ROW_BOUNDS = 8;
+constexpr int ROW_N_MAX = 65280;
+__host__ __device__ inline int cand_row_shift(int n_max) { const int tiles = (n_max + 255) >> 8; int sh = 0; while ((ROW_BOUNDS << sh) < tiles) ++sh; return sh; }
+__device__ __forceinline__ int cand_row_credit(const uint4 *__restrict__ rows, size_t slot, int row_shift, int seen, int n) {
+    if (!rows || seen >= n) return 0;
+    const int j = (((seen >> 8) + (1 << row_shift) - 1) >> row_shift) - 1;
+    if (j < 0 || j >= ROW_BOUNDS) return 0;
+    return (int)reinterpret_cast<const uint16_t *>(rows + slot)[j];
+}
+__device__ __forceinline__ int cand_row_credit(const uint4 &row, int row_shift, int processed, int n) {
+    if (processed >= n) return 0;
+    const int j = (((processed + 255) >> 8) + (1 << row_shift) - 1 >> row_shift) - 1;
+    if (j < 0 || j >= ROW_BOUNDS) return 0;
+    const uint32_t w = j < 2 ? row.x : j < 4 ? row.y : j < 6 ? row.z : row.w;
+    return (int)((j & 1) ? w >> 16 : w & 0xFFFFu);
+}
+
 constexpr int PLAN_THREADS = 1024;
 __device__ __forceinline__ int plan_block_scan(int v, int &total, int *s_w) {
     const int lane = threadIdx.x & 63, wave = threadIdx.x >> 6;
@@ -785,11 +802,14 @@
                                                           const int32_t *__restrict__ tag_begin = nullptr ,
                                                           int phase = 0, uint32_t *__restrict__ tags_und = nullptr, int32_t *__restrict__ und_part = nullptr,
                                                           int32_t *__restrict__ und_count = nullptr, const int32_t *__restrict__ part_in = nullptr,
-                                                          unsigned long long *__restrict__ cand_stat = nullptr ) {
+                                                          unsigned long long *__restrict__ cand_stat = nullptr ,
+                                                          uint4 *__restrict__ rows = nullptr ,
+                                                          int row_shift = 0 ) {
     constexpr int A_TILE_GROUPS = 16;
     __shared__ uint4 s_lds[2 * A_TILE_GROUPS * 64];
     uint4 (*s_frag)[CNT_WAVE_MODELS][4] = reinterpret_cast<uint4 (*)[CNT_WAVE_MODELS][4]>(s_lds);
     static_assert(sizeof(uint4) * (CNT_THREADS / 64) * CNT_WAVE_MODELS * 4 <= sizeof(uint4) * 2 * A_TILE_GROUPS * 64, "fragment staging fits the tile buffers");
+    __shared__ __attribute__((aligned(16))) uint16_t s_snap[CNT_THREADS / 64][ROW_BOUNDS][CNT_WAVE_MODELS];
     const int total = plan[rp.batch];
     const int w = blockIdx.x;
     if (w >= total) return;
@@ -804,12 +824,11 @@
     const uint32_t *tags_p = tags + slot_base + tbeg;
     const double thr = ps.sq_thr;
     uint32_t slot_r[CNT_ROUNDS] = {};
-    int part_r[CNT_ROUNDS] = {};
     double mq[CNT_ROUNDS][4], mt[CNT_ROUNDS][3], mf[CNT_ROUNDS][2], ms[CNT_ROUNDS][2];
 #pragma unroll
     for (int r = 0; r < CNT_ROUNDS; ++r) {
         const int i = m0 + 64 * r + lane;
-        if (i < cnt) { slot_r[r] = tags_p[i] & 0xFFFFFFu; if (phase == 2) part_r[r] = part_in[slot_base + tbeg + i]; }
+        if (i < cnt) slot_r[r] = tags_p[i] & 0xFFFFFFu;
     }
 #pragma unroll
     for (int r = 0; r < CNT_ROUNDS; ++r) {
@@ -918,9 +937,12 @@
     fetch(t_lo);
     commit(t_lo & 1);
     __syncthreads();
+    const int wave_s = __builtin_amdgcn_readfirstlane(wave);
     for (int tile = t_lo; tile < t_hi; ++tile) {
         const int buf = tile & 1;
         if (tile + 1 < t_hi) fetch(tile + 1);
+        const int snap_j = ((tile + 1) >> row_shift) - 1;
+        const bool snap_now = rows && ((tile + 1) & ((1 << row_shift) - 1)) == 0 && snap_j < ROW_BOUNDS;
         if (!idle) {
             const uint4 *T = s_lds + buf * A_TILE_GROUPS * 64 + lane;
             uint4 f0 = T[0], f1 = T[64];
@@ -940,11 +962,34 @@
                     for (int t = 0; t < CNT_TILES; t += 2) test2(t);
                 }
             }
+            if (snap_now) {
+                static_assert(CNT_TILES == 8, "eight uint16 per lane and boundary: one 16-byte write");
+                uint32_t sum[CNT_TILES / 2];
+#pragma unroll
+                for (int t = 0; t < CNT_TILES; t += 2) {
+                    uint32_t a = (uint32_t)(int)cand[t] | ((uint32_t)(int)cand[t + 1] << 16), b = a;
+                    asm volatile("s_nop 1\n\tv_permlane16_swap_b32 %0, %1" : "+v"(a), "+v"(b));
+                    a += b;
+                    b = a;
+                    asm volatile("s_nop 1\n\tv_permlane32_swap_b32 %0, %1" : "+v"(a), "+v"(b));
+                    sum[t / 2] = a + b;
+                }
+                int ln;
+                asm volatile("v_mbcnt_lo_u32_b32 %0, -1, 0\n\tv_mbcnt_hi_u32_b32 %0, -1, %0" : "=v"(ln));
+                if (ln < 16)
+                    *reinterpret_cast<uint4 *>(&s_snap[wave_s][snap_j][ln * CNT_TILES]) =
+                        make_uint4(sum[0], sum[1], sum[2], sum[3]);
+            }
         }
         if (tile + 1 < t_hi) commit(buf ^ 1);
         __syncthreads();
     }
     if (idle) return;
+    int part_r[CNT_ROUNDS] = {};
+    if (phase == 2) {
+#pragma unroll
+        for (int r = 0; r < CNT_ROUNDS; ++r) { const int i = m0 + 64 * r + lane; if (i < cnt) part_r[r] = part_in[slot_base + tbeg + i]; }
+    }
     uint32_t *s_out = reinterpret_cast<uint32_t *>(&s_frag[wave][0][0]);
     const int swept = (t_hi - t_lo) * A_TILE_GROUPS * 16, real = min(max(n - t_lo * A_TILE_GROUPS * 16, 0), swept);
     const int pad = swept - real;
@@ -986,6 +1031,21 @@
                     const uint32_t key = (uint32_t)min(PROBE_PTS, (int)(((long long)cnd * PROBE_PTS + n - 1) / n));
                     tags_surv[at] = slot_r[r] | (key << 24);
                 }
+                if (rows) {
+                    const int lo = t_lo * A_TILE_GROUPS * 16, hi = t_hi * A_TILE_GROUPS * 16;
+                    const int nc_here = real - (int)s_out[64 * r + lane];
+                    uint4 *rowp = rows + slot_base + slot_r[r];
+                    uint32_t e[ROW_BOUNDS] = {};
+                    if (phase == 2) { const uint4 a = *rowp; e[0] = a.x & 0xFFFFu; e[1] = a.x >> 16; e[2] = a.y & 0xFFFFu; e[3] = a.y >> 16; e[4] = a.z & 0xFFFFu; e[5] = a.z >> 16; e[6] = a.w & 0xFFFFu; e[7] = a.w >> 16; }
+#pragma unroll
+                    for (int j = 0; j < ROW_BOUNDS; ++j) {
+                        const int pos = ((j + 1) << row_shift) * A_TILE_GROUPS * 16;
+                        if (pos >= n || pos > hi) e[j] = 0u;
+                        else if (pos <= lo) e[j] += (uint32_t)nc_here;
+                        else e[j] = (uint32_t)(nc_here - ((pos - lo) - (int)s_snap[wave][j][(lane & 15) * CNT_TILES + 4 * r + (lane >> 4)]));
+                    }
+                    *rowp = make_uint4(e[0] | (e[1] << 16), e[2] | (e[3] << 16), e[4] | (e[5] << 16), e[6] | (e[7] << 16));
+                }
             }
         }
     }
@@ -1022,7 +1082,9 @@
                                                           uint32_t *__restrict__ tags_out,
                                                           int32_t *__restrict__ cnt_out, unsigned long long *__restrict__ stats,
                                                           double *__restrict__ dbg_lb = nullptr ,
-                                                          int32_t *__restrict__ dbg_cnt_ub = nullptr) {
+                                                          int32_t *__restrict__ dbg_cnt_ub = nullptr,
+                                                          const uint4 *__restrict__ rows = nullptr ,
+                                                          int row_shift = 0, unsigned long long *__restrict__ open_hist = nullptr ) {
     __shared__ float4 s_rec[BND_TILE];
     struct Open { uint32_t tag; int32_t sane; float Ef[9], eC, eD, thr_dn, c0, c1; double lb; };
     __shared__ Open s_open[BND_THREADS];
@@ -1109,9 +1171,11 @@
         }
         const int seen = t0 + npts;
         if (open && sane) {
-            const long long cnt_ub = (long long)(cnt2.x + cnt2.y) + 1 + (long long)(n - seen);
-            if (cnt_ub <= rec_cnt && total_lb * (1.0 - BOUND_SLACK) >= rec_score) open = false;
-        }
+            const int nc = cand_row_credit(rows, slot_base + (tag & 0xFFFFFFu), row_shift, seen, n);
+            const long long cnt_ub = (long long)(cnt2.x + cnt2.y) + 1 + (long long)(n - seen - nc);
+            if (cnt_ub <= rec_cnt && (total_lb + (double)thr_dn * (double)nc) * (1.0 - BOUND_SLACK) >= rec_score) open = false;
+        }
+        if (open_hist) { const int no = __popcll(__ballot(open)); if (lane == 0 && no) atomicAdd(&open_hist[t0 / BND_TILE], (unsigned long long)no); }
         if (seen >= n) break;
         const unsigned long long ob = __ballot(open);
         if (lane == 0) s_wave_open[wave] = __popcll(ob);
@@ -1381,7 +1445,8 @@
                                                                const Model *__restrict__ models, const uint32_t *__restrict__ tags ,
                                                                const int32_t *__restrict__ model_count, double *__restrict__ slot_score,
                                                                int32_t *__restrict__ slot_inl, const int32_t *__restrict__ plan ,
-                                                               const int32_t *__restrict__ totals) {
+                                                               const int32_t *__restrict__ totals,
+                                                               const uint4 *__restrict__ rows = nullptr , int row_shift = 0) {
     __shared__ double s_rec[2][SPLIT_WAVES][SPLIT_Q * PT_STRIDE];
     __shared__ float4 s_rec32[2][SPLIT_WAVES][SPLIT_Q];
     __shared__ double s_r2[2][SPLIT_STEP][SPLIT_HYP];
@@ -1405,6 +1470,8 @@
         const bool live = i < (dense ? cnt_dense : cnt_sparse);
         uint32_t slot = 0;
         if (live) slot = tags[slot_base + (dense ? rp.slot_stride - 1 - i : i)];
+        uint4 row = make_uint4(0u, 0u, 0u, 0u);
+        if (rows && live && wave == 0) row = rows[slot_base + slot];
         double E[9], R[9], t[3] = {0, 0, 0};
 #pragma unroll
         for (int q = 0; q < 9; ++q) { E[q] = 0; R[q] = 0; }
@@ -1470,9 +1537,11 @@
                         }
                     }
                     const int processed = min(j * SPLIT_STEP, n);
-                    if (rec_score < DBL_MAX && ((processed & 127) == 0 || processed == n))
-                        dead = dead || (((long long)cnt + (long long)(n - processed) <= rec_cnt) &&
-                                        (score + thr * (double)(processed - cnt) >= rec_score));
+                    if (rec_score < DBL_MAX && ((processed & 127) == 0 || processed == n)) {
+                        const int nc = cand_row_credit(row, row_shift, processed, n);
+                        dead = dead || (((long long)cnt + (long long)(n - processed - nc) <= rec_cnt) &&
+                                        (score + thr * (double)(processed - cnt + nc) >= rec_score));
+                    }
                 }
                 if (j < steps) {
                     const unsigned long long dm = __ballot(dead);
```

Result: slower. 125,800 (-3.3%).
